# HKUDS/GPT-ST

Measured on AMD Instinct MI355X. Metric: pretrain steps/sec at (B=32,T=12,N=170,C=64), higher is better.
Workload: dtype f32; 1 GPU; BASELINE configs[1]: PEMS08-shape synthetic pretrain step, per-GPU B=32 T=12 N=170 C=64 base=1, epoch 200/300 (adaptive mask + KL), fwd+loss+bwd+clip+Adam, hipGraph=True, 4 full optimiser steps on 4 different resident batches per graph replay; global_batch=32, parallelism=dp1

## Files before the change

gpt-st_amd/csrc/guidein.hip:

```cpp
#include "mfma_tile.h"
#include "kl_guest.h"

#define GI_CHUNKS 3

template <int C>
__global__ __launch_bounds__(256) void guide_in_fwd_kernel(const float* __restrict__ src, int lda, const float* __restrict__ w1,
                                                           const float* __restrict__ b1, const float* __restrict__ Wn, const float* __restrict__ bn,
                                                           float* __restrict__ h1, int BT, int N) {
    constexpr int LPR = C / 4, RPP = 256 / LPR, NQ = 256 / C, U = 4;
    __shared__ __attribute__((aligned(16))) float part[NQ * 2 * C];
    __shared__ __attribute__((aligned(16))) float vec[2 * C];
    const int n = blockIdx.x, chunk = blockIdx.y, tid = threadIdx.x;
    {
        const int q = tid / C, o = tid % C;
        const float* W = Wn + (size_t)n * C * C;
        float au = 0.f, ac = 0.f;
#pragma unroll 8
        for (int i = q * (C / NQ); i < (q + 1) * (C / NQ); ++i) {
            const float x = W[(size_t)i * C + o];
            au = fmaf(w1[i], x, au);
            ac = fmaf(b1[i], x, ac);
        }
        part[(q * 2 + 0) * C + o] = au;
        part[(q * 2 + 1) * C + o] = ac;
    }
    __syncthreads();
    if (tid < C) {
        float s0 = 0.f, s1 = 0.f;
#pragma unroll
        for (int q = 0; q < NQ; ++q) { s0 += part[(q * 2 + 0) * C + tid]; s1 += part[(q * 2 + 1) * C + tid]; }
        vec[tid] = s0; vec[C + tid] = s1 + bn[(size_t)n * C + tid];
    }
    __syncthreads();
    const int slot = tid / LPR, c4 = tid % LPR;
    const float4 u4 = ld4(vec + 4 * c4), k4 = ld4(vec + C + 4 * c4);
    const int per = (BT + GI_CHUNKS - 1) / GI_CHUNKS, r0 = chunk * per, r1 = min(BT, r0 + per);
    for (int rr = r0 + slot; rr < r1; rr += RPP * U) {
        float s[U];
#pragma unroll
        for (int u = 0; u < U; ++u) s[u] = src[((size_t)min(rr + u * RPP, r1 - 1) * N + n) * lda];
#pragma unroll
        for (int u = 0; u < U; ++u) {
            const int r = rr + u * RPP;
            if (r < r1) {
                float4 y = f4fma(s[u], u4, k4);
                y.x = lrelu(y.x); y.y = lrelu(y.y); y.z = lrelu(y.z); y.w = lrelu(y.w);
                st4(h1 + ((size_t)r * N + n) * C + 4 * c4, y);
            }
        }
    }
}

template <int C>
__global__ __launch_bounds__(256) void guide_in_bwd_kernel(const float* __restrict__ dPre, const float* __restrict__ src, int lda,
                                                           const float* __restrict__ w1, const float* __restrict__ b1, const float* __restrict__ Wn,
                                                           float* __restrict__ dWb, float* __restrict__ dinp, int BT, int N) {
    __shared__ __attribute__((aligned(16))) float lds[guide_in_bwd_lds_floats<C>()];
    guide_in_bwd_body<C>(dPre, src, lda, w1, b1, Wn, dWb, dinp, BT, N, blockIdx.x, lds);
}

extern "C" int gptst_guide_in_fwd(const float* src, int lda, const float* w1, const float* b1, const float* Wn, const float* bn, float* h1,
                                  int BT, int N, int C, void* stream) {
    if (!src || !w1 || !b1 || !Wn || !bn || !h1 || BT <= 0 || N <= 0 || lda <= 0) return GPTST_EARG;
    if (C == 64) hipLaunchKernelGGL((guide_in_fwd_kernel<64>), dim3(N, GI_CHUNKS), dim3(256), 0, (hipStream_t)stream, src, lda, w1, b1, Wn, bn, h1, BT, N);
    else if (C == 128) hipLaunchKernelGGL((guide_in_fwd_kernel<128>), dim3(N, GI_CHUNKS), dim3(256), 0, (hipStream_t)stream, src, lda, w1, b1, Wn, bn, h1, BT, N);
    else return GPTST_ESHAPE;
    GPTST_CHECK_LAUNCH();
    return GPTST_OK;
}

extern "C" int gptst_guide_in_bwd(const float* dPre, const float* src, int lda, const float* w1, const float* b1, const float* Wn, float* dWb,
                                  float* dinp, int BT, int N, int C, void* stream) {
    if (!dPre || !src || !w1 || !b1 || !Wn || !dWb || !dinp || BT <= 0 || N <= 0 || lda <= 0) return GPTST_EARG;
    if (C == 64) hipLaunchKernelGGL((guide_in_bwd_kernel<64>), dim3(N), dim3(256), 0, (hipStream_t)stream, dPre, src, lda, w1, b1, Wn, dWb, dinp, BT, N);
    else if (C == 128) hipLaunchKernelGGL((guide_in_bwd_kernel<128>), dim3(N), dim3(256), 0, (hipStream_t)stream, dPre, src, lda, w1, b1, Wn, dWb, dinp, BT, N);
    else return GPTST_ESHAPE;
    GPTST_CHECK_LAUNCH();
    return GPTST_OK;
}

template <int C>
__global__ __launch_bounds__(256) void guide_uc_kernel(const float* __restrict__ w1, const float* __restrict__ b1, const float* __restrict__ Wn,
                                                       const float* __restrict__ bn, float* __restrict__ uc) {
    constexpr int NQ = 256 / C;
    __shared__ __attribute__((aligned(16))) float part[NQ * 2 * C];
    const int n = blockIdx.x, tid = threadIdx.x;
    const int q = tid / C, o = tid % C;
    const float* W = Wn + (size_t)n * C * C;
    float au = 0.f, ac = 0.f;
#pragma unroll 8
    for (int i = q * (C / NQ); i < (q + 1) * (C / NQ); ++i) {
        const float x = W[(size_t)i * C + o];
        au = fmaf(w1[i], x, au);
        ac = fmaf(b1[i], x, ac);
    }
    part[(q * 2 + 0) * C + o] = au;
    part[(q * 2 + 1) * C + o] = ac;
    __syncthreads();
    if (tid < C) {
        float s0 = 0.f, s1 = 0.f;
#pragma unroll
        for (int qq = 0; qq < NQ; ++qq) { s0 += part[(qq * 2 + 0) * C + tid]; s1 += part[(qq * 2 + 1) * C + tid]; }
        uc[(size_t)n * 2 * C + tid] = s0;
        uc[(size_t)n * 2 * C + C + tid] = s1 + bn[(size_t)n * C + tid];
    }
}

#define GH_P 68
extern thread_local int g_apply_tpw;
__global__ __launch_bounds__(256, 2) void guide_head_fwd_kernel(const float* __restrict__ src, int lda, const float* __restrict__ uc,
                                                                const float* __restrict__ Wbt, const float* __restrict__ bbt,
                                                                const float* __restrict__ W3, const float* __restrict__ b3,
                                                                float* __restrict__ h1, float* __restrict__ h2, float* __restrict__ prob,
                                                                int* __restrict__ label, int N, int J, int tiles_per_wave) {
    constexpr int C = 64;
    __shared__ __attribute__((aligned(16))) float Wl[C * C];
    __shared__ __attribute__((aligned(16))) float tl[4][16 * GH_P];
    const int lane = threadIdx.x & 63, wave = threadIdx.x >> 6;
    const int j = lane & 15, kk = lane >> 4;
    const int g = blockIdx.x;
    const int ntiles = (N + 15) / 16;
    const int t0 = (blockIdx.y * 4 + wave) * tiles_per_wave, t1 = min(ntiles, t0 + tiles_per_wave);
    const float4 bias4 = ld4(bbt + (size_t)g * C + 4 * j);
    float4 bw[4];
#pragma unroll
    for (int q = 0; q < 4; ++q) bw[q] = j < J ? ld4(W3 + (size_t)j * C + 16 * q + 4 * kk) : f4zero();
    const float bj = j < J ? b3[j] : 0.f;
    float sn;
    float4 un[4], cn[4];
    auto fetch = [&](int t) {
        const int m = min(t * 16 + j, N - 1);
        sn = src[((size_t)g * N + m) * lda];
#pragma unroll
        for (int q = 0; q < 4; ++q) { un[q] = ld4(uc + (size_t)m * 2 * C + 16 * q + 4 * kk); cn[q] = ld4(uc + (size_t)m * 2 * C + C + 16 * q + 4 * kk); }
    };
    if (t0 < t1) fetch(t0);
    load_w_lds<C, 256>(Wl, Wbt + (size_t)g * C * C, 0, threadIdx.x);
    __syncthreads();
    float4 bv[4][4];
#pragma unroll
    for (int q = 0; q < 4; ++q)
#pragma unroll
        for (int e = 0; e < 4; ++e) bv[q][e] = ld4(Wl + (16 * q + 4 * kk + e) * C + 4 * j);
    float* tile = tl[wave];
    for (int t = t0; t < t1; ++t) {
        float4 a[4];
        const int mrow = t * 16 + j;
#pragma unroll
        for (int q = 0; q < 4; ++q) {
            float4 y = f4fma(sn, un[q], cn[q]);
            y.x = lrelu(y.x); y.y = lrelu(y.y); y.z = lrelu(y.z); y.w = lrelu(y.w);
            if (mrow < N) st4(h1 + ((size_t)g * N + mrow) * C + 16 * q + 4 * kk, y); else y = f4zero();
            a[q] = y;
        }
        if (t + 1 < t1) fetch(t + 1);
        SB();
        f32x4 acc[4];
#pragma unroll
        for (int ct = 0; ct < 4; ++ct) acc[ct] = (f32x4){0.f, 0.f, 0.f, 0.f};
#pragma unroll
        for (int q = 0; q < 4; ++q) {
            const float av[4] = {a[q].x, a[q].y, a[q].z, a[q].w};
#pragma unroll
            for (int e = 0; e < 4; ++e) {
                acc[0] = __builtin_amdgcn_mfma_f32_16x16x4f32(av[e], bv[q][e].x, acc[0], 0, 0, 0);
                acc[1] = __builtin_amdgcn_mfma_f32_16x16x4f32(av[e], bv[q][e].y, acc[1], 0, 0, 0);
                acc[2] = __builtin_amdgcn_mfma_f32_16x16x4f32(av[e], bv[q][e].z, acc[2], 0, 0, 0);
                acc[3] = __builtin_amdgcn_mfma_f32_16x16x4f32(av[e], bv[q][e].w, acc[3], 0, 0, 0);
            }
        }
        SB();
#pragma unroll
        for (int r = 0; r < 4; ++r) {
            const int m = t * 16 + kk * 4 + r;
            float4 y = f4add(make_float4(acc[0][r], acc[1][r], acc[2][r], acc[3][r]), bias4);
            y.x = lrelu(y.x); y.y = lrelu(y.y); y.z = lrelu(y.z); y.w = lrelu(y.w);
            if (m < N) st4(h2 + ((size_t)g * N + m) * C + 4 * j, y);
            st4(tile + (kk * 4 + r) * GH_P + 4 * j, y);
        }
        f32x4 z0 = {0.f, 0.f, 0.f, 0.f}, z1 = {0.f, 0.f, 0.f, 0.f};
#pragma unroll
        for (int q = 0; q < 4; ++q) {
            const float4 x = ld4(tile + j * GH_P + 16 * q + 4 * kk);
            z0 = __builtin_amdgcn_mfma_f32_16x16x4f32(x.x, bw[q].x, z0, 0, 0, 0);
            z1 = __builtin_amdgcn_mfma_f32_16x16x4f32(x.y, bw[q].y, z1, 0, 0, 0);
            z0 = __builtin_amdgcn_mfma_f32_16x16x4f32(x.z, bw[q].z, z0, 0, 0, 0);
            z1 = __builtin_amdgcn_mfma_f32_16x16x4f32(x.w, bw[q].w, z1, 0, 0, 0);
        }
#pragma unroll
        for (int r = 0; r < 4; ++r) {
            const int m = t * 16 + kk * 4 + r;
            const size_t i = (size_t)g * N + m;
            float v = z0[r] + z1[r] + bj;
            const float mx = group_max<16>(j < J ? v : -3.0e38f);
            const float e = j < J ? expf(v - mx) : 0.f;
            v = e / group_sum<16>(e);
            if (m < N && j < J) prob[i * J + j] = v;
            const float vv = j < J ? v : -3.0e38f;
            const float gm = group_max<16>(vv);
            const int first = (int)(-group_max<16>(vv == gm ? -(float)j : -3.0e38f));
            if (m < N && j == 0) label[i] = first;
        }
    }
}

extern "C" int gptst_guide_uc_floats(int N, int C) { return N * 2 * C; }

extern "C" int gptst_guide_head_fwd(const float* src, int lda, const float* w1, const float* b1, const float* Wn, const float* bn, const float* Wbt,
                                    const float* bbt, const float* W3, const float* b3, float* uc, float* h1, float* h2, float* prob, int* label,
                                    int BT, int N, int C, int J, void* stream) {
    if (!src || !w1 || !b1 || !Wn || !bn || !Wbt || !bbt || !W3 || !b3 || !uc || !h1 || !h2 || !prob || !label || BT <= 0 || N <= 0 || lda <= 0 || J <= 0)
        return GPTST_EARG;
    if (C != 64 || J > 16) return GPTST_ESHAPE;
    hipLaunchKernelGGL((guide_uc_kernel<64>), dim3(N), dim3(256), 0, (hipStream_t)stream, w1, b1, Wn, bn, uc);
    const int ntiles = (N + 15) / 16;
    int tpw = 1;
    if (g_apply_tpw > 0) tpw = g_apply_tpw;
    if (tpw < 1) tpw = 1;
    const int gy = (ntiles + 4 * tpw - 1) / (4 * tpw);
    hipLaunchKernelGGL(guide_head_fwd_kernel, dim3(BT, gy), dim3(256), 0, (hipStream_t)stream, src, lda, uc, Wbt, bbt, W3, b3, h1, h2, prob, label, N, J, tpw);
    GPTST_CHECK_LAUNCH();
    return GPTST_OK;
}
```

gpt-st_amd/csrc/stepbegin.hip:

```cpp
#include "common.h"

__device__ __forceinline__ void philox4x32_10(unsigned c0, unsigned c1, unsigned c2, unsigned c3, unsigned k0, unsigned k1, unsigned (&o)[4]) {
#pragma unroll
    for (int r = 0; r < 10; ++r) {
        const unsigned long long p0 = 0xD2511F53ull * c0, p1 = 0xCD9E8D57ull * c2;
        const unsigned n0 = (unsigned)(p1 >> 32) ^ c1 ^ k0, n1 = (unsigned)p1, n2 = (unsigned)(p0 >> 32) ^ c3 ^ k1, n3 = (unsigned)p0;
        c0 = n0; c1 = n1; c2 = n2; c3 = n3;
        k0 += 0x9E3779B9u; k1 += 0xBB67AE85u;
    }
    o[0] = c0; o[1] = c1; o[2] = c2; o[3] = c3;
}

__global__ __launch_bounds__(256) void step_begin_kernel(float* __restrict__ z0, long n0, float* __restrict__ z1, long n1,
                                                         const float* __restrict__ src, float* __restrict__ tidx, int BT, int N, int lda,
                                                         int base, float* __restrict__ noise, long n_noise, const int* __restrict__ rng) {
    const long q0 = n0 / 4, q1 = n1 / 4, stride = (long)gridDim.x * 256;
    for (long i = (long)blockIdx.x * 256 + threadIdx.x; i < q0 + q1; i += stride) {
        if (i < q0) st4(z0 + 4 * i, f4zero()); else st4(z1 + 4 * (i - q0), f4zero());
    }
    if (blockIdx.x == 0) {
        for (long i = 4 * q0 + threadIdx.x; i < n0; i += 256) z0[i] = 0.f;
        for (long i = 4 * q1 + threadIdx.x; i < n1; i += 256) z1[i] = 0.f;
    }
    if (tidx != nullptr)
        for (long i = (long)blockIdx.x * 256 + threadIdx.x; i < 2L * BT; i += stride)
            tidx[i] = src[(size_t)(i / 2) * N * lda + base + (i & 1)];
    if (noise != nullptr) {
        const unsigned seed = (unsigned)rng[0], step = (unsigned)rng[1];
        for (long i = (long)blockIdx.x * 256 + threadIdx.x; 4 * i < n_noise; i += stride) {
            unsigned w[4];
            philox4x32_10((unsigned)i, (unsigned)(i >> 32), step, 0u, seed, 0x5EEDu, w);
            const float4 u = make_float4((w[0] >> 8) * 5.9604644775390625e-8f, (w[1] >> 8) * 5.9604644775390625e-8f,
                                         (w[2] >> 8) * 5.9604644775390625e-8f, (w[3] >> 8) * 5.9604644775390625e-8f);
            if (4 * i + 3 < n_noise) st4(noise + 4 * i, u);
            else { const float uv[4] = {u.x, u.y, u.z, u.w}; for (int k = 0; 4 * i + k < n_noise; ++k) noise[4 * i + k] = uv[k]; }
        }
    }
}

extern "C" int gptst_step_begin(float* z0, long n0, float* z1, long n1, const float* src, float* tidx, int BT, int N, int lda, int base,
                                float* noise, long n_noise, const int* rng, void* stream) {
    if (!z0 || n0 <= 0 || n1 < 0 || (n1 > 0 && !z1) || (tidx && (!src || BT <= 0 || N <= 0 || lda < base + 2))) return GPTST_EARG;
    if (noise && (n_noise <= 0 || !rng)) return GPTST_EARG;
    long q = (n0 + n1) / 4;
    int nb = (int)((q + 255) / 256); if (nb > 1024) nb = 1024; if (nb < 1) nb = 1;
    hipLaunchKernelGGL(step_begin_kernel, dim3(nb), dim3(256), 0, (hipStream_t)stream, z0, n0, z1, n1, src, tidx, BT, N, lda, base, noise,
                       noise ? n_noise : 0L, rng);
    GPTST_CHECK_LAUNCH();
    return GPTST_OK;
}
```

gpt-st_amd/csrc/timefeat.hip:

```cpp
#include "common.h"

struct TfParams {
    const float *wd, *bd, *ww, *bw, *w1, *b1, *w2, *b2, *w3, *b3;
};
struct TfGrads {
    float *wd, *bd, *ww, *bw, *w1, *b1, *w2, *b2, *w3, *b3;
};

template <int E, int NT = 256> struct TfCfg { static constexpr int ROWS = NT / E; };

template <int E>
__device__ __forceinline__ float tf_matvec(const float (&wrow)[E], float b, const float* __restrict__ xline) {
    float s = b;
#pragma unroll
    for (int i = 0; i < E; ++i) s = fmaf(wrow[i], xline[i], s);
    return s;
}

template <int E>
__device__ __forceinline__ float tf_input(const TfParams& p, const float* __restrict__ tidx, int r, int e, int K) {
    float s = p.bd[e] + p.bw[e];
    for (int k = 0; k < K; ++k) {
        s = fmaf(p.wd[e * K + k], tidx[((size_t)r * K + k) * 2 + 0], s);
        s = fmaf(p.ww[e * K + k], tidx[((size_t)r * K + k) * 2 + 1], s);
    }
    return s;
}

#define TF_SH_FLOATS (7 * 128 * 3)

template <int E>
__device__ __forceinline__ void tf_fwd_body(const TfParams& p, const float* __restrict__ tidx, float* __restrict__ out,
                                            int rows, int K, int blk, float* __restrict__ shraw) {
    constexpr int ROWS = TfCfg<E>::ROWS;
    float (*line)[E + 1] = reinterpret_cast<float (*)[E + 1]>(shraw);
    const int e = threadIdx.x % E, rl = threadIdx.x / E;
    const int r = blk * ROWS + rl;
    const bool valid = r < rows;
    float w1[E], w2[E], w3[E];
#pragma unroll
    for (int i = 0; i < E; ++i) { w1[i] = p.w1[e * E + i]; w2[i] = p.w2[e * E + i]; w3[i] = p.w3[e * E + i]; }
    line[rl][e] = valid ? tf_input<E>(p, tidx, r, e, K) : 0.f;
    __syncthreads();
    float h = fmaxf(tf_matvec<E>(w1, p.b1[e], line[rl]), 0.f);
    __syncthreads();
    line[rl][e] = h;
    __syncthreads();
    h = fmaxf(tf_matvec<E>(w2, p.b2[e], line[rl]), 0.f);
    __syncthreads();
    line[rl][e] = h;
    __syncthreads();
    h = tf_matvec<E>(w3, p.b3[e], line[rl]);
    if (valid) out[(size_t)r * E + e] = h;
}

template <bool DET> __device__ __forceinline__ void tf_add(float* p, float v) { if (DET) *p += v; else atomicAdd(p, v); }

template <int E, bool DET, int NT>
__device__ __forceinline__ void tf_bwd_body(const TfParams& p, const TfGrads& g, const float* __restrict__ tidx,
                                            const float* __restrict__ dout, int rows, int K, int blk, float* __restrict__ shraw) {
    constexpr int ROWS = TfCfg<E, NT>::ROWS;
    float (*sh)[ROWS][E + 1] = reinterpret_cast<float (*)[ROWS][E + 1]>(shraw);
    const int tid = threadIdx.x, e = tid % E, rl = tid / E;
    const int r = blk * ROWS + rl;
    const bool valid = r < rows;
    float w1[E], w2[E], w3[E], c1[E], c2[E], c3[E];
#pragma unroll
    for (int i = 0; i < E; ++i) {
        w1[i] = p.w1[e * E + i]; w2[i] = p.w2[e * E + i]; w3[i] = p.w3[e * E + i];
        c1[i] = p.w1[i * E + e]; c2[i] = p.w2[i * E + e]; c3[i] = p.w3[i * E + e];
    }
    const float h0 = valid ? tf_input<E>(p, tidx, r, e, K) : 0.f;
    sh[0][rl][e] = h0;
    __syncthreads();
    const float h1 = fmaxf(tf_matvec<E>(w1, p.b1[e], sh[0][rl]), 0.f);
    sh[1][rl][e] = h1;
    __syncthreads();
    const float h2 = fmaxf(tf_matvec<E>(w2, p.b2[e], sh[1][rl]), 0.f);
    sh[2][rl][e] = h2;
    const float d3 = valid ? dout[(size_t)r * E + e] : 0.f;
    sh[3][rl][e] = d3;
    __syncthreads();
    const float z2 = h2 > 0.f ? tf_matvec<E>(c3, 0.f, sh[3][rl]) : 0.f;
    sh[4][rl][e] = z2;
    __syncthreads();
    const float z1 = h1 > 0.f ? tf_matvec<E>(c2, 0.f, sh[4][rl]) : 0.f;
    sh[5][rl][e] = z1;
    __syncthreads();
    const float z0 = tf_matvec<E>(c1, 0.f, sh[5][rl]);
    sh[6][rl][e] = z0;
    __syncthreads();
    const int nrow = min(ROWS, rows - blk * ROWS);
    for (int idx = tid; idx < 3 * E * E; idx += NT) {
        const int which = idx / (E * E), eo = (idx / E) % E, i = idx % E;
        const int ga = which == 0 ? 3 : (which == 1 ? 4 : 5), gb = which == 0 ? 2 : (which == 1 ? 1 : 0);
        float s = 0.f;
        for (int rr = 0; rr < nrow; ++rr) s = fmaf(sh[ga][rr][eo], sh[gb][rr][i], s);
        float* dst = which == 0 ? g.w3 : (which == 1 ? g.w2 : g.w1);
        tf_add<DET>(dst + eo * E + i, s);
    }
    for (int idx = tid; idx < 4 * E; idx += NT) {
        const int which = idx / E, eo = idx % E;
        const int ga = which == 0 ? 3 : (which == 1 ? 4 : (which == 2 ? 5 : 6));
        float s = 0.f;
        for (int rr = 0; rr < nrow; ++rr) s += sh[ga][rr][eo];
        if (which == 0) tf_add<DET>(g.b3 + eo, s);
        else if (which == 1) tf_add<DET>(g.b2 + eo, s);
        else if (which == 2) tf_add<DET>(g.b1 + eo, s);
        else { tf_add<DET>(g.bd + eo, s); tf_add<DET>(g.bw + eo, s); }
    }
    for (int idx = tid; idx < 2 * E * K; idx += NT) {
        const int ch = idx / (E * K), eo = (idx / K) % E, k = idx % K;
        float s = 0.f;
        for (int rr = 0; rr < nrow; ++rr)
            s = fmaf(sh[6][rr][eo], tidx[((size_t)(blk * ROWS + rr) * K + k) * 2 + ch], s);
        tf_add<DET>((ch == 0 ? g.wd : g.ww) + eo * K + k, s);
    }
}

#define TF_MAXJ 16
struct TfJob { TfParams p; TfGrads g; const float* tidx; float* out; const float* dout; int rows, K, E, blk0; };
struct TfJobs { TfJob j[TF_MAXJ]; int n; };

#define TF_DET_T 1024
template <int BWD>
__global__ __launch_bounds__(BWD == 2 ? TF_DET_T : 256) void timefeat_jobs_kernel(TfJobs t) {
    constexpr int NT = BWD == 2 ? TF_DET_T : 256;
    __shared__ float shraw[TF_SH_FLOATS * (NT / 256)];
    int q = 0;
    if (BWD == 2) q = blockIdx.x;
    else for (int i = 1; i < t.n; ++i) if ((int)blockIdx.x >= t.j[i].blk0) q = i;
    const TfJob& a = t.j[q];
    const int blk = blockIdx.x - a.blk0;
    const int nblk = (a.rows + NT / a.E - 1) / (NT / a.E);
#define TF_CASE(EE)                                                                              \
    case EE:                                                                                     \
        if (BWD == 2) { for (int b2 = 0; b2 < nblk; ++b2) { tf_bwd_body<EE, true, NT>(a.p, a.g, a.tidx, a.dout, a.rows, a.K, b2, shraw); __syncthreads(); } } \
        else if (BWD == 1) tf_bwd_body<EE, false, NT>(a.p, a.g, a.tidx, a.dout, a.rows, a.K, blk, shraw); \
        else tf_fwd_body<EE>(a.p, a.tidx, a.out, a.rows, a.K, blk, shraw);                       \
        break;
    switch (a.E) { TF_CASE(2) TF_CASE(4) TF_CASE(8) TF_CASE(16) default: break; }
#undef TF_CASE
}

static int tf_launch(TfJobs& t, int bwd, hipStream_t st) {
    int nb = 0;
    for (int q = 0; q < t.n; ++q) {
        TfJob& a = t.j[q];
        if (!a.p.wd || !a.tidx || a.rows <= 0 || a.K <= 0 || (bwd ? (!a.dout || !a.g.wd) : !a.out)) return GPTST_EARG;
        if (a.E != 2 && a.E != 4 && a.E != 8 && a.E != 16) return GPTST_ESHAPE;
        const int rows_per = 256 / a.E;
        a.blk0 = nb;
        nb += (a.rows + rows_per - 1) / rows_per;
    }
    if (bwd && g_deterministic) hipLaunchKernelGGL(timefeat_jobs_kernel<2>, dim3(t.n), dim3(TF_DET_T), 0, st, t);
    else if (bwd) hipLaunchKernelGGL(timefeat_jobs_kernel<1>, dim3(nb), dim3(256), 0, st, t);
    else hipLaunchKernelGGL(timefeat_jobs_kernel<0>, dim3(nb), dim3(256), 0, st, t);
    GPTST_CHECK_LAUNCH();
    return GPTST_OK;
}

extern "C" int gptst_timefeat_fwd(const float* wd, const float* bd, const float* ww, const float* bw, const float* w1, const float* b1,
                                  const float* w2, const float* b2, const float* w3, const float* b3, const float* tidx, float* out,
                                  int rows, int K, int E, void* stream) {
    TfJobs t; t.n = 1;
    t.j[0] = TfJob{TfParams{wd, bd, ww, bw, w1, b1, w2, b2, w3, b3}, TfGrads{}, tidx, out, nullptr, rows, K, E, 0};
    return tf_launch(t, 0, (hipStream_t)stream);
}

extern "C" int gptst_timefeat_bwd(const float* wd, const float* bd, const float* ww, const float* bw, const float* w1, const float* b1,
                                  const float* w2, const float* b2, const float* w3, const float* b3, float* gwd, float* gbd, float* gww,
                                  float* gbw, float* gw1, float* gb1, float* gw2, float* gb2, float* gw3, float* gb3, const float* tidx,
                                  const float* dout, int rows, int K, int E, void* stream) {
    TfJobs t; t.n = 1;
    t.j[0] = TfJob{TfParams{wd, bd, ww, bw, w1, b1, w2, b2, w3, b3}, TfGrads{gwd, gbd, gww, gbw, gw1, gb1, gw2, gb2, gw3, gb3}, tidx,
                   nullptr, dout, rows, K, E, 0};
    return tf_launch(t, 1, (hipStream_t)stream);
}

extern "C" int gptst_timefeat_jobs(int njobs, int bwd, const void* const* params, const void* const* grads, const float* tidx,
                                   const void* const* io, const int* rows, const int* K, const int* E, void* stream) {
    if (njobs <= 0 || njobs > TF_MAXJ || !params || !io || !rows || !K || !E || (bwd && !grads)) return GPTST_EARG;
    TfJobs t; t.n = njobs;
    for (int q = 0; q < njobs; ++q) {
        const float* const* pp = (const float* const*)params + 10 * q;
        TfGrads g{};
        if (bwd) { float* const* gg = (float* const*)grads + 10 * q; g = TfGrads{gg[0], gg[1], gg[2], gg[3], gg[4], gg[5], gg[6], gg[7], gg[8], gg[9]}; }
        t.j[q] = TfJob{TfParams{pp[0], pp[1], pp[2], pp[3], pp[4], pp[5], pp[6], pp[7], pp[8], pp[9]}, g, tidx,
                       bwd ? nullptr : (float*)io[q], bwd ? (const float*)io[q] : nullptr, rows[q], K[q], E[q], 0};
    }
    return tf_launch(t, bwd, (hipStream_t)stream);
}
```

gpt-st_amd/engine.py:

```python
import contextlib
import os
import threading
from typing import Any, NamedTuple

import torch

from . import _C, ops
from .ops import (EPI_ADD_DPRE, EPI_ADD_PREMUL, EPI_LRELU, EPI_PREMUL, EPI_PLAIN, EPI_RES_LRELU, MODE_NODE, MODE_SHARED, MODE_TIME, PRO_DPRE, PRO_NONE)

TF_NAMES = ("ln_day", "ln_week", "ln1", "ln2", "ln")


class ZeroArena:

    def __init__(self, device):
        self.device, self.buf, self.off, self.need = device, None, 0, 0

    def begin(self, zero=True):
        pending = None
        if self.buf is None or self.buf.numel() < self.need:
            self.buf = torch.zeros(max(self.need, 1), device=self.device) if self.need else None
        elif self.buf is not None:
            if zero:
                self.buf.zero_()
            else:
                pending = self.buf
        self.off, self.need = 0, 0
        return pending

    def zeros(self, *shape):
        n = 1
        for d in shape:
            n *= d
        n4 = (n + 3) // 4 * 4
        self.need += n4
        if self.buf is None or self.off + n4 > self.buf.numel():
            return torch.zeros(*shape, device=self.device)
        t = self.buf[self.off:self.off + n].view(*shape)
        self.off += n4
        return t


class _Context(threading.local):
    ARENA = None
    NODE_REDUCE = None
    NO_HANDOFFS = False


CTX = _Context()




class Reductions:

    def __init__(self):
        self.jobs = ops.PoolJobs()
        self.late = ops.PoolJobs()
        self.no_carry = False
        self.grams = []
        self.tf = []
        self.keep = []
        self.on_bucket = None
        self.nbucket = 0
        self.bucket_inline = False
        self.fork_side = None
        self.forked = False
        self._dG = self._dA = None

    def take_carry(self, mb):
        if not CARRY_RED or self.no_carry or self.on_bucket is not None or CTX.NODE_REDUCE is not None or not self.jobs.jobs:
            return None
        take, rest, nb = [], [], 0.0
        for j in self.jobs.jobs:
            b = 4.0 * j[5] * j[7] * j[8] / 2 ** 20
            if j[0] in (ops.PoolJobs.BWD_POOL, ops.PoolJobs.BWD_EMB) and nb + b <= mb and len(take) < 100 and (j[7] | j[9]) % 4 == 0:
                take.append(j); nb += b
            else:
                rest.append(j)
        if not take:
            return None
        self.jobs.jobs = rest
        c = ops.PoolJobs()
        c.jobs = take
        return c

    def untake(self, carry):
        if carry is not None and carry.jobs:
            self.jobs.jobs = carry.jobs + self.jobs.jobs
            carry.jobs = []

    def gram(self, A, dG, dA, N, nsG):
        self.grams.append((A, dG, dA, N, nsG))

    def timefeat(self, p, g, pfx, tidx, dout, spg=False):
        B, T = tidx.shape[0], tidx.shape[1]
        rows, K = (B, T) if spg else (B * T, 1)
        self.tf.append((_tf_tensors(p, pfx), _tf_tensors(g, pfx), dout, rows, K))

    def flush_async(self, tidx):
        if self.bucket_inline and self.on_bucket is not None and self.nbucket == 0 and (self.jobs.jobs or self.late.jobs or self.grams or self.tf):
            self._run(tidx)
            self.fork_side.wait_stream(torch.cuda.current_stream())
            with torch.cuda.stream(self.fork_side):
                self.on_bucket(0)
            self.forked = True
            self.nbucket += 1

    def flush(self, tidx):
        self._run(tidx)
        if self.forked:
            torch.cuda.current_stream().wait_stream(self.fork_side)
            self.forked = False

    def _run(self, tidx):
        gr, self.grams = sorted(self.grams, key=lambda t: t[0].data_ptr()), []
        while gr:
            A, dG, dA, N, nsG = gr.pop(0)
            while gr and gr[0][0].data_ptr() == A.data_ptr() + 4 * A.numel() and gr[0][1].data_ptr() == dG.data_ptr() + 4 * dG.numel() \
                    and gr[0][2].data_ptr() == dA.data_ptr() + 4 * dA.numel() and gr[0][3:] == (N, nsG):
                A2, dG2, dA2 = gr.pop(0)[:3]
                A = torch.as_strided(A, (A.shape[0] + A2.shape[0],) + tuple(A.shape[1:]), A.stride())
                dG = torch.as_strided(dG, (dG.shape[0] + dG2.shape[0],) + tuple(dG.shape[1:]), dG.stride())
                dA = torch.as_strided(dA, (dA.shape[0] + dA2.shape[0],) + tuple(dA.shape[1:]), dA.stride())
            ops.gram_bwd(A, dG, out=dA, layers=A.shape[0] // N, nsplit=nsG)
        self.jobs.jobs, self.late.jobs = self.jobs.jobs + self.late.jobs, []
        self.jobs.launch()
        tf, self.tf = self.tf, []
        ops.timefeat_jobs_bwd(tf, tidx)
        self.keep = []


def _zeros(ref, *shape):
    if CTX.ARENA is not None:
        return CTX.ARENA.zeros(*shape)
    return torch.zeros(*shape, device=ref.device)


def _tf_tensors(d, pfx):
    out = []
    for n in TF_NAMES:
        out += [d[pfx + n + ".weight"], d[pfx + n + ".bias"]]
    return out


def _tf_job(p, pfx, tidx, spg=False):
    B, T = tidx.shape[0], tidx.shape[1]
    rows, K = (B, T) if spg else (B * T, 1)
    return (_tf_tensors(p, pfx), rows, K)


DROP_R = os.environ.get("GPTST_DROP_R", "0") == "1"


def _ht_fused_bwd(dims):
    return dims[3] == 64 and FUSE_HT_BWD


def hypertem_core_fwd(x, G, Wbt, bbt, dims):
    B, T, N, C = dims
    if C == 64:
        keep = not (DROP_R and _ht_fused_bwd(dims) and ops.wgrad_nsplit(MODE_TIME, B * T, N, C) == 1)
        R, out = ops.hypertem_fwd(x.view(B, T, N, C), G, Wbt, bbt, want_R=keep)
        R, out = (R.view(-1, C) if keep else None), out.view(-1, C)
    else:
        R = ops.tmix(x.view(B, T, N, C), G).view(-1, C)
        out = ops.apply(R, Wbt, MODE_TIME, B * T, N, bias=bbt, resid=x, epi=EPI_RES_LRELU)
    return out, (x, R, out, G, Wbt)


FUSE_HT_BWD = True


def graph_grad_splits(dims):
    return dims[0] if dims[3] == 64 else 1


CHAIN128 = os.environ.get("GPTST_CHAIN128", "1") == "1"


def chain_ok(dims):
    return _ht_fused_bwd(dims) or (CHAIN128 and dims[3] == 128)


def _wb_cols(dWb, C):
    return dWb[:, :C * C], dWb[:, C * C:]


def _wb_record(dWb, ns, C):
    return dWb[:, :C * C], ns, dWb[:, C * C:]


def hypertem_core_bwd(saved, dout, dG_out, dims, chain=False, premul=False):
    B, T, N, C = dims
    x, R, out, G, Wbt = saved
    BT = B * T
    assert not chain or chain_ok(dims)
    if _ht_fused_bwd(dims):
        dx, dWb, ns, _ = ops.hypertem_bwd_wgrad(dout.view(B, T, N, C), None if chain else out.view(B, T, N, C), x.view(B, T, N, C), G, Wbt,
                                                R.view(B, T, N, C) if R is not None else None, dG=dG_out, premul=chain and premul)
        dWbt, dbias = _wb_cols(dWb, C)
        dx = dx.view(-1, C)
    elif C == 64:
        dWb, ns = ops.wgrad(R, dout, MODE_TIME, BT, N, D2=out, pro=PRO_DPRE, colsum_d=True)
        dWbt, dbias = _wb_cols(dWb, C)
        dx, _, _ = ops.hypertem_bwd(dout.view(B, T, N, C), out.view(B, T, N, C), x.view(B, T, N, C), G, Wbt, dG=dG_out, want_dbias=False)
        dx = dx.view(-1, C)
    elif chain:
        dWb, ns = ops.wgrad(R, dout, MODE_TIME, BT, N, colsum_d=True)
        dWbt, dbias = _wb_cols(dWb, C)
        dR = ops.apply(dout, Wbt, MODE_TIME, BT, N, transw=True)
        dx, _ = ops.tmix_bwd_chain(dR.view(B, T, N, C), x.view(B, T, N, C), G, dout.view(B, T, N, C), premul=premul, dG=dG_out[0])
        dx = dx.view(-1, C)
    else:
        dWb, ns = ops.wgrad(R, dout, MODE_TIME, BT, N, D2=out, pro=PRO_DPRE, colsum_d=True)
        dWbt, dbias = _wb_cols(dWb, C)
        dR = ops.apply(dout, Wbt, MODE_TIME, BT, N, A2=out, transw=True, pro=PRO_DPRE)
        dx, _ = ops.tmix_bwd(dR.view(B, T, N, C), x.view(B, T, N, C), G, dout.view(B, T, N, C), out.view(B, T, N, C), dG=dG_out[0])
        dx = dx.view(-1, C)
    return dx, (dWbt, ns, dbias)


CARRY_RED = os.environ.get("GPTST_CARRY_RED", "1") == "1"
CARRY_MB = float(os.environ.get("GPTST_CARRY_MB", "25"))
CARRY_KL = os.environ.get("GPTST_CARRY_KL", "1") == "1"
PAIR_UNDER_DP = os.environ.get("GPTST_PAIR_UNDER_DP", "1") == "1"
PAIR_BWD = os.environ.get("GPTST_PAIR_BWD", "1") == "1"


@contextlib.contextmanager
def no_handoffs():
    from . import _C
    keep = (CTX.NO_HANDOFFS, _C.lib().value("gptst_mask_cooperative_state"))
    CTX.NO_HANDOFFS = True
    _C.lib().call("gptst_mask_cooperative", 0)
    try:
        yield
    finally:
        CTX.NO_HANDOFFS = keep[0]
        _C.lib().call("gptst_mask_cooperative", keep[1])


def pair_bwd_on():
    return PAIR_BWD and not CTX.NO_HANDOFFS


def cross_role():
    return 0 if CTX.NO_HANDOFFS else CROSS_ROLE


def _ht_pair_shape_ok(dims):
    B, T, N, C = dims
    if T != 12 or C != 64:
        return False
    ns = ops.wgrad_nsplit(MODE_TIME, B * T, N, C)
    rps = (-(-N // ns) + 1) & ~1
    return -(-N // rps) == ns


def ht_pair_ok(saved1, saved0, dims):
    return (pair_bwd_on() and dims[3] == 64 and not isinstance(saved1, EncIn) and saved1[1] is not None and saved0[1] is not None
            and _ht_fused_bwd(dims) and _ht_pair_shape_ok(dims))


class PendingH1:

    def __init__(self, saved, dd, dG, dWb):
        self.saved, self.dd, self.dG, self.dWb = saved, dd, dG, dWb


def ht_pair_bwd(saved1, saved0, dout, dG1, dG0, dims, dWb1=None):
    B, T, N, C = dims
    if not ht_pair_ok(saved1, saved0, dims):
        assert dWb1 is None
        return None
    x1, R1, _, G1, Wbt1 = saved1
    x0, R0, _, G0, Wbt0 = saved0
    v = lambda a: a.view(B, T, N, C)
    r = ops.hypertem_bwd_pair(v(dout), v(x1), G1, Wbt1, v(R1), v(x0), G0, Wbt0, v(R0), dG1, dG0, _zeros(dout, B), dWb1=dWb1)
    assert r is not None or dWb1 is None
    if r is None:
        return None
    dmid, dx0, dWb1, dWb0, ns = r
    return dx0.view(-1, C), _wb_record(dWb1, ns, C), _wb_record(dWb0, ns, C)


FUSE_CROSS = os.environ.get("GPTST_FUSE_CROSS", "1") == "1"
CAP_LIN = os.environ.get("GPTST_CAP_LIN", "1") == "1"
CROSS_ROLE = int(os.environ.get("GPTST_CROSS_ROLE", "1"))


def cap_head_fwd(p, pfx, x, dadj, dyn, dims, num_route, HS, HT):
    B, T, N, C = dims
    c, s, Y = ops.cap_route_fwd(x.view(B, T, N, C), p[pfx + "ln_p.weight"], p[pfx + "ln_p.bias"], dadj, HS, num_route,
                                reduce_nodes=CTX.NODE_REDUCE, want_Y=True)
    fused = ops.cap_cross_rec_fwd(s, dyn, p[pfx + "mask_template"], c, B, T, N, HS, HT) if (FUSE_CROSS and CTX.NODE_REDUCE is None) else None
    if fused is not None:
        v, Ht, Rt, rec = fused
    else:
        v, Ht, Rt = ops.cap_cross_fwd(s, dyn, p[pfx + "mask_template"], B, T, HS, HT)
        rec = ops.cap_rec_fwd(c, v, N, C)
    return rec, c, (s, v, Ht, Rt, Y)


def cap_core_fwd(p, pfx, x, dadj, dyn, Wn, bn, dims, num_route, HS, HT):
    B, T, N, C = dims
    rec, c, (s, v, Ht, Rt, Y) = cap_head_fwd(p, pfx, x, dadj, dyn, dims, num_route, HS, HT)
    out = ops.apply(rec, Wn, MODE_NODE, B * T, N, bias=bn, resid=x, epi=EPI_RES_LRELU)
    return out, c, (x, out, rec, c, s, v, Ht, Rt, dyn, Wn, Y)


CHAIN_FWD = os.environ.get("GPTST_CHAIN_FWD", "1") == "1"


def chain_fwd_ok(dims):
    return CHAIN_FWD and dims[3] == 64 and not DROP_R


def ht_chain_fwd(x, stages, dims, kl=None):
    B, T, N, C = dims
    res = ops.hypertem_chain_fwd(x.view(B, T, N, C), stages, guest=kl.guest() if kl is not None else None)
    saved, xin = [], x
    for (G, Wbt, _b), (R, o) in zip(stages, res):
        o = o.view(-1, C)
        saved.append((xin, R.view(-1, C), o, G, Wbt))
        xin = o
    return saved, xin


def cap_core_bwd(p, g, pfx, saved, dout, dims, HS, HT, red, chain=False):
    B, T, N, C = dims
    x, out, rec, c, s, v, Ht, Rt, dyn, Wn, Y = saved
    BT, dev = B * T, x.device
    assert not chain or chain_ok(dims)
    if C == 64:
        drec, dWn, dbn, ns = ops.apply_wgrad(dout, None if chain else out, rec, Wn, MODE_NODE, BT, N)
    elif chain:
        drec = ops.apply(dout, Wn, MODE_NODE, BT, N, transw=True)
        dWb, ns = ops.wgrad(rec, dout, MODE_NODE, BT, N, colsum_d=True)
        dWn, dbn = _wb_cols(dWb, C)
    else:
        drec = ops.apply(dout, Wn, MODE_NODE, BT, N, A2=out, transw=True, pro=PRO_DPRE)
        dWb, ns = ops.wgrad(rec, dout, MODE_NODE, BT, N, D2=out, pro=PRO_DPRE, colsum_d=True)
        dWn, dbn = _wb_cols(dWb, C)
    dc1, dv = ops.cap_rec_bwd(drec, c, v, reduce_nodes=CTX.NODE_REDUCE)
    gw, gb = g[pfx + "ln_p.weight"], g[pfx + "ln_p.bias"]
    if FUSE_CROSS and CAP_LIN and C == 64 and CTX.NODE_REDUCE is None and Y is None:
        carry = red.take_carry(CARRY_MB) if cross_role() and _C.lib().value("gptst_cap_route_roles_ok", B, T, N, C, HS, HT) == 1 else None
        lin = ops.cap_cross_route_lin_bwd(x.view(B, T, N, C), p[pfx + "ln_p.weight"], p[pfx + "ln_p.bias"], c, dc1, dv, s, Rt, Ht, dyn,
                                          p[pfx + "mask_template"], dout, None if chain else out, chain, B, T, HS, HT,
                                          flags=_zeros(x, 4 * B) if cross_role() else None, jobs=carry)
        red.untake(carry)
        if lin is not None:
            dx, dWp, dbp, dlogit, ddyn = lin
            red.jobs.bwd_pool(_ones(dev, dWp.shape[0]), dWp, gw.view(1, C * C))
            red.jobs.bwd_pool(_ones(dev, dbp.shape[0]), dbp, gb.view(1, C))
            return dx, (dWn, ns, dbn, ddyn, dlogit)
    fused = None
    if FUSE_CROSS and CTX.NODE_REDUCE is None and Y is None:
        fused = ops.cap_cross_route_bwd(x.view(B, T, N, C), p[pfx + "ln_p.weight"], p[pfx + "ln_p.bias"], c, dc1, dv, s, Rt, Ht, dyn,
                                        p[pfx + "mask_template"], B, T, HS, HT, flags=_zeros(x, 4 * B) if cross_role() else None)
    if fused is not None:
        dY, dlogit, ddyn = fused
    else:
        dS, ddyn = ops.cap_cross_bwd(dv, s, Rt, Ht, dyn, p[pfx + "mask_template"], B, T, HS, HT)
        dY, dlogit = ops.cap_route_bwd(x.view(B, T, N, C), p[pfx + "ln_p.weight"], p[pfx + "ln_p.bias"], c, dc1, dS, Y=Y)
    if C == 64:
        dx, dWp, dbp, ns2 = ops.linear_bwd(dY, x, p[pfx + "ln_p.weight"], dout, None if chain else out, premul=chain)
        red.jobs.bwd_pool(_ones(dev, ns2), dWp, gw.view(1, C * C))
        red.jobs.bwd_pool(_ones(dev, ns2), dbp, gb.view(1, C))
    else:
        if chain:
            dx = ops.apply(dY, p[pfx + "ln_p.weight"], MODE_SHARED, BT, N, resid=dout, resid2=x, epi=EPI_ADD_PREMUL)
        else:
            dx = ops.apply(dY, p[pfx + "ln_p.weight"], MODE_SHARED, BT, N, resid=dout, resid2=out, epi=EPI_ADD_DPRE)
        dWp, ns2 = ops.wgrad(dY, x, MODE_SHARED, BT, N, colsum_a=True)
        dWp, dbp = _wb_cols(dWp, C)
        red.jobs.bwd_pool(_ones(dev, ns2), dWp, gw.view(1, C * C))
        red.jobs.bwd_pool(_ones(dev, ns2), dbp, gb.view(1, C))
    return dx, (dWn, ns, dbn, ddyn, dlogit)


_ONES = {}


def _ones(dev, n=1):
    if (dev, n) not in _ONES:
        _ONES[(dev, n)] = torch.ones(n, 1, device=dev)
    return _ONES[(dev, n)]


def condlin_fwd(x, Wg, bg, mode, dims):
    B, T, N, C = dims
    out = ops.apply(x, Wg, mode, B * T, N, bias=bg, epi=EPI_LRELU)
    return out, (x, out, Wg)


def condlin_bwd(saved, dout, emb, wpool, bpool, g_wpool, g_bpool, d_emb, mode, dims, red, chain=False, premul=False, carried=None):
    B, T, N, C = dims
    x, out, Wg = saved
    R, K = emb.shape
    assert not chain or chain_ok(dims)
    if carried is not None:
        dx, dW, db, ns = carried
    elif C == 64:
        dx, dW, db, ns = ops.apply_wgrad(dout, None if chain else out, x, Wg, mode, B * T, N, premul=chain and premul)
    elif chain:
        dx = (ops.apply(dout, Wg, mode, B * T, N, transw=True, resid2=x, epi=EPI_PREMUL) if premul
              else ops.apply(dout, Wg, mode, B * T, N, transw=True))
        dWb, ns = ops.wgrad(x, dout, mode, B * T, N, colsum_d=True)
        dW, db = _wb_cols(dWb, C)
    else:
        dx = ops.apply(dout, Wg, mode, B * T, N, A2=out, transw=True, pro=PRO_DPRE)
        dWb, ns = ops.wgrad(x, dout, mode, B * T, N, D2=out, pro=PRO_DPRE, colsum_d=True)
        dW, db = _wb_cols(dWb, C)
    dW = dW if dW.dim() == 2 else dW.view(ns * R, C * C)
    red.jobs.bwd_pool(emb, dW, g_wpool.view(K, C * C), nsplit=ns)
    red.jobs.bwd_pool(emb, db, g_bpool, nsplit=ns)
    red.jobs.bwd_emb(dW, wpool.view(K, C * C), d_emb, nsplit=ns)
    red.jobs.bwd_emb(db, bpool, d_emb, nsplit=ns)
    return dx


ENC, DEC = "encoder.STHCN_encode.", "decoder.STHCN_decode."
GUIDE_TF = "encoder.teb4mask."


def _sthcn_names(pfx):
    return [pfx + "hyperTem%d." % i for i in (1, 2, 3, 4)], [pfx + "cap1.", pfx + "cap2."]


def _sthcn_gen_jobs(p, pfx, emb, jobs, A_all, dims, G_all=None, gjobs=None):
    gjobs = jobs if gjobs is None else gjobs
    B, T, N, C = dims
    time_eb, teb, tes = emb
    ne, nes = p[pfx + "node_embeddings"], p[pfx + "node_embeddings_spg"]
    hts, cps = _sthcn_names(pfx)
    adj0 = p[hts[0] + "adj"]
    d, Hm = adj0.shape[0], adj0.shape[1]
    cadj, tadj = p[cps[0] + "adj"], p[cps[0] + "t_adj"]
    ds, HS, HT = cadj.shape[0], cadj.shape[1], tadj.shape[1]
    for i, h in enumerate(hts):
        jobs.fwd(ne, p[h + "adj"].view(d, Hm * T), out=A_all[i])
        if G_all is not None:
            gjobs.gram(ne, p[h + "adj"].view(d, Hm * T), out=G_all[i], A=A_all[i])
    Wb = [jobs.fwd(time_eb, t) for h in hts for t in (p[h + "weights_pool"], p[h + "bias_pool"])]
    Wn = [jobs.fwd(nes, t) for c in cps for t in (p[c + "weights_spa"], p[c + "bias_spa"])]
    dadj = [jobs.fwd(teb, p[c + "adj"].view(ds, HS * N)) for c in cps]
    dyn = [jobs.fwd(tes, p[c + "t_adj"].view(ds, HT * T * HS)).view(B, HT, T * HS) for c in cps]
    return dict(emb=emb, gen=(A_all, hts, cps, d, Hm, ds, HS, HT), Wb=Wb, Wn=Wn, dadj=dadj, dyn=dyn)


def gen_all(p, tidx, dims, which=(ENC, DEC), guide=True, defer=False):
    B, T, N, C = dims
    tfj = []
    for pfx in which:
        tfj += [_tf_job(p, pfx + "time_feature1.", tidx), _tf_job(p, pfx + "time_feature1_.", tidx),
                _tf_job(p, pfx + "time_feature2.", tidx, spg=True)]
    if guide:
        tfj.append(_tf_job(p, GUIDE_TF, tidx))
    embs = ops.timefeat_jobs_fwd(tfj, tidx)
    jobs = ops.PoolJobs()
    now = ops.PoolJobs() if defer else jobs
    res = {}
    L = 4 * len(which)
    if guide:
        gj = now
        m = "encoder.MLP_RL."
        t4m = embs[-1]
        res["guide"] = (t4m, gj.fwd(p["encoder.neb4mask"], p[m + "weights_pool_spa"]), gj.fwd(p["encoder.neb4mask"], p[m + "bias_pool_spa"]),
                        gj.fwd(t4m, p[m + "weights_pool_tem"]), gj.fwd(t4m, p[m + "bias_pool_tem"]))
    if L:
        adj0 = p[which[0] + "hyperTem1.adj"]
        Hm = adj0.shape[1]
        A_all = torch.empty(L, N, Hm * T, device=tidx.device)
        G_all = torch.empty(L, N, T, T, device=tidx.device)
        for k, pfx in enumerate(which):
            res[pfx] = _sthcn_gen_jobs(p, pfx, embs[3 * k:3 * k + 3], jobs, A_all[4 * k:4 * k + 4], dims, G_all[4 * k:4 * k + 4])
            res[pfx]["slot"] = (k, len(which))
            res[pfx]["G_all"] = G_all[4 * k:4 * k + 4]

    if defer:
        now.launch()
        res["pending"] = jobs
        return res
    jobs.launch()
    return res


def sthcn_fwd(p, pfx, tidx, x, dims, num_route, gen=None, head=None, next_gen=None, kl=None):
    if gen is None:
        gen = gen_all(p, tidx, dims, which=(pfx,), guide=False)[pfx]
    A_all, hts, cps, d, Hm, ds, HS, HT = gen["gen"]
    Wn, dadj, dyn = gen["Wn"], gen["dadj"], gen["dyn"]
    ht = lambda i, gn=gen: (gn["G_all"][i], gn["Wb"][2 * i], gn["Wb"][2 * i + 1])
    cap = lambda i, x: cap_core_fwd(p, cps[i], x, dadj[i], dyn[i], Wn[2 * i], Wn[2 * i + 1], dims, num_route, HS, HT)
    pairs = chain_fwd_ok(dims)
    sv, nhead = {}, None
    if head is not None:
        x, sv["h1"] = head
    else:
        x, sv["h1"] = hypertem_core_fwd(x, *ht(0), dims)
    x, c1, sv["c1"] = cap(0, x)
    if pairs:
        if kl is not None and kl.c1 is None:
            kl.c1 = c1
        (sv["h2"], sv["h3"]), x = ht_chain_fwd(x, [ht(1), ht(2)], dims, kl)
    else:
        x, sv["h2"] = hypertem_core_fwd(x, *ht(1), dims)
        x, sv["h3"] = hypertem_core_fwd(x, *ht(2), dims)
    x, _, sv["c2"] = cap(1, x)
    if pairs and next_gen is not None:
        (sv["h4"], h1n), xn = ht_chain_fwd(x, [ht(3), ht(0, next_gen)], dims, kl)
        x, nhead = sv["h4"][2], (xn, h1n)
    else:
        x, sv["h4"] = hypertem_core_fwd(x, *ht(3), dims)
    sv["emb"] = gen["emb"]
    sv["gen"] = gen["gen"]
    sv["slot"] = gen.get("slot")
    return x, c1, sv, nhead


def _grad_buffers(red, slot, N, T, HmT, ref, nsG):
    if slot is None:
        return torch.empty(4, nsG, N, T, T, device=ref.device), torch.empty(4, N, HmT, device=ref.device)
    k, n = slot
    if red._dG is None or red._dG.shape[0] != 4 * n:
        red._dG = torch.empty(4 * n, nsG, N, T, T, device=ref.device)
        red._dA = torch.empty(4 * n, N, HmT, device=ref.device)
    return red._dG[4 * k:4 * k + 4], red._dA[4 * k:4 * k + 4]


def sthcn_bwd(p, g, pfx, tidx, sv, dout, dims, red, chain=False, premul_in=False, defer_h1=False, after_pending=None):
    B, T, N, C = dims
    time_eb, teb, tes = sv["emb"]
    A_all, hts, cps, d, Hm, ds, HS, HT = sv["gen"]
    ne, nes = p[pfx + "node_embeddings"], p[pfx + "node_embeddings_spg"]
    dne, dnes = g[pfx + "node_embeddings"], g[pfx + "node_embeddings_spg"]
    d_te, d_teb, d_tes = _zeros(time_eb, *time_eb.shape), _zeros(teb, *teb.shape), _zeros(tes, *tes.shape)
    nsG = graph_grad_splits(dims)
    dG_all, dA_all = _grad_buffers(red, sv.get("slot"), N, T, Hm * T, dout, nsG)
    J = red.jobs
    CC, BT = C * C, B * T

    def queue_ht(h, hp):
        dWbt, ns, dbias = hp
        J.bwd_pool(time_eb, dWbt, g[h + "weights_pool"].view(d, CC), nsplit=ns)
        J.bwd_pool(time_eb, dbias, g[h + "bias_pool"], nsplit=ns)
        J.bwd_emb(dWbt, p[h + "weights_pool"].view(d, CC), d_te, nsplit=ns)
        J.bwd_emb(dbias, p[h + "bias_pool"], d_te, nsplit=ns)

    def queue_cap(c, cp):
        dWn, ns, dbn, ddyn, dlogit = cp
        dW2 = dWn if dWn.dim() == 2 else dWn.view(ns * N, CC)
        J.bwd_pool(nes, dW2, g[c + "weights_spa"].view(d, CC), nsplit=ns)
        J.bwd_pool(nes, dbn, g[c + "bias_spa"], nsplit=ns)
        J.bwd_emb(dW2, p[c + "weights_spa"].view(d, CC), dnes, nsplit=ns)
        J.bwd_emb(dbn, p[c + "bias_spa"], dnes, nsplit=ns)
        dd2 = ddyn.view(B, HT * T * HS)
        J.bwd_pool(tes, dd2, g[c + "t_adj"].view(ds, HT * T * HS))
        J.bwd_emb(dd2, p[c + "t_adj"].view(ds, HT * T * HS), d_tes)
        dl2 = dlogit.view(BT, HS * N)
        J.bwd_pool(teb, dl2, g[c + "adj"].view(ds, HS * N))
        J.bwd_emb(dl2, p[c + "adj"].view(ds, HS * N), d_teb)

    if isinstance(dout, PendingH1):
        up = dout
        dd, _, hp4 = ht_pair_bwd(up.saved, sv["h4"], up.dd, up.dG, dG_all[3], dims, dWb1=up.dWb)
        red.keep.append(up)
        if after_pending is not None:
            after_pending()
    else:
        dd, hp4 = hypertem_core_bwd(sv["h4"], dout, dG_all[3], dims, chain, True)
    queue_ht(hts[3], hp4)
    dd, cp2 = cap_core_bwd(p, g, cps[1], sv["c2"], dd, dims, HS, HT, red, chain)
    queue_cap(cps[1], cp2)
    pair = ht_pair_bwd(sv["h3"], sv["h2"], dd, dG_all[2], dG_all[1], dims) if chain and pair_bwd_on() else None
    if pair is not None:
        dd, hp3, hp2 = pair
    else:
        dd, hp3 = hypertem_core_bwd(sv["h3"], dd, dG_all[2], dims, chain, True)
        dd, hp2 = hypertem_core_bwd(sv["h2"], dd, dG_all[1], dims, chain, True)
    queue_ht(hts[2], hp3)
    queue_ht(hts[1], hp2)
    dd, cp1 = cap_core_bwd(p, g, cps[0], sv["c1"], dd, dims, HS, HT, red, chain)
    queue_cap(cps[0], cp1)
    if isinstance(sv["h1"], EncIn):
        assert chain
        e = sv["h1"]
        w, bi = p["encoder.dim_in_flow.weight"], p["encoder.dim_in_flow.bias"]
        if nsG == B:
            dWb, _, dinp = ops.encin_ht1_bwd(dd.view(B, T, N, C), e.source, e.mask, e.fill, w, bi, e.Wbt, e.ab, e.wv, dG=dG_all[0])
        else:
            dWb, dGb, dinp = ops.encin_ht1_bwd(dd.view(B, T, N, C), e.source, e.mask, e.fill, w, bi, e.Wbt, e.ab, e.wv)
            torch.sum(dGb, 0, out=dG_all[0][0])
        hp1 = _wb_record(dWb, 1, C)
        wb = _wb_view(g["encoder.dim_in_flow.weight"], g["encoder.dim_in_flow.bias"])
        if wb is not None:
            red.jobs.bwd_pool(_ones(dd.device, dinp.shape[0]), dinp, wb)
        else:
            g["encoder.dim_in_flow.weight"].add_(dinp[:, :C].sum(0).view(C, 1))
            g["encoder.dim_in_flow.bias"].add_(dinp[:, C:].sum(0))
        red.keep.append((dinp, dWb))
        dd = None
    elif defer_h1:
        assert chain and premul_in
        ns = ops.wgrad_nsplit(MODE_TIME, B * T, N, C)
        dWb = torch.empty(ns * B * T, C * C + C, device=dd.device, dtype=torch.float32)
        hp1 = _wb_record(dWb, ns, C)
        dd = PendingH1(sv["h1"], dd, dG_all[0], dWb)
    else:
        dd, hp1 = hypertem_core_bwd(sv["h1"], dd, dG_all[0], dims, chain, premul_in)
    queue_ht(hts[0], hp1)
    red.gram(A_all.view(4 * N, Hm, T), dG_all, dA_all.view(4 * N, Hm, T), N, nsG)
    for i, h in enumerate(hts):
        red.late.bwd_pool(ne, dA_all[i], g[h + "adj"].view(d, Hm * T))
        red.late.bwd_emb(dA_all[i], p[h + "adj"].view(d, Hm * T), dne)
    red.timefeat(p, g, pfx + "time_feature1.", tidx, d_te)
    red.timefeat(p, g, pfx + "time_feature1_.", tidx, d_teb)
    red.timefeat(p, g, pfx + "time_feature2.", tidx, d_tes, spg=True)
    red.keep.append((sv, hp1, hp2, hp3, hp4, cp1, cp2, dout))
    return dd


class EncIn:

    def __init__(self, source, mask, fill, Wbt, ab, wv):
        self.source, self.mask, self.fill, self.Wbt, self.ab, self.wv = source, mask, fill, Wbt, ab, wv


ENCIN = os.environ.get("GPTST_ENCIN", "1") == "1"


def encin_ok(dims, base):
    return ENCIN and base == 1 and dims[3] in (64, 128) and dims[1] == 12 and chain_ok(dims)


GUIDEIN = os.environ.get("GPTST_GUIDEIN", "1") == "1"
GUIDE_HEAD = os.environ.get("GPTST_GUIDE_HEAD", "1") == "1"


def guide_fwd(p, source, tidx, dims, base, gen=None, lowrank_in=False):
    B, T, N, C = dims
    if gen is None:
        gen = gen_all(p, tidx, dims, which=(), guide=True)["guide"]
    t4m, Wspa, bspa, Wtem, btem = gen
    m = "encoder.MLP_RL."
    if lowrank_in and GUIDEIN and GUIDE_HEAD and base == 1 and C == 64:
        r = ops.guide_head_fwd(source, p[m + "ln1.weight"], p[m + "ln1.bias"], Wspa, bspa, Wtem, btem, p[m + "ln3.weight"], p[m + "ln3.bias"])
        if r is not None:
            h1, h2, prob, label = r
            return prob, (t4m, ("lowrank", Wspa), (h1, h2, Wtem), h2, label)
    if lowrank_in and GUIDEIN and base == 1 and C in (64, 128):
        h1 = ops.guide_in_fwd(source, p[m + "ln1.weight"], p[m + "ln1.bias"], Wspa, bspa)
        s1 = ("lowrank", Wspa)
    else:
        h0 = ops.lin_in(source, base + 2, base, p[m + "ln1.weight"], p[m + "ln1.bias"], C)
        h1, s1 = condlin_fwd(h0, Wspa, bspa, MODE_NODE, dims)
    h2, s2 = condlin_fwd(h1, Wtem, btem, MODE_TIME, dims)
    prob, label = ops.rowdot(h2, p[m + "ln3.weight"], p[m + "ln3.bias"], softmax=True, want_label=True)
    return prob, (t4m, s1, s2, h2, label)


def _wb_view(gw, gb):
    n = gw.numel() + gb.numel()
    if gb.data_ptr() != gw.data_ptr() + 4 * gw.numel():
        return None
    return torch.as_strided(gw, (1, n), (n, 1))


def fused_tails_ok(p, C, base, HS):
    return (C in (64, 128) and base <= ops.TAIL_MAXJ and HS <= ops.TAIL_MAXJ
            and _wb_view(p["decoder.dim_flow_out.weight"], p["decoder.dim_flow_out.bias"]) is not None
            and _wb_view(p["encoder.MLP_RL.ln3.weight"], p["encoder.MLP_RL.ln3.bias"]) is not None)


def loss_tail(p, g, dec, source, mask, base, sigma, mu, thresh, sws, red, chain=False):
    wo = "decoder.dim_flow_out."
    out, dd, part = ops.tail_mae(dec, p[wo + "weight"], p[wo + "bias"], source, base + 2, mask, sigma, mu, thresh, sws, premul=chain)
    red.jobs.bwd_pool(_ones(dec.device, part.shape[0]), part, _wb_view(g[wo + "weight"], g[wo + "bias"]))
    red.keep.append((part, dd))
    return out, dd


def kl_head(p, g, sv_g, prob, c1, N, w, sws, red, chain=False, carried=None):
    m = "encoder.MLP_RL."
    dh2, part = carried if carried is not None else ops.tail_kl(sv_g[3], p[m + "ln3.weight"], prob, c1, N, w, sws, premul=chain)
    red.jobs.bwd_pool(_ones(prob.device, part.shape[0]), part, _wb_view(g[m + "ln3.weight"], g[m + "ln3.bias"]))
    red.keep.append((part, dh2))
    return dh2


def _linear_out_bwd(p, g, pfx, h, dy, C, chain, d_h=None):
    J = dy.shape[1]
    dh = ops.lin_in(dy, J, J, p[pfx + "weight"], None, C, wlayout=1)
    ops.rowouter(dy, J, J, h, g[pfx + "weight"], 1, asum=g[pfx + "bias"])
    if d_h is not None:
        dh = dh + d_h
    if chain:
        dh = dh * torch.where(h > 0, 1.0, 0.01)
    return dh


def guide_bwd(p, g, source, tidx, saved, dlogit, dims, base, red, dh2=None, chain=False, carried=(None, None)):
    B, T, N, C = dims
    t4m, s1, s2, h2 = saved[:4]
    m = "encoder.MLP_RL."
    if dh2 is None:
        dh2 = _linear_out_bwd(p, g, m + "ln3.", h2, dlogit, C, chain)
    d_t4m = _zeros(t4m, *t4m.shape)
    dh1 = condlin_bwd(s2, dh2, t4m, p[m + "weights_pool_tem"], p[m + "bias_pool_tem"], g[m + "weights_pool_tem"],
                      g[m + "bias_pool_tem"], d_t4m, MODE_TIME, dims, red, chain, True, carried=carried[0])
    if isinstance(s1[0], str):
        assert chain
        neb, wpool, bpool = p["encoder.neb4mask"], p[m + "weights_pool_spa"], p[m + "bias_pool_spa"]
        K = neb.shape[1]
        dWb, dinp = carried[1] if carried[1] is not None else ops.guide_in_bwd(dh1, source, p[m + "ln1.weight"], p[m + "ln1.bias"], s1[1])
        dW, db = _wb_cols(dWb, C)
        red.jobs.bwd_pool(neb, dW, g[m + "weights_pool_spa"].view(K, C * C))
        red.jobs.bwd_pool(neb, db, g[m + "bias_pool_spa"])
        red.jobs.bwd_emb(dW, wpool.view(K, C * C), g["encoder.neb4mask"])
        red.jobs.bwd_emb(db, bpool, g["encoder.neb4mask"])
        wb = _wb_view(g[m + "ln1.weight"], g[m + "ln1.bias"])
        if wb is not None:
            red.jobs.bwd_pool(_ones(dh1.device, N), dinp, wb)
        else:
            g[m + "ln1.weight"].add_(dinp[:, :C].sum(0).view(C, 1))
            g[m + "ln1.bias"].add_(dinp[:, C:].sum(0))
        red.keep.append((dWb, dinp))
        dh0 = None
    else:
        dh0 = condlin_bwd(s1, dh1, p["encoder.neb4mask"], p[m + "weights_pool_spa"], p[m + "bias_pool_spa"],
                          g[m + "weights_pool_spa"], g[m + "bias_pool_spa"], g["encoder.neb4mask"], MODE_NODE, dims, red, chain, False)
        _in_proj_grads(source, base, dh0, g[m + "ln1.weight"], g[m + "ln1.bias"], None, 0.0, red)
    red.timefeat(p, g, GUIDE_TF, tidx, d_t4m)
    red.keep.append((saved, dlogit, dh2, dh1, dh0))


def kl_carry_ok(dims, HS, sv_g):
    B, T, N, C = dims
    return (CARRY_KL and C == 64 and T == 12 and HS <= ops.TAIL_MAXJ and chain_fwd_ok(dims) and chain_ok(dims)
            and sv_g is not None and isinstance(sv_g[1][0], str))


class KlCarry:

    def __init__(self, p, sv_g, prob, source, dims, w, sws):
        self.p, self.sv_g, self.prob, self.source, self.dims, self.w, self.sws = p, sv_g, prob, source, dims, w, sws
        self.c1 = None
        self.stage = 0
        self.out = {}

    def guest(self):
        if self.c1 is None or self.stage == 3:
            return None
        B, T, N, C = self.dims
        m = "encoder.MLP_RL."
        p, sv_g, dev = self.p, self.sv_g, self.prob.device
        HS = self.prob.shape[1]
        st = self.stage + 1
        f = dict(device=dev, dtype=torch.float32)
        if st == 1:
            h2, W3 = sv_g[3], p[m + "ln3.weight"]
            dh2 = torch.empty_like(h2)
            part = torch.empty(ops.tail_parts(B * T * N), HS * C + HS, **f)
            self.out[1] = (dh2, part)
            ts = [h2, W3, self.prob, self.c1, dh2, part, self.sws]
        elif st == 2:
            h1, _, Wtem = sv_g[2]
            dh2 = self.out[1][0]
            ns = _C.lib().value("gptst_apply_wgrad_nsplit", MODE_TIME, B * T, N)
            dh1, dW, db = torch.empty_like(h1), torch.empty(ns * B * T, C * C, **f), torch.empty(ns * B * T, C, **f)
            self.out[2] = (dh1, dW, db, ns)
            ts = [dh2, h1, Wtem, dh1, dW, db]
        else:
            dWb, dinp = torch.empty(N, C * C + C, **f), torch.empty(N, 2 * C, **f)
            self.out[3] = (dWb, dinp)
            ts = [self.out[2][0], self.source, p[m + "ln1.weight"], p[m + "ln1.bias"], sv_g[1][1], dWb, dinp]
        self.stage = st
        return (st, ts, 0, ops.kl_guest_blocks(st, B, T, N), HS, self.source.shape[-1], self.w)

    def carried(self, st):
        return self.out.get(st)


def _in_proj_grads(source, base, dY, gW, gb, mask, fill, red):
    wb = _wb_view(gW, gb)
    if base == 1 and wb is not None:
        C = dY.shape[1]
        part = ops.rowouter_part(source, base + 2, base, dY, mask=mask, fill=fill)
        red.jobs.bwd_pool(_ones(dY.device, part.shape[0]), part[:, :2 * C], wb)
        red.keep.append(part)
    else:
        ops.rowouter(source, base + 2, base, dY, gW, 0, csum=gb, mask=mask, fill=fill)


class Forward(NamedTuple):
    emb: Any
    c1: Any
    dec: Any
    out: Any
    sv_e: Any
    sv_d: Any


def autoencoder_fwd(p, source, mask, dims, base, num_route, scaler_zeros, gen=None, tidx=None, lowrank_in=False, kl=None, head=True,
                    decoder=True, join=True):
    B, T, N, C = dims
    if tidx is None:
        tidx = source[:, :, 0, base:base + 2].contiguous()
    gen_e, gen_d = (gen[ENC], gen[DEC] if decoder else None) if gen is not None else (None, None)
    first = None
    if lowrank_in and gen_e is not None and encin_ok(dims, base):
        w, bi = p["encoder.dim_in_flow.weight"], p["encoder.dim_in_flow.bias"]
        G1, Wb = gen_e["G_all"][0], gen_e["Wb"]
        o1, ab, wv = ops.encin_ht1_fwd(source, base, mask, 0.0 if mask is None else scaler_zeros, w, bi, G1, Wb[0], Wb[1])
        first = (o1.view(-1, C), EncIn(source, mask, 0.0 if mask is None else scaler_zeros, Wb[0], ab, wv))
        x0 = None
    else:
        x0 = ops.lin_in(source, base + 2, base, p["encoder.dim_in_flow.weight"], p["encoder.dim_in_flow.bias"], C,
                        mask=mask, fill=scaler_zeros)
    emb, c1, sv_e, dec_h1 = sthcn_fwd(p, ENC, tidx, x0, dims, num_route, gen=gen_e, head=first, next_gen=gen_d if join else None, kl=kl)
    if not decoder:
        return Forward(emb, c1, None, None, sv_e, None)
    dec, _, sv_d, _ = sthcn_fwd(p, DEC, tidx, emb, dims, num_route, gen=gen_d, head=dec_h1, kl=kl)
    out = ops.rowdot(dec, p["decoder.dim_flow_out.weight"], p["decoder.dim_flow_out.bias"]) if head else None
    return Forward(emb, c1, dec, out, sv_e, sv_d)


def model_bwd(p, g, source, mask, tidx, sv_e, sv_d, dec, d_out, d_dec, dims, base, scaler_zeros, red, dd=None, chain=False):
    B, T, N, C = dims
    if dd is None:
        dd = _linear_out_bwd(p, g, "decoder.dim_flow_out.", dec, d_out, C, chain, d_h=d_dec)
    defer = (chain and (red.on_bucket is None or PAIR_UNDER_DP) and not isinstance(sv_d["h1"], EncIn)
             and ht_pair_ok(sv_d["h1"], sv_e["h4"], dims))
    late = defer and red.on_bucket is not None
    d_emb = sthcn_bwd(p, g, DEC, tidx, sv_d, dd, dims, red, chain, True, defer_h1=defer)
    if not late:
        red.flush_async(tidx)
    d_x0 = sthcn_bwd(p, g, ENC, tidx, sv_e, d_emb, dims, red, chain, False,
                     after_pending=(lambda: red.flush_async(tidx)) if late else None)
    red.flush_async(tidx)
    if d_x0 is not None:
        _in_proj_grads(source, base, d_x0, g["encoder.dim_in_flow.weight"], g["encoder.dim_in_flow.bias"], mask, scaler_zeros, red)


def step_bwd(p, g, source, mask, tidx, fw, prob, sv_g, dims, base, scaler_zeros, red, loss, stats, sws=None, with_kl=False, kl=None):
    B, T, N, C = dims
    sigma, mu, thresh = loss
    if sws is not None:
        chain = chain_ok(dims)
        done = kl.carried if kl is not None else (lambda st: None)
        _, dd = loss_tail(p, g, fw.dec, source, mask, base, sigma, mu, thresh, sws, red, chain=chain)
        model_bwd(p, g, source, mask, tidx, fw.sv_e, fw.sv_d, fw.dec, None, None, dims, base, scaler_zeros, red, dd=dd, chain=chain)
        if with_kl:
            dh2 = kl_head(p, g, sv_g, prob, fw.c1, N, 0.1, sws, red, chain=chain, carried=done(1))
            guide_bwd(p, g, source, tidx, sv_g, None, dims, base, red, dh2=dh2, chain=chain, carried=(done(2), done(3)))
    else:
        M = B * T * N
        ops.mae_fwd(fw.out, source, base + 2, mask, sigma, mu, thresh, M, base, stats)
        d_out = ops.mae_bwd(fw.out, source, base + 2, mask, sigma, mu, thresh, M, base, stats, normalize=False)
        model_bwd(p, g, source, mask, tidx, fw.sv_e, fw.sv_d, fw.dec, d_out, None, dims, base, scaler_zeros, red)
        if with_kl:
            dlogit = ops.kl(prob, fw.c1, N, 0.1, stats)
            guide_bwd(p, g, source, tidx, sv_g, dlogit, dims, base, red)


def module_bwd(p, g, source, mask, tidx, fw, prob, sv_g, dims, base, scaler_zeros, red, d_out, d_dec=None, d_prob=None, chain=False):
    model_bwd(p, g, source, mask, tidx, fw.sv_e, fw.sv_d, fw.dec, d_out, d_dec, dims, base, scaler_zeros, red, chain=chain)
    if d_prob is not None:
        dlogit = (prob * (d_prob - (d_prob * prob).sum(-1, keepdim=True))).contiguous()
        guide_bwd(p, g, source, tidx, sv_g, dlogit, dims, base, red, chain=chain)


def warm_up(fn):
    s = torch.cuda.Stream()
    s.wait_stream(torch.cuda.current_stream())
    with torch.cuda.stream(s):
        for _ in range(2):
            fn()
    torch.cuda.current_stream().wait_stream(s)
    torch.cuda.synchronize()
```

gpt-st_amd/ops.py:

```python
import torch

from . import _C

MODE_TIME, MODE_NODE, MODE_SHARED = 0, 1, 2
PRO_NONE, PRO_DPRE = 0, 1
EPI_PLAIN, EPI_RES_LRELU, EPI_ADD_DPRE, EPI_LRELU, EPI_ADD_PREMUL, EPI_PREMUL = 0, 1, 2, 3, 4, 5

_p = _C.ptr


TIMER = None
LAST_CALL = {}


CALL_LOCK = None


def _call(name, *args, tag="", nbytes=0):
    if CALL_LOCK is not None:
        with CALL_LOCK:
            _C.lib().call(name, *args, _C.stream())
        return
    if TIMER is None:
        _C.lib().call(name, *args, _C.stream())
        return
    e0, e1 = torch.cuda.Event(enable_timing=True), torch.cuda.Event(enable_timing=True)
    e0.record()
    _C.lib().call(name, *args, _C.stream())
    e1.record()
    TIMER.append((name, tag, e0, e1, nbytes))
    LAST_CALL[(name, tag)] = args


def _nb(*ts):
    return sum(t.numel() * t.element_size() for t in ts if t is not None)


def _chk(*ts):
    for t in ts:
        if t is not None:
            assert t.is_cuda and t.dtype == torch.float32 and t.is_contiguous(), (t.device, t.dtype, t.is_contiguous())


def poolgen(emb, pool, pool2=None):
    _chk(emb, pool, pool2)
    R, K = emb.shape
    cols = pool.numel() // K
    out = torch.empty((R,) + tuple(pool.shape[1:]), device=emb.device, dtype=torch.float32)
    out2, cols2 = None, 0
    if pool2 is not None:
        cols2 = pool2.numel() // K
        out2 = torch.empty((R,) + tuple(pool2.shape[1:]), device=emb.device, dtype=torch.float32)
    _call("gptst_poolgen_fwd", _p(emb), _p(pool), _p(out), cols, _p(pool2), _p(out2), cols2, R, K, nbytes=_nb(emb, pool, out, pool2, out2))
    return (out, out2) if pool2 is not None else out


def poolgen_bwd_pool(emb, dW, dpool, dW2=None, dpool2=None, nsplit=1):
    _chk(emb, dW, dpool, dW2, dpool2)
    R, K = emb.shape
    cols = dpool.numel() // K
    cols2 = dpool2.numel() // K if dpool2 is not None else 0
    _call("gptst_poolgen_bwd_pool", _p(emb), _p(dW), _p(dpool), cols, _p(dW2), _p(dpool2), cols2, R, nsplit, K,
          nbytes=_nb(emb, dW, dpool, dW2, dpool2))


def poolgen_bwd_emb(dW, pool, demb, dW2=None, pool2=None, nsplit=1):
    _chk(dW, pool, demb, dW2, pool2)
    R, K = demb.shape
    cols = pool.numel() // K
    cols2 = pool2.numel() // K if pool2 is not None else 0
    _call("gptst_poolgen_bwd_emb", _p(dW), _p(pool), cols, _p(dW2), _p(pool2), cols2, _p(demb), R, nsplit, K,
          nbytes=_nb(dW, pool, dW2, pool2, demb))


def _ptrs(ts):
    import ctypes
    return (ctypes.c_void_p * len(ts))(*[t.data_ptr() for t in ts])


def _ints(vs):
    import ctypes
    return (ctypes.c_int * len(vs))(*[int(v) for v in vs])


def poolgen_multi(emb, pools, outs=None):
    _chk(emb, *pools)
    R, K = emb.shape
    if outs is None:
        outs = [torch.empty((R,) + tuple(pl.shape[1:]), device=emb.device, dtype=torch.float32) for pl in pools]
    cols = [pl.numel() // K for pl in pools]
    _call("gptst_poolgen_fwd_multi", _p(emb), len(pools), _ptrs(pools), _ptrs(outs), _ints(cols), R, K, nbytes=_nb(emb, *pools, *outs))
    return outs


def poolgen_bwd_pool_multi(emb, dWs, dpools, nsplits=None):
    _chk(emb, *dWs, *dpools)
    R, K = emb.shape
    cols = [dp.numel() // K for dp in dpools]
    ns = nsplits if nsplits is not None else [1] * len(dWs)
    _call("gptst_poolgen_bwd_pool_multi", _p(emb), len(dWs), _ptrs(dWs), _ptrs(dpools), _ints(cols), _ints(ns), R, K,
          nbytes=_nb(emb, *dWs, *dpools))


def poolgen_bwd_emb_multi(dWs, pools, demb, nsplits=None):
    _chk(demb, *dWs, *pools)
    R, K = demb.shape
    cols = [pl.numel() // K for pl in pools]
    ns = nsplits if nsplits is not None else [1] * len(dWs)
    _call("gptst_poolgen_bwd_emb_multi", len(dWs), _ptrs(dWs), _ptrs(pools), _ints(cols), _ints(ns), _p(demb), R, K,
          nbytes=_nb(demb, *dWs, *pools))


class PoolJobs:
    FWD, BWD_POOL, BWD_EMB, GRAM = 0, 1, 2, 3

    def __init__(self):
        self.jobs = []
        self.post = []

    def fwd(self, emb, pool, out=None):
        _chk(emb, pool, out)
        R, K = emb.shape
        if out is None:
            out = torch.empty((R,) + tuple(pool.shape[1:]), device=emb.device, dtype=torch.float32)
        self.jobs.append((self.FWD, emb, None, pool, out, R, K, pool.numel() // K, 1, 0))
        return out

    def gram(self, emb, pool, out, A=None):
        _chk(emb, pool, out, A)
        R, K = emb.shape
        cols = pool.numel() // K
        assert cols % 12 == 0 and out.numel() == R * 144 and out.is_contiguous()
        if _C.lib().value("gptst_pool_jobs_gram_rows", K, cols) <= 0:
            assert A is not None and A.numel() == R * cols, "gram job does not fit and no forward output was given"
            self.post.append((A, out, R, cols // 12))
            return out
        self.jobs.append((self.GRAM, emb, None, pool, out, R, K, cols, 1, 0))
        return out

    @staticmethod
    def _ldx(dW, cols):
        assert dW.is_cuda and dW.dtype == torch.float32 and dW.dim() == 2 and dW.shape[1] == cols and dW.stride(1) == 1, (dW.shape, dW.stride(), cols)
        return dW.stride(0)

    def bwd_pool(self, emb, dW, dpool, nsplit=1):
        _chk(emb, dpool)
        R, K = emb.shape
        cols = dpool.numel() // K
        self.jobs.append((self.BWD_POOL, emb, dW, None, dpool, R, K, cols, nsplit, self._ldx(dW, cols)))

    def bwd_emb(self, dW, pool, demb, nsplit=1):
        _chk(pool, demb)
        R, K = demb.shape
        cols = pool.numel() // K
        self.jobs.append((self.BWD_EMB, None, dW, pool, demb, R, K, cols, nsplit, self._ldx(dW, cols)))

    def launch(self):
        js, self.jobs = self.jobs, []
        post, self.post = self.post, []
        if js:
            col = lambda i: [j[i] for j in js]
            _call("gptst_pool_jobs", len(js), _ints(col(0)), _ptrs0(col(1)), _ptrs0(col(2)), _ptrs0(col(3)), _ptrs0(col(4)), _ints(col(5)),
                  _ints(col(6)), _ints(col(7)), _ints(col(8)), _ints(col(9)), nbytes=_nb(*[t for j in js for t in j[1:5]]))
        for A, G, rows, Hm in post:
            _call("gptst_gram_fwd", _p(A), _p(G), rows, Hm)


def _ptrs0(ts):
    import ctypes
    return (ctypes.c_void_p * len(ts))(*[(t.data_ptr() if t is not None else None) for t in ts])


def apply(A, W, mode, BT, N, bias=None, resid=None, A2=None, transw=False, pro=PRO_NONE, epi=EPI_PLAIN, colsum=None,
          out=None, resid2=None):
    _chk(A, W, bias, resid, A2, resid2)
    C = A.shape[-1]
    if out is None:
        out = torch.empty_like(A)
    cs, ns = None, 0
    if colsum is not None:
        G = BT if mode == MODE_TIME else (N if mode == MODE_NODE else 1)
        ns = _C.lib().value("gptst_apply_nsplit", mode, BT, N, C)
        cs = torch.empty(ns * G, C, device=A.device, dtype=torch.float32)
    _call("gptst_apply", _p(A), _p(A2), _p(W), int(W.dim() == 3), int(transw), _p(bias), _p(resid), _p(resid2), _p(out), _p(cs),
          mode, pro, epi, BT, N, C, tag="mode%d pro%d epi%d" % (mode, pro, epi), nbytes=_nb(A, A2, W, bias, resid, resid2, out))
    if colsum is True:
        return out, cs, ns
    if colsum is not None:
        colsum.add_(cs.view(ns, -1, C).sum(0).view_as(colsum))
    return out


def apply_wgrad(dOut, Y, S, W, mode, BT, N, premul=False):
    _chk(dOut, Y, S, W)
    C = dOut.shape[-1]
    G = BT if mode == MODE_TIME else N
    ns = _C.lib().value("gptst_apply_wgrad_nsplit", mode, BT, N)
    dS = torch.empty_like(dOut)
    dW = torch.empty(ns * G, C * C, device=dOut.device, dtype=torch.float32)
    db = torch.empty(ns * G, C, device=dOut.device, dtype=torch.float32)
    _call("gptst_apply_wgrad", _p(dOut), _p(Y), _p(S), _p(W), _p(dS), _p(dW), _p(db), int(premul), mode, BT, N, C, tag="mode%d" % mode,
          nbytes=_nb(dOut, Y, S, W, dS, dW))
    return dS, dW, db, ns


def linear_bwd(dY, X, Wp, dOut, out, premul=False):
    _chk(dY, X, Wp, dOut, out)
    rows, C = dY.shape
    ns = _C.lib().value("gptst_linear_bwd_nsplit", rows)
    dX = torch.empty_like(dY)
    dWp = torch.empty(ns, C * C, device=dY.device, dtype=torch.float32)
    dbp = torch.empty(ns, C, device=dY.device, dtype=torch.float32)
    _call("gptst_linear_bwd", _p(dY), _p(X), _p(Wp), _p(dOut), _p(out), _p(dX), _p(dWp), _p(dbp), int(premul), rows, C,
          nbytes=_nb(dY, X, dOut, out, dX, dWp))
    return dX, dWp, dbp, ns


def wgrad_nsplit(mode, BT, N, C=64):
    return _C.lib().value("gptst_wgrad_nsplit", mode, BT, N, C)


def wgrad(A, D, mode, BT, N, D2=None, pro=PRO_NONE, colsum_a=False, colsum_d=False):
    _chk(A, D, D2)
    C = A.shape[-1]
    ns = wgrad_nsplit(mode, BT, N, C)
    G = BT if mode == MODE_TIME else (N if mode == MODE_NODE else 1)
    if colsum_a or colsum_d:
        dW = torch.empty(ns * G, C * C + C, device=A.device, dtype=torch.float32)
        _call("gptst_wgrad_colsum", _p(A), _p(D), _p(D2), _p(dW), mode, pro, 1 if colsum_a else 2, BT, N, C,
              tag="mode%d pro%d cs" % (mode, pro), nbytes=_nb(A, D, D2, dW))
    else:
        dW = torch.empty(ns * G, C, C, device=A.device, dtype=torch.float32)
        _call("gptst_wgrad", _p(A), _p(D), _p(D2), _p(dW), mode, pro, BT, N, C, tag="mode%d pro%d" % (mode, pro), nbytes=_nb(A, D, D2, dW))
    return dW, ns


def gram_fwd(A):
    N, Hm, T = A.shape
    G = torch.empty(N, T, T, device=A.device, dtype=torch.float32)
    _call("gptst_gram_fwd", _p(A), _p(G), N, Hm)
    return G


def gram_bwd(A, dG, out=None, layers=1, nsplit=1):
    LN, Hm, T = A.shape
    dA = out if out is not None else torch.empty_like(A)
    _call("gptst_gram_bwd", _p(A), _p(dG), _p(dA), layers, LN // layers, Hm, nsplit)
    return dA


def tmix(X, G, dOut=None, Y=None):
    _chk(X, G, dOut, Y)
    B, T, N, C = X.shape
    out = torch.empty_like(X)
    _call("gptst_tmix", _p(X), _p(G), _p(dOut), _p(Y), _p(out), B, T, N, C, tag="bwd" if dOut is not None else "fwd",
          nbytes=_nb(X, G, dOut, Y, out))
    return out


def hypertem_fwd(X, G, Wbt, bbt, want_R=True):
    _chk(X, G, Wbt, bbt)
    B, T, N, C = X.shape
    R = torch.empty_like(X) if want_R else None
    out = torch.empty_like(X)
    _call("gptst_hypertem_fwd", _p(X), _p(G), _p(Wbt), _p(bbt), _p(R), _p(out), B, T, N, C, nbytes=_nb(X, G, Wbt, bbt, R, out))
    return R, out


def hypertem_chain_fwd(X, stages, want_R=True, guest=None):
    B, T, N, C = X.shape
    _chk(X, *[t for st in stages for t in st])
    f = lambda: torch.empty(B, T, N, C, device=X.device, dtype=torch.float32)
    Rs = [f() if want_R else None for _ in stages]
    outs = [f() for _ in stages]
    chain = (_p(X), len(stages), _ptrs0([st[0] for st in stages]), _ptrs0([st[1] for st in stages]), _ptrs0([st[2] for st in stages]),
             _ptrs0(Rs), _ptrs0(outs), B, T, N, C)
    if guest is None:
        _call("gptst_hypertem_chain_fwd", *chain, tag="x%d" % len(stages), nbytes=_nb(X, *Rs, *outs))
    else:
        stage, ts, v0, v1, HS, lda, w = guest
        _chk(*ts)
        _call("gptst_hypertem_chain_fwd_kl", *chain, stage, _ptrs0(ts), v0, v1, HS, lda, float(w), tag="x%d+kl%d" % (len(stages), stage),
              nbytes=_nb(X, *Rs, *outs))
    return list(zip(Rs, outs))


def kl_guest_blocks(stage, B, T, N):
    return _C.lib().value("gptst_kl_guest_blocks", stage, B, T, N)


def encin_ht1_fwd(source, base, mask, fill, w, bi, G, Wbt, bbt):
    B, T, N, F = source.shape
    C = Wbt.shape[-1]
    assert base == 1
    _chk(source, mask, w, bi, G, Wbt, bbt)
    f = dict(device=source.device, dtype=torch.float32)
    out, ab, wv = torch.empty(B, T, N, C, **f), torch.empty(B * T * N, 2, **f), torch.empty(B * T, 2 * C, **f)
    _call("gptst_encin_ht1_fwd", _p(source), F, _p(mask), float(fill), _p(w), _p(bi), _p(G), _p(Wbt), _p(bbt), _p(out), _p(ab), _p(wv), B, T, N, C,
          nbytes=_nb(Wbt, out))
    return out, ab, wv


def encin_ht1_bwd(dPre, source, mask, fill, w, bi, Wbt, ab, wv, dG=None):
    B, T, N, F = source.shape
    C = Wbt.shape[-1]
    _chk(dPre, source, mask, w, bi, Wbt, ab, wv, dG)
    f = dict(device=source.device, dtype=torch.float32)
    dWb, dinp = torch.empty(B * T, C * C + C, **f), torch.empty(B * T, 2 * C, **f)
    if dG is None:
        dG = torch.empty(B, N, T, T, **f)
    _call("gptst_encin_ht1_bwd", _p(dPre), _p(source), F, _p(mask), float(fill), _p(w), _p(bi), _p(Wbt), _p(ab), _p(wv), _p(dWb), _p(dG), _p(dinp),
          B, T, N, C, nbytes=_nb(dPre, Wbt, dWb, dG))
    return dWb, dG, dinp


def guide_in_fwd(source, w1, b1, Wn, bn):
    B, T, N, F = source.shape
    C = Wn.shape[-1]
    _chk(source, w1, b1, Wn, bn)
    h1 = torch.empty(B * T * N, C, device=source.device, dtype=torch.float32)
    _call("gptst_guide_in_fwd", _p(source), F, _p(w1), _p(b1), _p(Wn), _p(bn), _p(h1), B * T, N, C, nbytes=_nb(Wn, h1))
    return h1


def guide_head_fwd(source, w1, b1, Wn, bn, Wbt, bbt, W3, b3):
    B, T, N, F = source.shape
    C, J = Wn.shape[-1], W3.shape[0]
    if C != 64 or J > 16:
        return None
    _chk(source, w1, b1, Wn, bn, Wbt, bbt, W3, b3)
    dev = source.device
    f = dict(device=dev, dtype=torch.float32)
    uc = torch.empty(N, 2 * C, **f)
    h1, h2 = torch.empty(B * T * N, C, **f), torch.empty(B * T * N, C, **f)
    prob = torch.empty(B * T * N, J, **f)
    label = torch.empty(B * T * N, device=dev, dtype=torch.int32)
    _call("gptst_guide_head_fwd", _p(source), F, _p(w1), _p(b1), _p(Wn), _p(bn), _p(Wbt), _p(bbt), _p(W3), _p(b3), _p(uc), _p(h1), _p(h2), _p(prob),
          _p(label), B * T, N, C, J, nbytes=_nb(Wbt, h1, h2, prob))
    return h1, h2, prob, label


def guide_in_bwd(dPre, source, w1, b1, Wn):
    B, T, N, F = source.shape
    C = Wn.shape[-1]
    _chk(dPre, source, w1, b1, Wn)
    f = dict(device=source.device, dtype=torch.float32)
    dWb, dinp = torch.empty(N, C * C + C, **f), torch.empty(N, 2 * C, **f)
    _call("gptst_guide_in_bwd", _p(dPre), _p(source), F, _p(w1), _p(b1), _p(Wn), _p(dWb), _p(dinp), B * T, N, C, nbytes=_nb(dPre, Wn, dWb))
    return dWb, dinp


def hypertem_ntiles(N):
    return _C.lib().value("gptst_hypertem_ntiles", N)


def hypertem_bwd(dOut, Y, X, G, Wbt, dG=None, want_dbias=True, premul=False):
    _chk(dOut, Y, X, G, Wbt, dG)
    B, T, N, C = X.shape
    dX = torch.empty_like(X)
    nt = hypertem_ntiles(N)
    dbias = torch.empty(nt * B * T, C, device=X.device, dtype=torch.float32) if want_dbias else None
    if dG is None:
        dG = torch.empty(B, N, T, T, device=X.device, dtype=torch.float32)
    _call("gptst_hypertem_bwd", _p(dOut), _p(Y), _p(X), _p(G), _p(Wbt), _p(dX), _p(dbias), _p(dG), int(premul), B, T, N, C,
          nbytes=_nb(dOut, Y, X, G, Wbt, dX))
    return dX, dbias, dG


def hypertem_bwd_wgrad(dOut, Y, X, G, Wbt, R, dG=None, premul=False):
    _chk(dOut, Y, X, G, Wbt, R, dG)
    B, T, N, C = X.shape
    dX = torch.empty_like(X)
    if dG is None:
        dG = torch.empty(B, N, T, T, device=X.device, dtype=torch.float32)
    ns = wgrad_nsplit(MODE_TIME, B * T, N, C)
    dWb = torch.empty(ns * B * T, C * C + C, device=X.device, dtype=torch.float32)
    _call("gptst_hypertem_bwd_wgrad", _p(dOut), _p(Y), _p(X), _p(G), _p(Wbt), _p(R), _p(dX), _p(dG), _p(dWb), int(premul), B, T, N, C,
          nbytes=_nb(dOut, Y, X, G, Wbt, R, dX, dWb))
    return dX, dWb, ns, dG


def hypertem_bwd_pair(dOut1, X1, G1, Wbt1, R1, X0, G0, Wbt0, R0, dG1, dG0, cnt, dWb1=None):
    _chk(dOut1, X1, G1, Wbt1, R1, X0, G0, Wbt0, R0, dG1, dG0, cnt, dWb1)
    B, T, N, C = X1.shape
    if C != 64:
        return None
    dXmid, dX0 = torch.empty_like(X1), torch.empty_like(X0)
    ns = wgrad_nsplit(MODE_TIME, B * T, N, C)
    dWb0 = torch.empty(ns * B * T, C * C + C, device=X1.device, dtype=torch.float32)
    if dWb1 is None:
        dWb1 = torch.empty_like(dWb0)
    assert dWb1.shape == dWb0.shape
    try:
        _call("gptst_hypertem_bwd_pair", _p(dOut1), _p(X1), _p(G1), _p(Wbt1), _p(R1), _p(X0), _p(G0), _p(Wbt0), _p(R0), _p(dXmid), _p(dX0),
              _p(dG1), _p(dG0), _p(dWb1), _p(dWb0), _p(cnt), B, T, N, C, nbytes=_nb(dOut1, X1, R1, X0, R0, dXmid, dX0, dWb0, dWb1))
    except _C.GptstError as e:
        if e.code != _C.ESHAPE:
            raise
        return None
    return dXmid, dX0, dWb1, dWb0, ns


def tmix_bwd(dR, X, G, dOut, Y, dG=None):
    _chk(dR, X, G, dOut, Y, dG)
    B, T, N, C = X.shape
    dX = torch.empty_like(X)
    if dG is None:
        dG = torch.empty(N, T, T, device=X.device, dtype=torch.float32)
    _call("gptst_tmix_bwd", _p(dR), _p(X), _p(G), _p(dOut), _p(Y), _p(dX), _p(dG), B, T, N, C, nbytes=_nb(dR, X, dOut, Y, dX))
    return dX, dG


def tmix_bwd_chain(dR, X, G, dPre, premul=False, dG=None):
    _chk(dR, X, G, dPre, dG)
    B, T, N, C = X.shape
    dX = torch.empty_like(X)
    if dG is None:
        dG = torch.empty(N, T, T, device=X.device, dtype=torch.float32)
    _call("gptst_tmix_bwd_chain", _p(dR), _p(X), _p(G), _p(dPre), int(bool(premul)), _p(dX), _p(dG), B, T, N, C, nbytes=_nb(dR, X, dPre, dX))
    return dX, dG


def tmix_dgraph(dR, X, out=None):
    _chk(dR, X, out)
    B, T, N, C = X.shape
    dG = out if out is not None else torch.empty(N, T, T, device=X.device, dtype=torch.float32)
    _call("gptst_tmix_dgraph", _p(dR), _p(X), _p(dG), B, T, N, C, nbytes=_nb(dR, X, dG))
    return dG


FORCE_CAP_BIG = False


def cap_fits_lds(N, C, HS):
    return (not FORCE_CAP_BIG) and bool(_C.lib().value("gptst_cap_fits_lds", N, C, HS))


def _lds_or_stream(lds_call, stream_call):
    if FORCE_CAP_BIG:
        return stream_call()
    try:
        return lds_call()
    except _C.GptstError as e:
        if e.code != _C.ESHAPE:
            raise
        return stream_call()


def _capbig_linear(X, Wp, bp):
    B, T, N, C = X.shape
    return apply(X.reshape(-1, C), Wp, MODE_SHARED, B * T, N, bias=bp, transw=True)


def _capbig_type1(cs, P, S, BT, HS, N, C, reduce_nodes=None):
    _call("gptst_capbig_type1", _p(cs), _p(P), _p(S), BT, HS, N, C)
    if reduce_nodes is not None:
        reduce_nodes(S)


def _cap_route_fwd_big(X, Wp, bp, dadj, HS, R, reduce_nodes=None):
    B, T, N, C = X.shape
    BT, dev = B * T, X.device
    P = _capbig_linear(X, Wp, bp)
    _call("gptst_capbig_squash_rows", _p(P), BT * N, C)
    f = dict(device=dev, dtype=torch.float32)
    cs, c = torch.empty(BT, HS, N, **f), torch.empty(BT, HS, N, **f)
    S, V0, V, s = (torch.empty(BT, HS, C, **f) for _ in range(4))
    bl = torch.zeros(BT, HS, N, **f)
    _call("gptst_capbig_softmax", None, _p(dadj), _p(cs), BT, HS, N, 0, 1)
    _capbig_type1(cs, P, S, BT, HS, N, C, reduce_nodes)
    _call("gptst_capbig_post", _p(S), None, _p(V0), BT * HS, C, 1)
    for r in range(R):
        if r > 0:
            _call("gptst_capbig_type2", _p(V), _p(P), _p(bl), BT, HS, N, C)
        _call("gptst_capbig_softmax", _p(bl), None, _p(cs), BT, HS, N, 1, 0)
        _capbig_type1(cs, P, S, BT, HS, N, C, reduce_nodes)
        _call("gptst_capbig_post", _p(S), _p(V0), _p(V), BT * HS, C, 2)
    if R > 0:
        _call("gptst_capbig_type2", _p(V), _p(P), _p(bl), BT, HS, N, C)
    _call("gptst_capbig_softmax", _p(bl), _p(dadj), _p(c), BT, HS, N, 1, 1)
    _capbig_type1(c, P, S, BT, HS, N, C, reduce_nodes)
    _call("gptst_capbig_post", _p(S), None, _p(s), BT * HS, C, 0)
    return c, s


CAP_FLOW = True


def capflow_ok(HS, C):
    return CAP_FLOW and bool(_C.lib().value("gptst_capflow_supported", HS, C))


def _capflow_post(part, nparts, prow, V0, Vout, mode, BT, HS, C, reduce_nodes):
    if reduce_nodes is not None:
        full = torch.empty(BT, prow, C, device=part.device, dtype=torch.float32)
        _call("gptst_capflow_post", _p(part), nparts, prow, None, _p(full), 3, BT, HS, C)
        reduce_nodes(full)
        part, nparts = full, 1
    _call("gptst_capflow_post", _p(part), nparts, prow, _p(V0), _p(Vout), mode, BT, HS, C)


def _cap_route_fwd_flow(X, Wp, bp, dadj, HS, R, reduce_nodes=None):
    B, T, N, C = X.shape
    BT, dev = B * T, X.device
    f = dict(device=dev, dtype=torch.float32)
    Y = _capbig_linear(X, Wp, bp)
    P = torch.empty_like(Y)
    npart = _C.lib().value("gptst_capflow_nparts", N)
    part = torch.empty(BT, npart, HS + 1, C, **f)
    c = torch.empty(BT, HS, N, **f)
    V0, V, s = (torch.empty(BT, HS, C, **f) for _ in range(3))
    _call("gptst_capflow_squash", _p(Y), _p(dadj), _p(P), _p(part), BT, HS, N, C)
    _capflow_post(part, npart, HS + 1, V0, V if R > 0 else None, 0, BT, HS, C, reduce_nodes)
    bl = None
    for r in range(1, R):
        bl2 = torch.empty(BT, HS, N, **f)
        _call("gptst_capflow_route", _p(P), _p(V), _p(bl), _p(bl2), None, None, None, _p(part), BT, HS, N, C)
        bl = bl2
        _capflow_post(part, npart, HS, V0, V, 1, BT, HS, C, reduce_nodes)
    _call("gptst_capflow_route", _p(P), _p(V) if R > 0 else None, _p(bl), None, _p(dadj), None, _p(c), _p(part), BT, HS, N, C)
    _capflow_post(part, npart, HS, None, s, 2, BT, HS, C, reduce_nodes)
    return c, s, Y


def cap_route_fwd(X, Wp, bp, dadj, HS, R, reduce_nodes=None, want_Y=False):
    _chk(X, Wp, bp, dadj)
    B, T, N, C = X.shape

    def stream():
        if capflow_ok(HS, C):
            return _cap_route_fwd_flow(X, Wp, bp, dadj, HS, R, reduce_nodes)
        return _cap_route_fwd_big(X, Wp, bp, dadj, HS, R, reduce_nodes) + (None,)

    def lds():
        c = torch.empty(B * T, HS, N, device=X.device, dtype=torch.float32)
        s = torch.empty(B * T, HS, C, device=X.device, dtype=torch.float32)
        _call("gptst_cap_route_fwd", _p(X), _p(Wp), _p(bp), _p(dadj), _p(c), _p(s), B * T, N, C, HS, R, nbytes=_nb(X, Wp, bp, dadj, c, s))
        return c, s, None
    out = stream() if reduce_nodes is not None else _lds_or_stream(lds, stream)
    return out if want_Y else out[:2]


def cap_cross_fwd(s, dyn, tmpl, B, T, HS, HT):
    _chk(s, dyn, tmpl)
    C = s.shape[-1]
    v = torch.empty_like(s)
    Ht = torch.empty(B, HT, C, device=s.device, dtype=torch.float32)
    Rt = torch.empty_like(s)
    _call("gptst_cap_cross_fwd", _p(s), _p(dyn), _p(tmpl), _p(v), _p(Ht), _p(Rt), B, T, C, HS, HT)
    return v, Ht, Rt


def cap_cross_rec_fwd(s, dyn, tmpl, c, B, T, N, HS, HT):
    _chk(s, dyn, tmpl, c)
    C = s.shape[-1]
    if C != 64 or FORCE_CAP_BIG:
        return None
    v, Rt = torch.empty_like(s), torch.empty_like(s)
    Ht = torch.empty(B, HT, C, device=s.device, dtype=torch.float32)
    rec = torch.empty(B * T * N, C, device=s.device, dtype=torch.float32)
    try:
        _call("gptst_cap_cross_rec_fwd", _p(s), _p(dyn), _p(tmpl), _p(c), _p(v), _p(Ht), _p(Rt), _p(rec), B, T, N, C, HS, HT,
              nbytes=_nb(s, dyn, c, v, Rt, rec))
    except _C.GptstError as e:
        if e.code != _C.ESHAPE:
            raise
        return None
    return v, Ht, Rt, rec


def cap_cross_bwd(dv, s, Rt, Ht, dyn, tmpl, B, T, HS, HT):
    _chk(dv, s, Rt, Ht, dyn, tmpl)
    C = s.shape[-1]
    dS = torch.empty_like(s)
    ddyn = torch.empty_like(dyn)
    nws = _C.lib().value("gptst_cap_cross_ws_floats", B, T, C, HS, HT)
    ws = torch.empty(nws, device=s.device, dtype=torch.float32) if nws else None
    _call("gptst_cap_cross_bwd", _p(dv), _p(s), _p(Rt), _p(Ht), _p(dyn), _p(tmpl), _p(dS), _p(ddyn), _p(ws), B, T, C, HS, HT)
    return dS, ddyn


def cap_rec_fwd(c, v, N, C):
    _chk(c, v)
    BT, HS = c.shape[0], c.shape[1]
    rec = torch.empty(BT * N, C, device=c.device, dtype=torch.float32)

    def stream():
        if capflow_ok(HS, C):
            return _call("gptst_capflow_rec_fwd", _p(c), _p(v), _p(rec), BT, HS, N, C)
        return _call("gptst_capbig_rec_fwd", _p(c), _p(v), _p(rec), BT, HS, N, C)
    _lds_or_stream(lambda: _call("gptst_cap_rec_fwd", _p(c), _p(v), _p(rec), BT, N, C, HS, nbytes=_nb(c, v, rec)), stream)
    return rec


def cap_rec_bwd(drec, c, v, reduce_nodes=None):
    _chk(drec, c, v)
    BT, HS, N = c.shape
    C = v.shape[-1]
    dc1 = torch.empty_like(c)
    dv = torch.empty_like(v)

    def stream():
        if capflow_ok(HS, C):
            npart = _C.lib().value("gptst_capflow_nparts", N)
            part = torch.empty(BT, npart, HS, C, device=c.device, dtype=torch.float32)
            _call("gptst_capflow_route", _p(drec), _p(v), None, _p(dc1), None, _p(c), None, _p(part), BT, HS, N, C)
            _capflow_post(part, npart, HS, None, dv, 2, BT, HS, C, reduce_nodes)
            return
        _call("gptst_capbig_rec_bwd_dc", _p(drec), _p(v), _p(dc1), BT, HS, N, C)
        _capbig_type1(c, drec, dv, BT, HS, N, C, reduce_nodes)
    if reduce_nodes is not None or (HS > 16 and capflow_ok(HS, C)):
        stream()
    else:
        _lds_or_stream(lambda: _call("gptst_cap_rec_bwd", _p(drec), _p(c), _p(v), _p(dc1), _p(dv), BT, N, C, HS, nbytes=_nb(drec, c, v, dc1, dv)),
                       stream)
    return dc1, dv


def cap_route_bwd(X, Wp, bp, c, dc1, dS, Y=None):
    _chk(X, Wp, bp, c, dc1, dS)
    B, T, N, C = X.shape
    HS = c.shape[1]
    dY = torch.empty(B * T * N, C, device=X.device, dtype=torch.float32)
    dlogit = torch.empty_like(c)

    def stream():
        Yv = Y if Y is not None else _capbig_linear(X, Wp, bp)
        name = "gptst_capflow_route_bwd" if capflow_ok(HS, C) else "gptst_capbig_route_bwd_rows"
        _call(name, _p(Yv), _p(c), _p(dc1), _p(dS), _p(dY), _p(dlogit), B * T, HS, N, C)
    if Y is not None:
        stream()
    else:
        _lds_or_stream(lambda: _call("gptst_cap_route_bwd", _p(X), _p(Wp), _p(bp), _p(c), _p(dc1), _p(dS), _p(dY), _p(dlogit), B * T, N, C, HS,
                                     nbytes=_nb(X, Wp, bp, c, dc1, dS, dY, dlogit)), stream)
    return dY, dlogit


def cap_cross_route_bwd(X, Wp, bp, c, dc1, dv, s, Rt, Ht, dyn, tmpl, B, T, HS, HT, flags=None):
    _chk(X, Wp, bp, c, dc1, dv, s, Rt, Ht, dyn, tmpl)
    N, C = X.shape[2], X.shape[3]
    if C != 64 or FORCE_CAP_BIG:
        return None
    dY = torch.empty(B * T * N, C, device=X.device, dtype=torch.float32)
    dlogit = torch.empty_like(c)
    ddyn = torch.empty_like(dyn)
    try:
        dS_ws = torch.empty(B * T, HS, C, device=X.device, dtype=torch.float32) if flags is not None else None
        _call("gptst_cap_cross_route_bwd", _p(X), _p(Wp), _p(bp), _p(c), _p(dc1), _p(dv), _p(s), _p(Rt), _p(Ht), _p(dyn), _p(tmpl), _p(dY),
              _p(dlogit), _p(ddyn), _p(dS_ws), _p(flags), B, T, N, C, HS, HT, nbytes=_nb(X, Wp, bp, c, dc1, dv, s, Rt, dY, dlogit))
    except _C.GptstError as e:
        if e.code != _C.ESHAPE:
            raise
        return None
    return dY, dlogit, ddyn


def cap_cross_route_lin_bwd(X, Wp, bp, c, dc1, dv, s, Rt, Ht, dyn, tmpl, dPre, out, premul, B, T, HS, HT, flags=None, jobs=None, nsplit=None):
    _chk(X, Wp, bp, c, dc1, dv, s, Rt, Ht, dyn, tmpl, dPre, out)
    N, C = X.shape[2], X.shape[3]
    if C != 64 or FORCE_CAP_BIG:
        return None
    dev = X.device
    if nsplit is None:
        nsplit = _C.lib().value("gptst_cap_split_units", B * T, N, C, HS)
    rows = B * T + nsplit
    dX = torch.empty(B * T * N, C, device=dev, dtype=torch.float32)
    dWp = torch.empty(rows, C * C, device=dev, dtype=torch.float32)
    dbp = torch.empty(rows, C, device=dev, dtype=torch.float32)
    dlogit = torch.empty_like(c)
    ddyn = torch.empty_like(dyn)
    try:
        dS_ws = torch.empty(B * T, HS, C, device=dev, dtype=torch.float32) if flags is not None else None
        js = jobs.jobs if jobs is not None and not jobs.post and all(j[0] in (PoolJobs.BWD_POOL, PoolJobs.BWD_EMB) for j in jobs.jobs) else []
        col = lambda i: [j[i] for j in js]
        _call("gptst_cap_cross_route_lin_bwd_split", _p(X), _p(Wp), _p(bp), _p(c), _p(dc1), _p(dv), _p(s), _p(Rt), _p(Ht), _p(dyn), _p(tmpl),
              _p(dPre), _p(out), int(bool(premul)), _p(dX), _p(dWp), _p(dbp), _p(dlogit), _p(ddyn), _p(dS_ws), _p(flags), B, T, N, C, HS, HT, nsplit,
              len(js), _ints(col(0)), _ptrs0(col(1)), _ptrs0(col(2)), _ptrs0(col(3)), _ptrs0(col(4)), _ints(col(5)), _ints(col(6)), _ints(col(7)),
              _ints(col(8)), _ints(col(9)), nbytes=_nb(X, Wp, bp, c, dc1, dv, s, Rt, dPre, out, dX, dWp, dlogit))
        if js:
            jobs.jobs = []
    except _C.GptstError as e:
        if e.code != _C.ESHAPE:
            raise
        return None
    return dX, dWp, dbp, dlogit, ddyn


_MASK_WS = {}


def _mask_ws(dev):
    if dev not in _MASK_WS:
        _MASK_WS[dev] = torch.zeros(_C.lib().value("gptst_mask_ws_bytes") // 4, dtype=torch.int32, device=dev)
    return _MASK_WS[dev]


def mask_ws_floats():
    return _C.lib().value("gptst_mask_ws_bytes") // 4


def _fused_jobs(jobs, u24):
    if jobs is None or not (jobs.jobs or jobs.post):
        return None
    if not u24 or jobs.post or any(j[0] not in (PoolJobs.FWD, PoolJobs.GRAM) for j in jobs.jobs):
        jobs.launch()
        return None
    odd = [j for j in jobs.jobs if j[0] == PoolJobs.FWD and j[7] % 4]
    if odd:
        rest = [j for j in jobs.jobs if not (j[0] == PoolJobs.FWD and j[7] % 4)]
        jobs.jobs = odd
        jobs.launch()
        jobs.jobs = rest
        if not rest:
            return None
    js, jobs.jobs = jobs.jobs, []
    col = lambda i: [j[i] for j in js]
    return js, (len(js), _ints(col(0)), _ptrs0(col(1)), _ptrs0(col(3)), _ptrs0(col(4)), _ints(col(5)), _ints(col(6)), _ints(col(7)))


def mask_random(noise, k, ws=None, u24=False, jobs=None):
    _chk(noise)
    mask = torch.empty_like(noise)
    fj = _fused_jobs(jobs, u24)
    if fj is not None:
        _call("gptst_mask_u24_fwd_jobs", 0, None, None, None, None, _p(noise), None, 0, noise.numel(), 0, 1, int(k), None, None, _p(mask),
              _p(ws if ws is not None else _mask_ws(noise.device)), int(ws is not None), *fj[1])
        return mask
    _call("gptst_mask_random_u24" if u24 else "gptst_mask_random", _p(noise), noise.numel(), int(k), _p(mask),
          _p(ws if ws is not None else _mask_ws(noise.device)), int(ws is not None))
    return mask


MASK_SMALL = 1 << 13


def mask_labels(prob):
    _chk(prob)
    rows, HS = prob.shape
    label = torch.empty(rows, device=prob.device, dtype=torch.int32)
    counts = torch.empty(HS, device=prob.device, dtype=torch.int32)
    _call("gptst_mask_labels", _p(prob), rows, HS, _p(label), _p(counts))
    return label, counts


def mask_adaptive(label, counts, list_c, nums, noise_a, noise_r, ada_all, base, ws=None, u24=False, jobs=None):
    M, HS = label.numel(), list_c.numel()
    m_ada = torch.empty(M, device=label.device, dtype=torch.float32)
    m_rnd = torch.empty_like(m_ada)
    mask = torch.empty(M * base, device=label.device, dtype=torch.float32)
    fj = _fused_jobs(jobs, u24)
    if fj is not None:
        _call("gptst_mask_u24_fwd_jobs", 1, _p(label), _p(counts), _p(list_c), _p(nums), _p(noise_a), _p(noise_r), int(ada_all), M, HS, base, 0,
              _p(m_ada), _p(m_rnd), _p(mask), _p(ws if ws is not None else _mask_ws(label.device)), int(ws is not None), *fj[1])
        return m_ada, m_rnd, mask
    _call("gptst_mask_adaptive_u24" if u24 else "gptst_mask_adaptive", _p(label), _p(counts), _p(list_c), _p(nums), _p(noise_a), _p(noise_r),
          int(ada_all), M, HS, base, _p(m_ada), _p(m_rnd), _p(mask), _p(ws if ws is not None else _mask_ws(label.device)), int(ws is not None))
    return m_ada, m_rnd, mask


def lin_in(a, lda, J, W, b, C, mask=None, fill=0.0, wlayout=0, rows=None):
    rows = rows if rows is not None else a.numel() // lda
    Y = torch.empty(rows, C, device=a.device, dtype=torch.float32)
    _call("gptst_lin_in", _p(a), lda, _p(mask), float(fill), _p(W), wlayout, _p(b), _p(Y), rows, J, C, nbytes=_nb(a, mask, W, b, Y))
    return Y


def rowdot(X, W, b, softmax=False, want_label=False):
    rows, C = X.shape
    J = W.shape[0]
    Z = torch.empty(rows, J, device=X.device, dtype=torch.float32)
    label = torch.empty(rows, device=X.device, dtype=torch.int32) if want_label else None
    _call("gptst_rowdot", _p(X), _p(W), _p(b), _p(Z), rows, J, C, int(softmax), _p(label), nbytes=_nb(X, W, b, Z))
    return (Z, label) if want_label else Z


def rowouter(a, lda, J, X, out, olayout, csum=None, asum=None, mask=None, fill=0.0):
    rows, C = X.shape
    ws = torch.empty(_C.lib().value("gptst_rowouter_ws_floats", J, C), device=X.device, dtype=torch.float32)
    _call("gptst_rowouter", _p(a), lda, _p(mask), float(fill), _p(X), _p(out), olayout, _p(csum), _p(asum), _p(ws), rows, J, C,
          nbytes=_nb(a, mask, X, out))


def rowouter_part(a, lda, J, X, mask=None, fill=0.0, want_asum=False):
    rows, C = X.shape
    nparts = _C.lib().value("gptst_rowouter_nparts", rows)
    part = torch.empty(nparts, J * C + C + J, device=X.device, dtype=torch.float32)
    _call("gptst_rowouter_part", _p(a), lda, _p(mask), float(fill), _p(X), _p(part), int(want_asum), rows, J, C, nbytes=_nb(X))
    return part


def timefeat_fwd(params, tidx, rows, K):
    E = params[1].numel()
    out = torch.empty(rows, E, device=tidx.device, dtype=torch.float32)
    _call("gptst_timefeat_fwd", *[_p(t) for t in params], _p(tidx), _p(out), rows, K, E)
    return out


def timefeat_bwd(params, grads, tidx, dout, rows, K):
    E = params[1].numel()
    _call("gptst_timefeat_bwd", *[_p(t) for t in params], *[_p(t) for t in grads], _p(tidx), _p(dout), rows, K, E)


def timefeat_jobs_fwd(jobs, tidx):
    outs = [torch.empty(rows, params[1].numel(), device=tidx.device, dtype=torch.float32) for params, rows, K in jobs]
    _call("gptst_timefeat_jobs", len(jobs), 0, _ptrs([t for params, _, _ in jobs for t in params]), None, _p(tidx), _ptrs(outs),
          _ints([r for _, r, _ in jobs]), _ints([k for _, _, k in jobs]), _ints([params[1].numel() for params, _, _ in jobs]))
    return outs


def timefeat_jobs_bwd(jobs, tidx):
    if not jobs:
        return
    _call("gptst_timefeat_jobs", len(jobs), 1, _ptrs([t for j in jobs for t in j[0]]), _ptrs([t for j in jobs for t in j[1]]), _p(tidx),
          _ptrs([j[2] for j in jobs]), _ints([j[3] for j in jobs]), _ints([j[4] for j in jobs]), _ints([j[0][1].numel() for j in jobs]))


def mae_fwd(out, src, lda, mask, sigma, mu, thresh, rows, J, stats):
    _call("gptst_mae_fwd", _p(out), _p(src), lda, _p(mask), float(sigma), float(mu), float(thresh), rows, J, _p(stats))


def mae_bwd(out, src, lda, mask, sigma, mu, thresh, rows, J, stats, normalize=True):
    dOut = torch.empty_like(out)
    _call("gptst_mae_bwd", _p(out), _p(src), lda, _p(mask), float(sigma), float(mu), float(thresh), rows, J, _p(stats), int(normalize),
          _p(dOut))
    return dOut


def kl(prob, c, N, w, stats, want_grad=True):
    rows, HS = prob.shape
    dlogit = torch.empty_like(prob) if want_grad else None
    _call("gptst_kl", _p(prob), _p(c), rows, N, HS, float(w), _p(dlogit), _p(stats))
    return dlogit


TAIL_MAXJ = 16


def set_deterministic(on):
    _C.lib().call("gptst_set_deterministic", int(bool(on)))



def tail_parts(rows):
    return _C.lib().value("gptst_tail_parts", rows)


def tail_sws(rows, device):
    return torch.zeros(_C.lib().value("gptst_tail_parts", rows), 4, device=device, dtype=torch.float32)


def tail_mae(dec, W, b, src, lda, mask, sigma, mu, thresh, sws, premul=False):
    rows, C = dec.shape
    J = W.shape[0]
    nparts = _C.lib().value("gptst_tail_parts", rows)
    out = torch.empty(rows, J, device=dec.device, dtype=torch.float32)
    d_dec = torch.empty_like(dec)
    part = torch.empty(nparts, J * C + J, device=dec.device, dtype=torch.float32)
    _call("gptst_tail_mae", _p(dec), _p(W), _p(b), _p(src), lda, _p(mask), float(sigma), float(mu), float(thresh), _p(out), _p(d_dec),
          _p(part), _p(sws), int(premul), rows, J, C, nbytes=_nb(dec, d_dec))
    return out, d_dec, part


def tail_kl(h2, W3, prob, c, N, w, sws, premul=False):
    rows, C = h2.shape
    HS = W3.shape[0]
    nparts = _C.lib().value("gptst_tail_parts", rows)
    d_h2 = torch.empty_like(h2)
    part = torch.empty(nparts, HS * C + HS, device=h2.device, dtype=torch.float32)
    _call("gptst_tail_kl", _p(h2), _p(W3), _p(prob), _p(c), float(w), _p(d_h2), _p(part), _p(sws), int(premul), rows, N, HS, C, nbytes=_nb(h2, d_h2))
    return d_h2, part


def stats_fold(sws, stats):
    _call("gptst_stats_fold", _p(sws), sws.shape[0], _p(stats))


_ADAM_WS = {}


def step_begin(z0, z1, src, base, noise=None, rng=None):
    B, T, N, lda = src.shape
    tidx = torch.empty(B, T, 2, device=src.device, dtype=torch.float32)
    _call("gptst_step_begin", _p(z0), z0.numel(), _p(z1), z1.numel() if z1 is not None else 0, _p(src), _p(tidx), B * T, N, lda, base,
          _p(noise), noise.numel() if noise is not None else 0, _p(rng))
    return tidx


def clip_adam(p, g, m, v, nA, nB, hyper, stats, ws=None, stats_out=None, sws=None):
    if ws is None:
        if p.device not in _ADAM_WS:
            _ADAM_WS[p.device] = torch.empty(_C.lib().value("gptst_clip_adam_ws_floats"), device=p.device, dtype=torch.float32)
        ws = _ADAM_WS[p.device]
    _call("gptst_clip_adam", _p(p), _p(g), _p(m), _p(v), int(nA), int(nB), _p(hyper), _p(stats), _p(ws), _p(stats_out), _p(sws),
          sws.shape[0] if sws is not None else 0)


def metrics_new(T, N, device):
    return torch.zeros(T, 5, device=device, dtype=torch.float64), torch.zeros(T, N, 6, device=device, dtype=torch.float64)


def metrics_accum(out, src, lda, vis, sigma, mu, mae_thresh, mape_thresh, B, T, N, D, sums_t, sums_tn):
    _call("gptst_metrics_accum", _p(out), _p(src), lda, _p(vis), float(sigma), float(mu), int(mae_thresh is not None),
          float(mae_thresh if mae_thresh is not None else 0.0), float(mape_thresh), B, T, N, D, _p(sums_t), _p(sums_tn))


def metrics_report(sums_t, sums_tn):
    st, sn = sums_t.cpu(), sums_tn.cpu()

    def rows_of(a, m):
        mae, rmse, mape = a[..., 1] / a[..., 0], torch.sqrt(a[..., 2] / a[..., 0]), a[..., 4] / a[..., 3]
        K, sp, sy, spp, syy, spy = (m[..., k] for k in range(6))
        pm, ym = sp / K, sy / K
        cov = spy / K - pm * ym
        pvar, yvar = (spp - K * pm * pm) / (K - 1), (syy - K * ym * ym) / (K - 1)
        c = cov / torch.sqrt(pvar.clamp_min(0) * yvar.clamp_min(0))
        ok = yvar > 1e-9 * (syy / K).clamp_min(1e-30)
        corr = torch.stack([c[i][ok[i]].mean() for i in range(c.shape[0])]) if c.dim() == 2 else c[ok].mean()
        return torch.stack([mae, rmse, mape, corr], -1)

    per_t = rows_of(st, sn)
    avg = rows_of(st.sum(0), sn.sum(0))
    return torch.cat([per_t, avg[None]], 0)
```

gpt-st_amd/step.py:

```python
import contextlib
import math
import os
import random

import torch

from . import engine, ops

DEFER_GEN = os.environ.get("GPTST_DEFER_GEN", "1") == "1"
U24 = os.environ.get("GPTST_MASK_U24", "1") == "1"


class PretrainStep:
    RING = 8
    DETERMINISTIC_MODE = True

    def __init__(self, model, args, scaler_mean, scaler_std, batch_size, use_graph=True, dp=None, seed=0, global_mask=True,
                 deterministic=None):
        self.model, self.args = model, args
        self.mean, self.std = float(scaler_mean), float(scaler_std)
        self.B, self.T, self.N = batch_size, args.lag, args.num_nodes
        self.C, self.base, self.HS = args.hidden_dim, args.input_base_dim, args.HS
        self.dims = (self.B, self.T, self.N, self.C)
        self.dev = model.flat.device
        assert self.dev.type == "cuda", "PretrainStep needs the model on an MI355X (no CPU fallback)"
        self.use_graph, self.dp = use_graph, dp
        self.deterministic = self.DETERMINISTIC_MODE and ((os.environ.get("GPTST_DETERMINISTIC", "0") == "1") if deterministic is None else bool(deterministic))
        n = model.flat.numel()
        self.gbuf = torch.zeros(n + 8, device=self.dev)
        self.gflat, self.stats = self.gbuf[:n], self.gbuf[n:]
        self.g = model.views_of(self.gflat)
        self.m, self.v = torch.zeros(n, device=self.dev), torch.zeros(n, device=self.dev)
        M = self.B * self.T * self.N
        self.src = torch.zeros(self.B, self.T, self.N, self.base + 2, device=self.dev)
        self.noise = torch.zeros(M * self.base, device=self.dev)
        self.noise_ar = torch.zeros(2 * M, device=self.dev)
        self.noise_a, self.noise_r = self.noise_ar[:M], self.noise_ar[M:]
        self.hc = torch.zeros(16 + self.HS + 4, dtype=torch.int32, device=self.dev)
        self.hyper = self.hc[:16].view(torch.float32)
        self.ctrl = self.hc[16:16 + self.HS + 2]
        self.rng_words = self.hc[16 + self.HS + 2:]
        self.noise_seed = 1234567 + seed
        self._ring = [self._views(torch.zeros(16 + self.HS + 4, dtype=torch.int32).pin_memory()) for _ in range(self.RING)]
        self._ring_i = 0
        self.phase_kl = False
        self._gK, self._g_last, self._group_failed = 0, None, False
        self.stats_out = torch.zeros(8, device=self.dev)
        self.mask_buf = torch.ones(M * self.base, device=self.dev)
        self.last_mask = None
        self.force_mask = False
        self.tA = self.tB = 0
        self.lr = args.lr_init
        self.rng = random.Random(seed)
        self.graphs = {}
        self._g_graphs = {}
        self._g_fallback = None
        self._graph_comm_failed = False
        self._ctx_keep = []
        self._sws = None
        self.inject_noise = False
        self.global_count_scale = False
        self.node_reduce = None
        self.join_enc_dec = True
        self.safe_mode = False
        self.lost_steps = 0
        self.lost_batches = 0
        self._unseen = []
        self._last_call = None
        self._g_list_cs = None
        self.arena = engine.ZeroArena(self.dev)
        self.fused_tails = os.environ.get("GPTST_FUSED_TAILS", "1") == "1" and engine.fused_tails_ok(model.param_views(), self.C, self.base, self.HS)
        self.W = dp.world if dp is not None else 1
        self.gmask = bool(global_mask) and dp is not None and self.W > 1
        if self.gmask:
            Mg = M * self.W
            self.noise_g = torch.zeros(Mg * self.base, device=self.dev)
            self.noise_ar_g = torch.zeros(2 * Mg, device=self.dev)
            self.noise_a_g, self.noise_r_g = self.noise_ar_g[:Mg], self.noise_ar_g[Mg:]
            self.label_l = torch.zeros(M, dtype=torch.int32, device=self.dev)
            self.label_g = torch.zeros(Mg, dtype=torch.int32, device=self.dev)
        self.always_guide = os.environ.get("GPTST_ALWAYS_GUIDE", "0") == "1"
        self.dp_overlap = (os.environ.get("GPTST_DP_OVERLAP", "0") != "0" and dp is not None and getattr(dp, "capturable", False)
                           and (self.W > 1 or os.environ.get("GPTST_FORCE_DP", "0") == "1"))
        self.dec_lo, self.dec_hi = self._decoder_bucket(model)
        self.rank_weight = 1.0
        self.fork_side = torch.cuda.Stream() if self.dp_overlap else None

    def _needs_exchange(self, phase):
        return self.gmask and phase == 1 and not self.force_mask

    @staticmethod
    def _decoder_bucket(model):
        offs = [(o, model.state_dict()[k].numel()) for k, o in model._offs.items() if k.startswith("decoder.") and o < model.nA]
        lo = min(o for o, _ in offs)
        hi = max(o + (n + 3) // 4 * 4 for o, n in offs)
        assert hi == model.nA and all(o >= lo for o, _ in offs), (lo, hi, model.nA)
        assert not any(lo <= o < hi for k, o in model._offs.items() if not k.startswith("decoder.")), "decoder bucket is not contiguous"
        return lo, hi

    def _allreduce(self, sl):
        if self.rank_weight != 1.0:
            assert not self.use_graph, "a rank weight is baked into a captured graph: tail rounds use eager steppers"
            lost = self.stats[5:6].clone()
            sl.mul_(self.rank_weight)
            self.stats[5:6].copy_(lost)
        self.dp.allreduce_(sl)

    def _bucket_ready(self, k):
        if k == 0:
            self._allreduce(self.gbuf[self.dec_lo:self.dec_hi])
            self._dec_reduced = True

    def _dp_in_graph(self):
        return self.dp is not None and getattr(self.dp, "capturable", False) and not self._graph_comm_failed

    def _part1(self, phase):
        p, dims, base = self.model.param_views(), self.dims, self.base
        engine.CTX.ARENA, engine.CTX.NODE_REDUCE = self.arena, self.node_reduce
        src = self.src
        noise = None if self.inject_noise or self.force_mask else self._noise_buffer(phase)
        tidx = ops.step_begin(self.gbuf, self.arena.begin(zero=False), src, base, noise=noise, rng=self.rng_words)
        need_guide = self._need_guide(phase)
        gen = engine.gen_all(p, tidx, dims, guide=need_guide, defer=DEFER_GEN)
        red = engine.Reductions()
        red.no_carry = self.deterministic
        self._dec_reduced = False
        if self.dp_overlap and self._dp_in_graph():
            red.on_bucket = self._bucket_ready
            red.bucket_inline, red.fork_side = True, self.fork_side
        lowrank = self.fused_tails and engine.chain_ok(dims)
        prob, sv_g = engine.guide_fwd(p, src, tidx, dims, base, gen=gen["guide"], lowrank_in=lowrank) if need_guide else (None, None)
        if self._needs_exchange(phase):
            self.label_l.copy_(sv_g[4])
        return dict(tidx=tidx, gen=gen, red=red, prob=prob, sv_g=sv_g)

    def _part2(self, phase, ctx):
        if not self.safe_mode:
            return self._part2_impl(phase, ctx)
        with engine.no_handoffs():
            return self._part2_impl(phase, ctx)

    def _part2_impl(self, phase, ctx):
        mdl, p, g, dims, base = self.model, self.model.param_views(), self.g, self.dims, self.base
        a = self.args
        src, tidx, gen, red, prob, sv_g = self.src, ctx["tidx"], ctx["gen"], ctx["red"], ctx["prob"], ctx["sv_g"]
        engine.CTX.ARENA, engine.CTX.NODE_REDUCE = self.arena, self.node_reduce
        pend = gen.pop("pending", None)
        mask = self._make_mask(phase, prob, sv_g[4] if sv_g is not None else None, pend)
        if pend is not None:
            pend.launch()
        self.last_mask = mask
        fused = self.fused_tails
        kl, sws = None, None
        if phase == 1 and self._carry_kl(sv_g):
            sws = self._tail_sws()
            kl = engine.KlCarry(p, sv_g, prob, src, dims, 0.1, sws)
        fw = engine.autoencoder_fwd(p, src, mask, dims, base, mdl.num_route, mdl.scaler_zeros, gen=gen, tidx=tidx,
                                    lowrank_in=fused and engine.chain_ok(dims), kl=kl, head=not fused, join=self.join_enc_dec)
        if fused and sws is None:
            sws = self._tail_sws()
        engine.step_bwd(p, g, src, mask, tidx, fw, prob, sv_g, dims, base, mdl.scaler_zeros, red, (self.std, self.mean, a.mape_thresh),
                        self.stats, sws=sws, with_kl=phase == 1, kl=kl)
        self._fold_stats(sws)
        red.flush(tidx)
        engine.CTX.ARENA = engine.CTX.NODE_REDUCE = None
        self._after_backward(phase)

    def _noise_buffer(self, phase):
        if self.gmask:
            return self.noise_g if phase == 0 else self.noise_ar_g
        return self.noise if phase == 0 else self.noise_ar

    def _need_guide(self, phase):
        return phase == 1 or self.always_guide

    def _make_mask(self, phase, prob, label, pend):
        a, base, M = self.args, self.base, self.B * self.T * self.N
        if self.gmask:
            return self._global_mask(phase, jobs=pend)
        if self.force_mask:
            return self.mask_buf
        if phase == 0:
            return ops.mask_random(self.noise, int(M * base * a.mask_ratio), ws=self._mask_ws(), u24=U24, jobs=pend)
        return ops.mask_adaptive(label, None, self.ctrl[:self.HS], self.ctrl[self.HS:], self.noise_a, self.noise_r,
                                 a.ada_type == "all", base, ws=self._mask_ws(), u24=U24, jobs=pend)[2]

    def _fold_stats(self, sws):
        if sws is None:
            return
        if self.dp is None:
            self._sws = sws
        else:
            ops.stats_fold(sws, self.stats)

    def _after_backward(self, phase):
        if self.dp is None:
            self._optim()
        elif self._dp_in_graph():
            if self._dec_reduced:
                self._allreduce(self.gbuf[:self.dec_lo])
                self._allreduce(self.gbuf[self.dec_hi:])
            else:
                self._allreduce(self.gbuf)
            self._optim()

    def _tail_sws(self):
        return self.arena.zeros(ops.tail_parts(self.B * self.T * self.N), 4)

    def _carry_kl(self, sv_g):
        return (self.fused_tails and self.dp is None and not self.global_count_scale and not self.deterministic and not self.safe_mode
                and not self.always_guide and engine.CTX.NODE_REDUCE is None and engine.kl_carry_ok(self.dims, self.HS, sv_g))

    def _mask_ws(self):
        return self.arena.zeros(ops.mask_ws_floats())

    def _global_mask(self, phase, jobs=None):
        a, base, M = self.args, self.base, self.B * self.T * self.N
        Mg = M * self.W
        if self.force_mask:
            return self.mask_buf
        if phase == 0:
            mask_g = ops.mask_random(self.noise_g, int(Mg * base * a.mask_ratio), ws=self._mask_ws(), u24=U24, jobs=jobs)
        else:
            mask_g = ops.mask_adaptive(self.label_g, None, self.ctrl[:self.HS], self.ctrl[self.HS:], self.noise_a_g,
                                       self.noise_r_g, a.ada_type == "all", base, ws=self._mask_ws(), u24=U24, jobs=jobs)[2]
        self.last_mask_global = mask_g
        return self.dp.rows_of(mask_g, M * base)

    def _exchange_labels(self):
        self.dp.gather_labels(self.label_l, out=self.label_g)

    def _optim(self):
        sws, self._sws = self._sws, None
        ops.clip_adam(self.model.flat, self.gflat, self.m, self.v, self.model.nA, self.model.nB, self.hyper, self.stats,
                      stats_out=self.stats_out, sws=sws)

    @contextlib.contextmanager
    def _launch_mode(self):
        if self.DETERMINISTIC_MODE:
            ops.set_deterministic(self.deterministic)
        try:
            yield
        finally:
            if self.DETERMINISTIC_MODE:
                ops.set_deterministic(False)
            engine.CTX.ARENA = engine.CTX.NODE_REDUCE = None

    def _enqueue(self, phase):
        ctx = self._part1(phase)
        if self._needs_exchange(phase):
            self._exchange_labels()
        self._part2(phase, ctx)

    def _body(self, phase):
        with self._launch_mode():
            self._enqueue(phase)

    def _views(self, hc):
        HS = self.HS
        n = hc.numpy()
        return dict(hc=hc, hyper=n[:16].view("float32"), ctrl=n[16:16 + HS + 2], rng=n[16 + HS + 2:], ev=None)

    def _slot(self):
        sl = self._ring[self._ring_i]
        self._ring_i = (self._ring_i + 1) % self.RING
        if sl["ev"] is not None:
            sl["ev"].synchronize()
        return sl

    def _host_prepare(self, phase, epoch, list_c):
        sl = self._slot()
        self._fill(sl, phase, epoch, list_c)
        self.hc.copy_(sl["hc"], non_blocking=True)
        if sl["ev"] is None:
            sl["ev"] = torch.cuda.Event()
        sl["ev"].record()

    def _fill(self, sl, phase, epoch, list_c):
        a = self.args
        self.tA += 1
        if phase == 1:
            self.tB += 1
        self.phase_kl = phase == 1
        b1, b2 = 0.9, 0.999
        tA, tB = self.tA, self.tB
        sl["hyper"][11:13] = (1 - b1, 1 - b2)
        sl["hyper"][:11] = (self.lr / (1 - b1 ** tA), math.sqrt(1 - b2 ** tA),
                            self.lr / (1 - b1 ** tB) if tB else 0.0, math.sqrt(1 - b2 ** tB) if tB else 1.0,
                            b1, b2, 1e-8, float(a.max_grad_norm) if a.grad_norm else 0.0, 1.0 if phase == 1 else 0.0,
                            1.0,
                            1.0)
        sl["rng"][:2] = (self.noise_seed & 0x7FFFFFFF, tA & 0x7FFFFFFF)
        if phase == 1:
            if list_c is None:
                list_c = list(range(self.HS))
                self.rng.shuffle(list_c)
            ada, rnd = self.model.adaptive_counts(self.B * self.T * self.N * (self.W if self.gmask else 1), epoch)
            ada, rnd = self._budgets(ada, rnd, epoch)
            sl["ctrl"][:] = [int(v) for v in list_c] + [int(ada), int(rnd)]
        self._filled_list_c = [int(v) for v in list_c] if phase == 1 else None

    def _budgets(self, ada, rnd, epoch):
        return ada, rnd

    def step(self, source, epoch, noise=None, noise_a=None, noise_r=None, list_c=None, forced_mask=None):
        phase = 0 if epoch <= self.args.change_epoch else 1
        self._g_last = None
        self._g_fallback = None
        if source is not self.src:
            self.src.copy_(source, non_blocking=True)
        inject = noise is not None or noise_a is not None
        if inject:
            n0, na, nr = (self.noise_g, self.noise_a_g, self.noise_r_g) if self.gmask else (self.noise, self.noise_a, self.noise_r)
            if phase == 0:
                n0.copy_(noise.reshape(-1), non_blocking=True)
            else:
                na.copy_(noise_a.reshape(-1), non_blocking=True)
                nr.copy_(noise_r.reshape(-1), non_blocking=True)
        if forced_mask is not None:
            self.mask_buf.copy_(forced_mask.reshape(-1), non_blocking=True)
        self._host_prepare(phase, epoch, list_c)
        self._last_call = (epoch, self._filled_list_c, self.rank_weight) if not inject and forced_mask is None else None
        self._unseen.append(phase)
        if len(self._unseen) > 4096:
            del self._unseen[:2048]
        key = (phase, inject, forced_mask is not None)
        if not self.use_graph:
            self.inject_noise, self.force_mask = inject, forced_mask is not None
            self._body(phase)
        else:
            if key not in self.graphs:
                self._capture(key)
            g1, g2 = self.graphs[key]
            g1.replay()
            if g2 is not None:
                self._exchange_labels()
                g2.replay()
        if self.dp is not None and not self._dp_in_graph():
            self._allreduce(self.gbuf)
            self._optim()

    def _capture(self, key):
        try:
            return self._capture_impl(key)
        except Exception as e:
            if not self._dp_in_graph():
                raise
            import sys
            print("gpt-st_amd: capturing the step with its collectives failed (%s: %s) -> collectives between graph replays"
                  % (type(e).__name__, str(e).splitlines()[0][:200]), file=sys.stderr)
            self._graph_comm_failed = True
            self.graphs.clear()
            self._g_graphs.clear()
            torch.cuda.synchronize()
            return self._capture_impl(key)

    def _capture_impl(self, key):
        phase, inject, forced = key
        self.inject_noise, self.force_mask = inject, forced
        keep = (self.model.flat.clone(), self.m.clone(), self.v.clone())
        engine.warm_up(lambda: self._body(phase))
        try:
            with self._launch_mode():
                g1 = torch.cuda.CUDAGraph()
                if self._needs_exchange(phase) and not self._dp_in_graph():
                    with torch.cuda.graph(g1, capture_error_mode="thread_local"):
                        ctx = self._part1(phase)
                    g2 = torch.cuda.CUDAGraph()
                    with torch.cuda.graph(g2, pool=g1.pool(), capture_error_mode="thread_local"):
                        self._part2(phase, ctx)
                    self._ctx_keep.append(ctx)
                else:
                    g2 = None
                    with torch.cuda.graph(g1, capture_error_mode="thread_local"):
                        self._enqueue(phase)
        finally:
            self.model.flat.copy_(keep[0]); self.m.copy_(keep[1]); self.v.copy_(keep[2])
            torch.cuda.synchronize()
        self.graphs[key] = (g1, g2)

    def group_ok(self, epoch):
        phase = 0 if epoch <= self.args.change_epoch else 1
        if self._group_failed:
            return False
        return self.use_graph and (self.dp is None or self._dp_in_graph()) and not (self._needs_exchange(phase) and not self._dp_in_graph())

    def _group_init(self, K):
        if self._gK == K:
            return
        W = self.hc.numel()
        self._gK = K
        self._g_hc = torch.zeros(K, W, dtype=torch.int32, device=self.dev)
        self._g_src = [torch.zeros_like(self.src) for _ in range(K)]
        self._g_stats = torch.zeros(K, 8, device=self.dev)
        self._g_ring = []
        for _ in range(self.RING):
            hc = torch.zeros(K, W, dtype=torch.int32).pin_memory()
            self._g_ring.append(dict(hc=hc, rows=[self._views(hc[j]) for j in range(K)], ev=None))
        self._g_ring_i = 0
        self._g_graphs = {}

    def group_sources(self, K):
        self._group_init(K)
        return self._g_src

    def _sub(self, j):
        HS = self.HS
        r = self._g_hc[j]
        self.src, self.stats_out = self._g_src[j], self._g_stats[j]
        self.hyper, self.ctrl, self.rng_words = r[:16].view(torch.float32), r[16:16 + HS + 2], r[16 + HS + 2:]

    def step_group(self, sources, epoch, list_cs=None):
        K = len(sources)
        if K == 1 or not self.group_ok(epoch):
            snaps = []
            for j, src in enumerate(sources):
                self.step(src, epoch, list_c=None if list_cs is None else list_cs[j])
                snaps.append((self.stats_out.clone(), bool(self.tB and self.phase_kl), src, self._filled_list_c, epoch))
            self._g_last = None
            self._g_fallback = snaps
            return
        phase = 0 if epoch <= self.args.change_epoch else 1
        self._group_init(K)
        for j, src in enumerate(sources):
            if src is not self._g_src[j]:
                self._g_src[j].copy_(src, non_blocking=True)
        if phase not in self._g_graphs:
            keep = (self.src, self.stats_out, self.hyper, self.ctrl, self.rng_words)
            try:
                self._capture_group(phase, K, epoch)
            except Exception as e:
                import sys
                print("gpt-st_amd: capturing %d steps in one graph failed (%s: %s) -> one replay per step"
                      % (K, type(e).__name__, str(e).splitlines()[0][:200] if str(e) else ""), file=sys.stderr)
                self._group_failed = True
                torch.cuda.synchronize()
                torch.cuda.empty_cache()
            finally:
                self.src, self.stats_out, self.hyper, self.ctrl, self.rng_words = keep
            if self.dp is not None and getattr(self.dp, "world", 1) > 1 and hasattr(self.dp, "max_over_ranks"):
                if self.dp.max_over_ranks(1.0 if self._group_failed else 0.0) > 0 and not self._group_failed:
                    self._group_failed = True
                    self._g_graphs.pop(phase, None)
            if self._group_failed:
                return self.step_group(sources, epoch, list_cs)
        sl = self._g_ring[self._g_ring_i]
        self._g_ring_i = (self._g_ring_i + 1) % self.RING
        if sl["ev"] is not None:
            sl["ev"].synchronize()
        self._g_list_cs = []
        for j in range(K):
            self._fill(sl["rows"][j], phase, epoch, None if list_cs is None else list_cs[j])
            self._g_list_cs.append(self._filled_list_c)
        self._g_epoch = epoch
        self._g_hc.copy_(sl["hc"], non_blocking=True)
        if sl["ev"] is None:
            sl["ev"] = torch.cuda.Event()
        sl["ev"].record()
        self._g_graphs[phase].replay()
        self._g_last = (K, phase)

    def _capture_group(self, phase, K, epoch):
        self.inject_noise, self.force_mask = False, False
        keep = (self.model.flat.clone(), self.m.clone(), self.v.clone())
        st = (self.tA, self.tB, self.phase_kl, self.rng.getstate())
        for j in range(K):
            self._fill(self._g_ring[0]["rows"][j], phase, epoch, None)
        self._g_hc.copy_(self._g_ring[0]["hc"])
        torch.cuda.synchronize()
        self.tA, self.tB, self.phase_kl = st[:3]
        self.rng.setstate(st[3])
        base = torch.cuda.memory_allocated()
        torch.cuda.reset_peak_memory_stats()
        subs = iter(range(K))
        engine.warm_up(lambda: (self._sub(next(subs)), self._body(phase)))
        per_step = torch.cuda.max_memory_allocated() - base
        total = torch.cuda.get_device_properties(self.dev).total_memory
        if self.dp is not None and getattr(self.dp, "world", 1) > 1 and hasattr(self.dp, "max_over_ranks"):
            per_step = int(self.dp.max_over_ranks(per_step))
            total = -int(self.dp.max_over_ranks(-total))
        if per_step * K > 0.25 * total:
            self.model.flat.copy_(keep[0]); self.m.copy_(keep[1]); self.v.copy_(keep[2])
            torch.cuda.synchronize()
            raise RuntimeError("a group of %d steps would need ~%.0f GB of activations (device: %.0f GB)" % (K, per_step * K / 2**30, total / 2**30))
        try:
            with self._launch_mode():
                g = torch.cuda.CUDAGraph()
                with torch.cuda.graph(g, capture_error_mode="thread_local"):
                    for j in range(K):
                        self._sub(j)
                        self._enqueue(phase)
        finally:
            self.model.flat.copy_(keep[0]); self.m.copy_(keep[1]); self.v.copy_(keep[2])
            torch.cuda.synchronize()
        self._g_graphs[phase] = g

    def losses_group(self):
        if self._g_last is None:
            if self._g_fallback:
                snaps, self._g_fallback = self._g_fallback, None
                rows = [(st.cpu(), kl) for st, kl, _, _, _ in snaps]
                out = [self._stats_row(st, kl) for st, kl in rows]
                lost = [j for j, (st, _) in enumerate(rows) if float(st[5]) > 0]
                del self._unseen[:]
                if lost:
                    j0 = lost[0]
                    self._enter_safe_mode(len(snaps) - j0, sum(1 for _, kl, _, _, _ in snaps[j0:] if kl))
                    for j in range(j0, len(snaps)):
                        _, kl, src, lc, ep = snaps[j]
                        self.step(src, ep, list_c=lc)
                        out[j] = self._stats_row(self.stats_out.cpu(), kl)
                    del self._unseen[:]
                return out
            return [self.losses()]
        K, phase = self._g_last
        st = self._g_stats.cpu()
        del self._unseen[:]
        rerun = {}
        if float(st[:, 5].max()) > 0:
            j0 = int((st[:, 5] > 0).float().argmax())
            extra = max(0, int(st[K - 1, 6]) - (K - j0))
            if extra:
                import sys
                self.lost_batches += extra
                print("gpt-st_amd: %d step(s) of earlier groups were skipped too and cannot be repeated (their batches are gone): the optimiser counters "
                      "were taken back, the batches were not trained on" % extra, file=sys.stderr)
            self._enter_safe_mode(K - j0 + extra, (K - j0 + extra) if phase == 1 else 0)
            srcs, lcs, epoch = [t.clone() for t in self._g_src[j0:]], self._g_list_cs[j0:], self._g_epoch
            for j, (src, lc) in enumerate(zip(srcs, lcs)):
                self.step(src, epoch, list_c=lc)
                rerun[j0 + j] = self._stats_row(self.stats_out.cpu(), phase == 1)
            del self._unseen[:]
            self._g_last = (K, phase)
        out = []
        for j in range(K):
            out.append(rerun[j] if j in rerun else self._stats_row(st[j], phase == 1))
        return out

    @staticmethod
    def _stats_row(st, kl):
        lf = float(st[0] / max(float(st[1]), 1.0))
        ls = float(st[2]) * 0.1 if kl else 0.0
        return (lf + ls, lf, ls)

    def _enter_safe_mode(self, nsteps, nkl):
        import sys
        from . import _C
        torch.cuda.synchronize()
        print("gpt-st_amd: an in-launch hand-off expired (the GPU was shared?) — %d skipped step(s) are re-run without hand-off launches; "
              "this stepper stays in that mode" % nsteps, file=sys.stderr)
        self.tA -= nsteps
        self.tB -= nkl
        self.lost_steps += nsteps
        self.safe_mode = True
        self.graphs.clear()
        self._g_graphs.clear()
        _C.lib().call("gptst_handoff_reset")

    def losses(self):
        if self._g_last is not None:
            return self.losses_group()[-1]
        st = self.stats_out.cpu()
        unseen, self._unseen = self._unseen, []
        if float(st[5]) > 0:
            if self._last_call is None:
                raise RuntimeError("an in-launch hand-off expired in a step with injected mask inputs: call _enter_safe_mode() and repeat the step")
            nskip = max(1, min(int(st[6]), len(unseen))) if unseen else 1
            epoch, lc, weight = self._last_call
            self._enter_safe_mode(nskip, sum(unseen[-nskip:]) if unseen else (1 if self.phase_kl else 0))
            if nskip > 1:
                import sys
                self.lost_batches += nskip - 1
                print("gpt-st_amd: %d step(s) enqueued before the last one were skipped with it and cannot be repeated (their batches are gone): "
                      "the optimiser counters were taken back, the batches were not trained on" % (nskip - 1), file=sys.stderr)
            keep_w, self.rank_weight = self.rank_weight, weight
            try:
                self.step(self.src, epoch, list_c=lc)
            finally:
                self.rank_weight = keep_w
            st = self.stats_out.cpu()
            del self._unseen[:]
        return self._stats_row(st, bool(self.tB and self.phase_kl))
```

include/gptst_hip.h:

```cpp
#ifndef GPTST_HIP_H
#define GPTST_HIP_H
#include <stdint.h>

#ifdef __cplusplus
extern "C" {
#endif
#if defined(__GNUC__)
#pragma GCC visibility push(default)
#endif

#define GPTST_ABI_VERSION 16
int gptst_abi_version(void);
int gptst_set_deterministic(int on);
int gptst_handoff_timeouts(int* out);
int gptst_handoff_reset(void);
int gptst_mask_cooperative(int on);
int gptst_mask_cooperative_state(void);
int gptst_set_handoff_guard(int on);

int gptst_poolgen_fwd(const float* emb, const float* pool, float* out, int cols, const float* pool2, float* out2,
                      int cols2, int R, int K, void* stream);
int gptst_poolgen_bwd_pool(const float* emb, const float* dW, float* dpool, int cols, const float* dW2, float* dpool2,
                           int cols2, int R, int nsplit, int K, void* stream);
int gptst_poolgen_bwd_emb(const float* dW, const float* pool, int cols, const float* dW2, const float* pool2, int cols2,
                          float* demb, int R, int nsplit, int K, void* stream);

int gptst_poolgen_fwd_multi(const float* emb, int nprob, const void* pools, const void* outs, const int* cols, int R, int K,
                            void* stream);
int gptst_poolgen_bwd_pool_multi(const float* emb, int nprob, const void* dWs, const void* dpools, const int* cols, const int* nsplit,
                                 int R, int K, void* stream);
int gptst_poolgen_bwd_emb_multi(int nprob, const void* dWs, const void* pools, const int* cols, const int* nsplit, float* demb, int R,
                                int K, void* stream);

int gptst_pool_jobs(int njobs, const int* kind, const void* const* emb, const void* const* x, const void* const* pool,
                    const void* const* out, const int* R, const int* K, const int* cols, const int* nsplit, const int* ldx, void* stream);
int gptst_pool_jobs_gram_rows(int K, int cols);

int gptst_apply_nsplit(int mode, int BT, int N, int C);
int gptst_apply(const float* A, const float* A2, const float* W, int w_per_group, int transw, const float* bias,
                const float* resid, const float* resid2, float* out, float* colsum, int mode, int pro, int epi, int BT,
                int N, int C, void* stream);
int gptst_wgrad_nsplit(int mode, int BT, int N, int C);
int gptst_wgrad(const float* A, const float* D, const float* D2, float* dW, int mode, int pro, int BT, int N, int C,
                void* stream);
int gptst_wgrad_colsum(const float* A, const float* D, const float* D2, float* dW, int mode, int pro, int which, int BT, int N, int C,
                       void* stream);

int gptst_apply_wgrad_nsplit(int mode, int BT, int N);
int gptst_apply_wgrad(const float* dOut, const float* Y, const float* S, const float* W, float* dS, float* dW, float* colsum, int premul,
                      int mode, int BT, int N, int C, void* stream);

int gptst_linear_bwd_nsplit(int rows);
int gptst_linear_bwd(const float* dY, const float* X, const float* Wp, const float* dOut, const float* out, float* dX, float* dWp, float* dbp,
                     int premul, int rows, int C, void* stream);

int gptst_gram_fwd(const float* A, float* G, int N, int Hm, void* stream);
int gptst_gram_bwd(const float* A, const float* dG, float* dA, int L, int N, int Hm, int nsplit, void* stream);
int gptst_tmix(const float* X, const float* G, const float* dOut, const float* Y, float* out, int B, int T, int N, int C,
               void* stream);
int gptst_tmix_dgraph(const float* dR, const float* X, float* dG, int B, int T, int N, int C, void* stream);
int gptst_tmix_bwd(const float* dR, const float* X, const float* G, const float* dOut, const float* Y, float* dX, float* dG, int B, int T,
                   int N, int C, void* stream);
int gptst_tmix_bwd_chain(const float* dR, const float* X, const float* G, const float* dPre, int premul, float* dX, float* dG, int B, int T,
                         int N, int C, void* stream);

int gptst_hypertem_fwd(const float* X, const float* G, const float* Wbt, const float* bbt, float* R_out, float* out, int B, int T,
                       int N, int C, void* stream);
int gptst_hypertem_chain_fwd(const float* X, int nstage, const void* Gs, const void* Wbts, const void* bbts, const void* Rs, const void* outs,
                             int B, int T, int N, int C, void* stream);
int gptst_hypertem_chain_fwd_kl(const float* X, int nstage, const void* Gs, const void* Wbts, const void* bbts, const void* Rs, const void* outs,
                                int B, int T, int N, int C, int stage, const void* ops, int v0, int v1, int HS, int lda, float w, void* stream);
int gptst_kl_guest_blocks(int stage, int B, int T, int N);

int gptst_encin_ht1_fwd(const float* src, int lda, const float* mask, float fill, const float* w, const float* bi, const float* G,
                        const float* Wbt, const float* bbt, float* out, float* ab, float* wv, int B, int T, int N, int C, void* stream);
int gptst_encin_ht1_bwd(const float* dPre, const float* src, int lda, const float* mask, float fill, const float* w, const float* bi,
                        const float* Wbt, const float* ab, const float* wv, float* dWb, float* dG, float* dinp, int B, int T, int N, int C,
                        void* stream);

int gptst_guide_in_fwd(const float* src, int lda, const float* w1, const float* b1, const float* Wn, const float* bn, float* h1, int BT, int N,
                       int C, void* stream);
int gptst_guide_in_bwd(const float* dPre, const float* src, int lda, const float* w1, const float* b1, const float* Wn, float* dWb, float* dinp,
                       int BT, int N, int C, void* stream);
int gptst_guide_uc_floats(int N, int C);
int gptst_guide_head_fwd(const float* src, int lda, const float* w1, const float* b1, const float* Wn, const float* bn, const float* Wbt,
                         const float* bbt, const float* W3, const float* b3, float* uc, float* h1, float* h2, float* prob, int* label,
                         int BT, int N, int C, int J, void* stream);

int gptst_hypertem_ntiles(int N);
int gptst_hypertem_bwd(const float* dOut, const float* Y, const float* X, const float* G, const float* Wbt, float* dX, float* dbias,
                       float* dG, int premul, int B, int T, int N, int C, void* stream);
int gptst_hypertem_bwd_wgrad(const float* dOut, const float* Y, const float* X, const float* G, const float* Wbt, const float* R, float* dX,
                             float* dG, float* dWb, int premul, int B, int T, int N, int C, void* stream);
int gptst_hypertem_bwd_pair(const float* dOut1, const float* X1, const float* G1, const float* Wbt1, const float* R1, const float* X0,
                            const float* G0, const float* Wbt0, const float* R0, float* dXmid, float* dX0, float* dG1, float* dG0,
                            float* dWb1, float* dWb0, void* cnt, int B, int T, int N, int C, void* stream);

int gptst_cap_route_fwd(const float* X, const float* Wp, const float* bp, const float* dadj, float* c_out, float* s_out, int BT, int N,
                        int C, int HS, int R, void* stream);
int gptst_cap_cross_fwd(const float* s, const float* dyn, const float* tmpl, float* v, float* Ht, float* Rt, int B, int T, int C,
                        int HS, int HT, void* stream);
int gptst_cap_cross_ws_floats(int B, int T, int C, int HS, int HT);
int gptst_cap_cross_bwd(const float* dv, const float* s, const float* Rt, const float* Ht, const float* dyn, const float* tmpl,
                        float* dS, float* ddyn, float* ws, int B, int T, int C, int HS, int HT, void* stream);
int gptst_cap_rec_fwd(const float* c, const float* v, float* rec, int BT, int N, int C, int HS, void* stream);
int gptst_cap_cross_rec_fwd(const float* s, const float* dyn, const float* tmpl, const float* c, float* v, float* Ht, float* Rt, float* rec,
                            int B, int T, int N, int C, int HS, int HT, void* stream);
int gptst_cap_rec_bwd(const float* drec, const float* c, const float* v, float* dc1, float* dv, int BT, int N, int C, int HS,
                      void* stream);
int gptst_cap_route_bwd(const float* X, const float* Wp, const float* bp, const float* c, const float* dc1, const float* dS,
                        float* dY, float* dlogit, int BT, int N, int C, int HS, void* stream);
int gptst_cap_cross_route_bwd(const float* X, const float* Wp, const float* bp, const float* c, const float* dc1, const float* dv,
                              const float* s, const float* Rt, const float* Ht, const float* dyn, const float* tmpl, float* dY,
                              float* dlogit, float* ddyn, float* dS_ws, void* flags, int B, int T, int N, int C, int HS, int HT, void* stream);
int gptst_cap_cross_route_lin_bwd(const float* X, const float* Wp, const float* bp, const float* c, const float* dc1, const float* dv,
                                  const float* s, const float* Rt, const float* Ht, const float* dyn, const float* tmpl,
                                  const float* dPre, const float* out, int premul, float* dX, float* dWp, float* dbp, float* dlogit,
                                  float* ddyn, float* dS_ws, void* flags, int B, int T, int N, int C, int HS, int HT, void* stream);
int gptst_cap_route_roles_ok(int B, int T, int N, int C, int HS, int HT);
int gptst_cap_cross_route_lin_bwd_jobs(const float* X, const float* Wp, const float* bp, const float* c, const float* dc1, const float* dv,
                                       const float* s, const float* Rt, const float* Ht, const float* dyn, const float* tmpl,
                                       const float* dPre, const float* out, int premul, float* dX, float* dWp, float* dbp, float* dlogit,
                                       float* ddyn, float* dS_ws, void* flags, int B, int T, int N, int C, int HS, int HT,
                                       int njobs, const int* jkind, const void* const* jemb, const void* const* jx, const void* const* jpool,
                                       const void* const* jout, const int* jR, const int* jK, const int* jcols, const int* jnsplit, const int* jldx,
                                       void* stream);
int gptst_cap_split_units(int BT, int N, int C, int HS);
int gptst_cap_cross_route_lin_bwd_split(const float* X, const float* Wp, const float* bp, const float* c, const float* dc1, const float* dv,
                                        const float* s, const float* Rt, const float* Ht, const float* dyn, const float* tmpl,
                                        const float* dPre, const float* out, int premul, float* dX, float* dWp, float* dbp, float* dlogit,
                                        float* ddyn, float* dS_ws, void* flags, int B, int T, int N, int C, int HS, int HT, int nsplit,
                                        int njobs, const int* jkind, const void* const* jemb, const void* const* jx, const void* const* jpool,
                                        const void* const* jout, const int* jR, const int* jK, const int* jcols, const int* jnsplit, const int* jldx,
                                        void* stream);

int gptst_cap_fits_lds(int N, int C, int HS);
int gptst_capbig_squash_rows(float* Y, long rows, int C, void* stream);
int gptst_capbig_softmax(const float* bl, const float* l0, float* cs, int BT, int HS, int N, int use_bl, int use_l0, void* stream);
int gptst_capbig_type1(const float* cs, const float* P, float* S, int BT, int HS, int N, int C, void* stream);
int gptst_capbig_post(const float* S, const float* V0, float* out, long rows, int C, int post, void* stream);
int gptst_capbig_type2(const float* V, const float* P, float* bl, int BT, int HS, int N, int C, void* stream);
int gptst_capbig_rec_fwd(const float* c, const float* v, float* rec, int BT, int HS, int N, int C, void* stream);
int gptst_capbig_rec_bwd_dc(const float* drec, const float* v, float* dc1, int BT, int HS, int N, int C, void* stream);
int gptst_capbig_route_bwd_rows(const float* Y, const float* c, const float* dc1, const float* dS, float* dY, float* dlogit, int BT,
                                int HS, int N, int C, void* stream);

int gptst_capflow_supported(int HS, int C);
int gptst_capflow_nparts(int N);
int gptst_capflow_squash(const float* Y, const float* dadj, float* P, float* part, int BT, int HS, int N, int C, void* stream);
int gptst_capflow_route(const float* rows, const float* V, const float* bl_in, float* bl_out, const float* l0, const float* c_in,
                        float* c_out, float* part, int BT, int HS, int N, int C, void* stream);
int gptst_capflow_post(const float* part, int nparts, int prow, float* V0, float* Vout, int mode, int BT, int HS, int C, void* stream);
int gptst_capflow_rec_fwd(const float* c, const float* v, float* rec, int BT, int HS, int N, int C, void* stream);
int gptst_capflow_route_bwd(const float* Y, const float* c, const float* dc1, const float* dS, float* dY, float* dlogit, int BT,
                            int HS, int N, int C, void* stream);

int gptst_metrics_accum(const float* out, const float* src, int lda, const float* vis, float sigma, float mu, int has_mae_thresh,
                        float mae_thresh, float mape_thresh, int B, int T, int N, int D, double* sums_t, double* sums_tn, void* stream);

int gptst_mask_ws_bytes(void);
int gptst_mask_random(const float* noise, int M, int k, float* mask, void* ws, int ws_zeroed, void* stream);
int gptst_mask_labels(const float* prob, int rows, int HS, int* label, int* counts, void* stream);
int gptst_mask_adaptive(const int* label, const int* counts, const int* list_c, const int* nums, const float* noise_a,
                        const float* noise_r, int ada_all, int M, int HS, int base, float* m_ada, float* m_rnd, float* mask,
                        void* ws, int ws_zeroed, void* stream);

int gptst_mask_random_u24(const float* noise, int M, int k, float* mask, void* ws, int ws_zeroed, void* stream);
int gptst_mask_adaptive_u24(const int* label, const int* counts, const int* list_c, const int* nums, const float* noise_a, const float* noise_r,
                            int ada_all, int M, int HS, int base, float* m_ada, float* m_rnd, float* mask, void* ws, int ws_zeroed, void* stream);
int gptst_mask_u24_fwd_jobs(int adaptive, const int* label, const int* counts, const int* list_c, const int* nums, const float* noise_a,
                            const float* noise_r, int ada_all, int M, int HS, int base, int k, float* m_ada, float* m_rnd, float* mask, void* ws,
                            int ws_zeroed, int njobs, const int* kind, const void* const* emb, const void* const* pool, const void* const* out,
                            const int* R, const int* K, const int* cols, void* stream);

int gptst_lin_in(const float* a, int lda, const float* mask, float fill, const float* W, int wlayout, const float* b, float* Y,
                 int rows, int J, int C, void* stream);
int gptst_rowdot(const float* X, const float* W, const float* b, float* Z, int rows, int J, int C, int do_softmax, int* label,
                 void* stream);
int gptst_fusion_gate_fwd(const float* F, const float* src, int lda, int base, const float* Ws, const float* bs, const float* Wh,
                          const float* bh, const float* Wo, const float* bo, const float* Wt, const float* bt, float* out, float* z,
                          int rows, int C, void* stream);
int gptst_fusion_gate_bwd(const float* dOut, const float* F, const float* z, const float* src, int lda, int base, const float* Wo,
                          const float* Wt, const float* bt, float* dpre, float* dxd, float* Hm, float* xt, int rows, int C, void* stream);
int gptst_rowouter_ws_floats(int J, int C);
int gptst_rowouter_nparts(int rows);
int gptst_rowouter_part(const float* a, int lda, const float* mask, float fill, const float* X, float* part, int want_asum, int rows,
                        int J, int C, void* stream);
int gptst_rowouter(const float* a, int lda, const float* mask, float fill, const float* X, float* out, int olayout, float* csum,
                   float* asum, float* ws, int rows, int J, int C, void* stream);

int gptst_timefeat_fwd(const float* wd, const float* bd, const float* ww, const float* bw, const float* w1, const float* b1,
                       const float* w2, const float* b2, const float* w3, const float* b3, const float* tidx, float* out, int rows,
                       int K, int E, void* stream);
int gptst_timefeat_bwd(const float* wd, const float* bd, const float* ww, const float* bw, const float* w1, const float* b1,
                       const float* w2, const float* b2, const float* w3, const float* b3, float* gwd, float* gbd, float* gww,
                       float* gbw, float* gw1, float* gb1, float* gw2, float* gb2, float* gw3, float* gb3, const float* tidx,
                       const float* dout, int rows, int K, int E, void* stream);

int gptst_tail_parts(int rows);
int gptst_tail_mae(const float* dec, const float* W, const float* b, const float* src, int lda, const float* mask, float sigma, float mu,
                   float thresh, float* out, float* d_dec, float* part, float* sws, int premul, int rows, int J, int C, void* stream);
int gptst_tail_kl(const float* h2, const float* W3, const float* prob, const float* c, float w, float* d_h2, float* part, float* sws,
                  int premul, int rows, int N, int HS, int C, void* stream);
int gptst_stats_fold(const float* sws, int rows, float* stats, void* stream);

int gptst_timefeat_jobs(int njobs, int bwd, const void* const* params, const void* const* grads, const float* tidx,
                        const void* const* io, const int* rows, const int* K, const int* E, void* stream);

int gptst_step_begin(float* z0, long n0, float* z1, long n1, const float* src, float* tidx, int BT, int N, int lda, int base,
                     float* noise, long n_noise, const int* rng, void* stream);

int gptst_mae_fwd(const float* out, const float* src, int lda, const float* mask, float sigma, float mu, float thresh, int rows,
                  int J, float* stats, void* stream);
int gptst_mae_bwd(const float* out, const float* src, int lda, const float* mask, float sigma, float mu, float thresh, int rows,
                  int J, const float* stats, int normalize, float* dOut, void* stream);
int gptst_kl(const float* prob, const float* c, int rows, int N, int HS, float w, float* dlogit, float* stats, void* stream);
int gptst_clip_adam_ws_floats(void);
int gptst_clip_adam(float* p, const float* g, float* m, float* v, long nA, long nB, const float* hyper, float* stats, float* ws,
                    float* stats_out, const float* sws, int sws_rows, void* stream);

int gptst_layer_bytes(int kind, int B, int T, int N, int C, int d, int Hm, int ds, int HS, int HT, int base, long* saved_bytes,
                      long* scratch_bytes);
int gptst_hypertem_layer_fwd(const float* x, const float* node_emb, const float* time_eb, const float* adj, const float* wpool,
                             const float* bpool, float* out, void* saved, long saved_bytes, int B, int T, int N, int C, int d, int Hm,
                             void* stream);
int gptst_hypertem_layer_bwd(const float* dout, const float* x, const float* out, const float* node_emb, const float* time_eb,
                             const float* adj, const float* wpool, const float* bpool, const void* saved, long saved_bytes, float* dx,
                             float* d_node_emb, float* d_time_eb, float* d_adj, float* d_wpool, float* d_bpool, void* scratch,
                             long scratch_bytes, int B, int T, int N, int C, int d, int Hm, void* stream);
int gptst_cap_layer_fwd(const float* x, const float* node_emb_spg, const float* time_eb_spg, const float* teb, const float* ln_p_w,
                        const float* ln_p_b, const float* adj, const float* t_adj, const float* wspa, const float* bspa,
                        const float* mask_template, float* out, float* c_out, float* dyn_out, void* saved, long saved_bytes, int B, int T,
                        int N, int C, int d, int ds, int HS, int HT, int R, void* stream);
int gptst_cap_layer_bwd(const float* dout, const float* x, const float* out, const float* c, const float* dyn, const float* node_emb_spg,
                        const float* time_eb_spg, const float* teb, const float* ln_p_w, const float* ln_p_b, const float* adj,
                        const float* t_adj, const float* wspa, const float* bspa, const float* mask_template, const void* saved,
                        long saved_bytes, float* dx, float* d_node_emb_spg, float* d_time_eb_spg, float* d_teb, float* d_ln_p_w,
                        float* d_ln_p_b, float* d_adj, float* d_t_adj, float* d_wspa, float* d_bspa, void* scratch, long scratch_bytes, int B,
                        int T, int N, int C, int d, int ds, int HS, int HT, void* stream);
int gptst_mlprl_layer_fwd(const float* a, int lda, const float* time_eb, const float* node_emb, const float* ln1_w, const float* ln1_b,
                          const float* wpool_spa, const float* bpool_spa, const float* wpool_tem, const float* bpool_tem, const float* ln3_w,
                          const float* ln3_b, float* logits, void* saved, long saved_bytes, int B, int T, int N, int C, int d, int base,
                          int HS, void* stream);
int gptst_mlprl_layer_bwd(const float* dlogits, const float* a, int lda, const float* time_eb, const float* node_emb, const float* ln1_w,
                          const float* wpool_spa, const float* bpool_spa, const float* wpool_tem, const float* bpool_tem, const float* ln3_w,
                          const void* saved, long saved_bytes, float* d_time_eb, float* d_node_emb, float* d_ln1_w, float* d_ln1_b,
                          float* d_wpool_spa, float* d_bpool_spa, float* d_wpool_tem, float* d_bpool_tem, float* d_ln3_w, float* d_ln3_b,
                          void* scratch, long scratch_bytes, int B, int T, int N, int C, int d, int base, int HS, void* stream);

int gptst_comm_available(void);
int gptst_comm_unique_id(void* out128);
int gptst_comm_init(int rank, int world, const void* unique_id, void** comm_out);
int gptst_allreduce_f32(void* comm, float* buf, long n, void* stream);
int gptst_allgather_i32(void* comm, const int* send, int* recv, long n, void* stream);
int gptst_comm_count(void* comm, int* out);
int gptst_comm_destroy(void* comm);

#if defined(__GNUC__)
#pragma GCC visibility pop
#endif
#ifdef __cplusplus
}
#endif
#endif
```

Baseline: 925.4 steps/s.

## Fuse step-begin, time-feature and pool-gen forward into two role-split head kernels

```diff
diff --git a/gpt-st_amd/csrc/guidein.hip b/gpt-st_amd/csrc/guidein.hip
--- a/gpt-st_amd/csrc/guidein.hip
+++ b/gpt-st_amd/csrc/guidein.hip
@@ -1,5 +1,6 @@
 #include "mfma_tile.h"
 #include "kl_guest.h"
+#include "guidein_dev.h"
 
 #define GI_CHUNKS 3
 
@@ -82,28 +83,8 @@
 template <int C>
 __global__ __launch_bounds__(256) void guide_uc_kernel(const float* __restrict__ w1, const float* __restrict__ b1, const float* __restrict__ Wn,
                                                        const float* __restrict__ bn, float* __restrict__ uc) {
-    constexpr int NQ = 256 / C;
-    __shared__ __attribute__((aligned(16))) float part[NQ * 2 * C];
-    const int n = blockIdx.x, tid = threadIdx.x;
-    const int q = tid / C, o = tid % C;
-    const float* W = Wn + (size_t)n * C * C;
-    float au = 0.f, ac = 0.f;
-#pragma unroll 8
-    for (int i = q * (C / NQ); i < (q + 1) * (C / NQ); ++i) {
-        const float x = W[(size_t)i * C + o];
-        au = fmaf(w1[i], x, au);
-        ac = fmaf(b1[i], x, ac);
-    }
-    part[(q * 2 + 0) * C + o] = au;
-    part[(q * 2 + 1) * C + o] = ac;
-    __syncthreads();
-    if (tid < C) {
-        float s0 = 0.f, s1 = 0.f;
-#pragma unroll
-        for (int qq = 0; qq < NQ; ++qq) { s0 += part[(qq * 2 + 0) * C + tid]; s1 += part[(qq * 2 + 1) * C + tid]; }
-        uc[(size_t)n * 2 * C + tid] = s0;
-        uc[(size_t)n * 2 * C + C + tid] = s1 + bn[(size_t)n * C + tid];
-    }
+    __shared__ __attribute__((aligned(16))) float part[GUIDE_UC_LDS(C)];
+    guide_uc_body<C>(w1, b1, Wn, bn, uc, blockIdx.x, part);
 }
 
 #define GH_P 68
@@ -206,6 +187,18 @@
 
 extern "C" int gptst_guide_uc_floats(int N, int C) { return N * 2 * C; }
 
+static int guide_head_rows_launch(const float* src, int lda, const float* uc, const float* Wbt, const float* bbt, const float* W3, const float* b3, float* h1,
+                                  float* h2, float* prob, int* label, int BT, int N, int J, hipStream_t st) {
+    const int ntiles = (N + 15) / 16;
+    int tpw = 1;
+    if (g_apply_tpw > 0) tpw = g_apply_tpw;
+    if (tpw < 1) tpw = 1;
+    const int gy = (ntiles + 4 * tpw - 1) / (4 * tpw);
+    hipLaunchKernelGGL(guide_head_fwd_kernel, dim3(BT, gy), dim3(256), 0, st, src, lda, uc, Wbt, bbt, W3, b3, h1, h2, prob, label, N, J, tpw);
+    GPTST_CHECK_LAUNCH();
+    return GPTST_OK;
+}
+
 extern "C" int gptst_guide_head_fwd(const float* src, int lda, const float* w1, const float* b1, const float* Wn, const float* bn, const float* Wbt,
                                     const float* bbt, const float* W3, const float* b3, float* uc, float* h1, float* h2, float* prob, int* label,
                                     int BT, int N, int C, int J, void* stream) {
@@ -213,12 +206,12 @@
         return GPTST_EARG;
     if (C != 64 || J > 16) return GPTST_ESHAPE;
     hipLaunchKernelGGL((guide_uc_kernel<64>), dim3(N), dim3(256), 0, (hipStream_t)stream, w1, b1, Wn, bn, uc);
-    const int ntiles = (N + 15) / 16;
-    int tpw = 1;
-    if (g_apply_tpw > 0) tpw = g_apply_tpw;
-    if (tpw < 1) tpw = 1;
-    const int gy = (ntiles + 4 * tpw - 1) / (4 * tpw);
-    hipLaunchKernelGGL(guide_head_fwd_kernel, dim3(BT, gy), dim3(256), 0, (hipStream_t)stream, src, lda, uc, Wbt, bbt, W3, b3, h1, h2, prob, label, N, J, tpw);
-    GPTST_CHECK_LAUNCH();
-    return GPTST_OK;
-}
+    return guide_head_rows_launch(src, lda, uc, Wbt, bbt, W3, b3, h1, h2, prob, label, BT, N, J, (hipStream_t)stream);
+}
+
+extern "C" int gptst_guide_head_rows(const float* src, int lda, const float* uc, const float* Wbt, const float* bbt, const float* W3, const float* b3,
+                                     float* h1, float* h2, float* prob, int* label, int BT, int N, int C, int J, void* stream) {
+    if (!src || !uc || !Wbt || !bbt || !W3 || !b3 || !h1 || !h2 || !prob || !label || BT <= 0 || N <= 0 || lda <= 0 || J <= 0) return GPTST_EARG;
+    if (C != 64 || J > 16) return GPTST_ESHAPE;
+    return guide_head_rows_launch(src, lda, uc, Wbt, bbt, W3, b3, h1, h2, prob, label, BT, N, J, (hipStream_t)stream);
+}
diff --git a/gpt-st_amd/csrc/guidein_dev.h b/gpt-st_amd/csrc/guidein_dev.h
--- /dev/null
+++ b/gpt-st_amd/csrc/guidein_dev.h
@@ -0,0 +1,29 @@
+#pragma once
+#include "common.h"
+
+#define GUIDE_UC_LDS(C) ((256 / (C)) * 2 * (C))
+template <int C>
+__device__ __forceinline__ void guide_uc_body(const float* __restrict__ w1, const float* __restrict__ b1, const float* __restrict__ Wn,
+                                              const float* __restrict__ bn, float* __restrict__ uc, int n, float* __restrict__ part) {
+    constexpr int NQ = 256 / C;
+    const int tid = threadIdx.x;
+    const int q = tid / C, o = tid % C;
+    const float* W = Wn + (size_t)n * C * C;
+    float au = 0.f, ac = 0.f;
+#pragma unroll 8
+    for (int i = q * (C / NQ); i < (q + 1) * (C / NQ); ++i) {
+        const float x = W[(size_t)i * C + o];
+        au = fmaf(w1[i], x, au);
+        ac = fmaf(b1[i], x, ac);
+    }
+    part[(q * 2 + 0) * C + o] = au;
+    part[(q * 2 + 1) * C + o] = ac;
+    __syncthreads();
+    if (tid < C) {
+        float s0 = 0.f, s1 = 0.f;
+#pragma unroll
+        for (int qq = 0; qq < NQ; ++qq) { s0 += part[(qq * 2 + 0) * C + tid]; s1 += part[(qq * 2 + 1) * C + tid]; }
+        uc[(size_t)n * 2 * C + tid] = s0;
+        uc[(size_t)n * 2 * C + C + tid] = s1 + bn[(size_t)n * C + tid];
+    }
+}
diff --git a/gpt-st_amd/csrc/stepbegin.hip b/gpt-st_amd/csrc/stepbegin.hip
--- a/gpt-st_amd/csrc/stepbegin.hip
+++ b/gpt-st_amd/csrc/stepbegin.hip
@@ -1,49 +1,17 @@
 #include "common.h"
-
-__device__ __forceinline__ void philox4x32_10(unsigned c0, unsigned c1, unsigned c2, unsigned c3, unsigned k0, unsigned k1, unsigned (&o)[4]) {
-#pragma unroll
-    for (int r = 0; r < 10; ++r) {
-        const unsigned long long p0 = 0xD2511F53ull * c0, p1 = 0xCD9E8D57ull * c2;
-        const unsigned n0 = (unsigned)(p1 >> 32) ^ c1 ^ k0, n1 = (unsigned)p1, n2 = (unsigned)(p0 >> 32) ^ c3 ^ k1, n3 = (unsigned)p0;
-        c0 = n0; c1 = n1; c2 = n2; c3 = n3;
-        k0 += 0x9E3779B9u; k1 += 0xBB67AE85u;
-    }
-    o[0] = c0; o[1] = c1; o[2] = c2; o[3] = c3;
-}
+#include "stepbegin_dev.h"
 
 __global__ __launch_bounds__(256) void step_begin_kernel(float* __restrict__ z0, long n0, float* __restrict__ z1, long n1,
                                                          const float* __restrict__ src, float* __restrict__ tidx, int BT, int N, int lda,
                                                          int base, float* __restrict__ noise, long n_noise, const int* __restrict__ rng) {
-    const long q0 = n0 / 4, q1 = n1 / 4, stride = (long)gridDim.x * 256;
-    for (long i = (long)blockIdx.x * 256 + threadIdx.x; i < q0 + q1; i += stride) {
-        if (i < q0) st4(z0 + 4 * i, f4zero()); else st4(z1 + 4 * (i - q0), f4zero());
-    }
-    if (blockIdx.x == 0) {
-        for (long i = 4 * q0 + threadIdx.x; i < n0; i += 256) z0[i] = 0.f;
-        for (long i = 4 * q1 + threadIdx.x; i < n1; i += 256) z1[i] = 0.f;
-    }
-    if (tidx != nullptr)
-        for (long i = (long)blockIdx.x * 256 + threadIdx.x; i < 2L * BT; i += stride)
-            tidx[i] = src[(size_t)(i / 2) * N * lda + base + (i & 1)];
-    if (noise != nullptr) {
-        const unsigned seed = (unsigned)rng[0], step = (unsigned)rng[1];
-        for (long i = (long)blockIdx.x * 256 + threadIdx.x; 4 * i < n_noise; i += stride) {
-            unsigned w[4];
-            philox4x32_10((unsigned)i, (unsigned)(i >> 32), step, 0u, seed, 0x5EEDu, w);
-            const float4 u = make_float4((w[0] >> 8) * 5.9604644775390625e-8f, (w[1] >> 8) * 5.9604644775390625e-8f,
-                                         (w[2] >> 8) * 5.9604644775390625e-8f, (w[3] >> 8) * 5.9604644775390625e-8f);
-            if (4 * i + 3 < n_noise) st4(noise + 4 * i, u);
-            else { const float uv[4] = {u.x, u.y, u.z, u.w}; for (int k = 0; 4 * i + k < n_noise; ++k) noise[4 * i + k] = uv[k]; }
-        }
-    }
+    step_begin_body(z0, n0, z1, n1, src, tidx, BT, N, lda, base, noise, n_noise, rng, blockIdx.x, gridDim.x);
 }
 
 extern "C" int gptst_step_begin(float* z0, long n0, float* z1, long n1, const float* src, float* tidx, int BT, int N, int lda, int base,
                                 float* noise, long n_noise, const int* rng, void* stream) {
     if (!z0 || n0 <= 0 || n1 < 0 || (n1 > 0 && !z1) || (tidx && (!src || BT <= 0 || N <= 0 || lda < base + 2))) return GPTST_EARG;
     if (noise && (n_noise <= 0 || !rng)) return GPTST_EARG;
-    long q = (n0 + n1) / 4;
-    int nb = (int)((q + 255) / 256); if (nb > 1024) nb = 1024; if (nb < 1) nb = 1;
+    const int nb = step_begin_blocks(n0, n1);
     hipLaunchKernelGGL(step_begin_kernel, dim3(nb), dim3(256), 0, (hipStream_t)stream, z0, n0, z1, n1, src, tidx, BT, N, lda, base, noise,
                        noise ? n_noise : 0L, rng);
     GPTST_CHECK_LAUNCH();
diff --git a/gpt-st_amd/csrc/stepbegin_dev.h b/gpt-st_amd/csrc/stepbegin_dev.h
--- /dev/null
+++ b/gpt-st_amd/csrc/stepbegin_dev.h
@@ -0,0 +1,46 @@
+#pragma once
+#include "common.h"
+
+__device__ __forceinline__ void philox4x32_10(unsigned c0, unsigned c1, unsigned c2, unsigned c3, unsigned k0, unsigned k1, unsigned (&o)[4]) {
+#pragma unroll
+    for (int r = 0; r < 10; ++r) {
+        const unsigned long long p0 = 0xD2511F53ull * c0, p1 = 0xCD9E8D57ull * c2;
+        const unsigned n0 = (unsigned)(p1 >> 32) ^ c1 ^ k0, n1 = (unsigned)p1, n2 = (unsigned)(p0 >> 32) ^ c3 ^ k1, n3 = (unsigned)p0;
+        c0 = n0; c1 = n1; c2 = n2; c3 = n3;
+        k0 += 0x9E3779B9u; k1 += 0xBB67AE85u;
+    }
+    o[0] = c0; o[1] = c1; o[2] = c2; o[3] = c3;
+}
+
+__device__ __forceinline__ void step_begin_body(float* __restrict__ z0, long n0, float* __restrict__ z1, long n1, const float* __restrict__ src,
+                                                float* __restrict__ tidx, int BT, int N, int lda, int base, float* __restrict__ noise,
+                                                long n_noise, const int* __restrict__ rng, int blk, int nblk) {
+    const long q0 = n0 / 4, q1 = n1 / 4, stride = (long)nblk * 256;
+    for (long i = (long)blk * 256 + threadIdx.x; i < q0 + q1; i += stride) {
+        if (i < q0) st4(z0 + 4 * i, f4zero()); else st4(z1 + 4 * (i - q0), f4zero());
+    }
+    if (blk == 0) {
+        for (long i = 4 * q0 + threadIdx.x; i < n0; i += 256) z0[i] = 0.f;
+        for (long i = 4 * q1 + threadIdx.x; i < n1; i += 256) z1[i] = 0.f;
+    }
+    if (tidx != nullptr)
+        for (long i = (long)blk * 256 + threadIdx.x; i < 2L * BT; i += stride)
+            tidx[i] = src[(size_t)(i / 2) * N * lda + base + (i & 1)];
+    if (noise != nullptr) {
+        const unsigned seed = (unsigned)rng[0], step = (unsigned)rng[1];
+        for (long i = (long)blk * 256 + threadIdx.x; 4 * i < n_noise; i += stride) {
+            unsigned w[4];
+            philox4x32_10((unsigned)i, (unsigned)(i >> 32), step, 0u, seed, 0x5EEDu, w);
+            const float4 u = make_float4((w[0] >> 8) * 5.9604644775390625e-8f, (w[1] >> 8) * 5.9604644775390625e-8f,
+                                         (w[2] >> 8) * 5.9604644775390625e-8f, (w[3] >> 8) * 5.9604644775390625e-8f);
+            if (4 * i + 3 < n_noise) st4(noise + 4 * i, u);
+            else { const float uv[4] = {u.x, u.y, u.z, u.w}; for (int k = 0; 4 * i + k < n_noise; ++k) noise[4 * i + k] = uv[k]; }
+        }
+    }
+}
+
+static inline int step_begin_blocks(long n0, long n1) {
+    const long q = (n0 + n1) / 4;
+    int nb = (int)((q + 255) / 256); if (nb > 1024) nb = 1024; if (nb < 1) nb = 1;
+    return nb;
+}
diff --git a/gpt-st_amd/csrc/stephead.hip b/gpt-st_amd/csrc/stephead.hip
--- /dev/null
+++ b/gpt-st_amd/csrc/stephead.hip
@@ -0,0 +1,96 @@
+#include "common.h"
+#include "guidein_dev.h"
+#include "poolgen_dev.h"
+#include "stepbegin_dev.h"
+#include "timefeat_dev.h"
+
+#define SH_MAXPJ 8
+struct ShPJobs { PJob j[SH_MAXPJ]; int n; };
+struct ShBegin {
+    float* z0; long n0; float* z1; long n1;
+    const float* src; float* tidx; int BT, N, lda, base;
+    float* noise; long n_noise; const int* rng;
+};
+
+__device__ __forceinline__ void sh_pj_role(const ShPJobs& t, int rel) {
+    int p = 0;
+    for (int q = 1; q < t.n; ++q) if (rel >= t.j[q].blk0) p = q;
+    const PJob& a = t.j[p];
+    const int r = rel - a.blk0;
+    pj_fwd_mfma(a, r % a.nbx, r / a.nbx, PG_MFMA_ROWS, threadIdx.x);
+}
+
+__global__ __launch_bounds__(256, 6) void step_head_a_kernel(ShBegin b, TfJobs tf, ShPJobs pj, int ntf, int npj, int nbegin) {
+    __shared__ float shraw[TF_SH_FLOATS];
+    const int blk = blockIdx.x;
+    if (blk < ntf) tf_fwd_jobs(tf, b.src + b.base, (long)b.N * b.lda, blk, shraw);
+    else if (blk < ntf + npj) sh_pj_role(pj, blk - ntf);
+    else step_begin_body(b.z0, b.n0, b.z1, b.n1, b.src, b.tidx, b.BT, b.N, b.lda, b.base, b.noise, b.n_noise, b.rng, blk - ntf - npj, nbegin);
+}
+
+__global__ __launch_bounds__(256) void step_head_b_kernel(ShPJobs pj, int npj, const float* __restrict__ w1, const float* __restrict__ b1,
+                                                          const float* __restrict__ Wn, const float* __restrict__ bn, float* __restrict__ uc) {
+    __shared__ __attribute__((aligned(16))) float part[GUIDE_UC_LDS(64)];
+    const int blk = blockIdx.x;
+    if (blk < npj) sh_pj_role(pj, blk);
+    else guide_uc_body<64>(w1, b1, Wn, bn, uc, blk - npj, part);
+}
+
+GPTST_INTERNAL int gptst_pj_embed_table(PJobs* t, int njobs, const int* kind, const void* const* emb, const void* const* pool, const void* const* out,
+                                        const int* R, const int* K, const int* cols, int* nf, int* nvb, int* ngw);
+
+static int sh_table(ShPJobs* s, int njobs, const void* const* emb, const void* const* pool, const void* const* out, const int* R, const int* K,
+                    const int* cols, int* nb) {
+    s->n = 0; *nb = 0;
+    if (njobs == 0) return GPTST_OK;
+    if (njobs < 0 || njobs > SH_MAXPJ) return GPTST_ESHAPE;
+    if (!emb || !pool || !out || !R || !K || !cols) return GPTST_EARG;
+    PJobs t;
+    int nf = 0, ngw = 0;
+    const int rc = gptst_pj_embed_table(&t, njobs, nullptr, emb, pool, out, R, K, cols, &nf, nb, &ngw);
+    if (rc) return rc;
+    for (int p = 0; p < t.n; ++p) s->j[p] = t.j[p];
+    s->n = t.n;
+    return GPTST_OK;
+}
+
+extern "C" int gptst_step_head_a(float* z0, long n0, float* z1, long n1, const float* src, float* tidx, int BT, int N, int lda, int base, float* noise,
+                                 long n_noise, const int* rng, int ntf, const void* const* tf_params, const void* const* tf_out, const int* tf_rows,
+                                 const int* tf_K, const int* tf_E, int npj, const void* const* emb, const void* const* pool, const void* const* out,
+                                 const int* R, const int* K, const int* cols, void* stream) {
+    if (!z0 || n0 <= 0 || n1 < 0 || (n1 > 0 && !z1) || !tidx || !src || BT <= 0 || N <= 0 || lda < base + 2 || base < 0) return GPTST_EARG;
+    if (noise && (n_noise <= 0 || !rng)) return GPTST_EARG;
+    if (ntf <= 0 || ntf > TF_MAXJ || !tf_params || !tf_out || !tf_rows || !tf_K || !tf_E) return GPTST_EARG;
+    TfJobs tf; tf.n = ntf;
+    for (int q = 0; q < ntf; ++q) {
+        const float* const* pp = (const float* const*)tf_params + 10 * q;
+        if ((long)tf_rows[q] * tf_K[q] > BT) return GPTST_EARG;
+        tf.j[q] = TfJob{TfParams{pp[0], pp[1], pp[2], pp[3], pp[4], pp[5], pp[6], pp[7], pp[8], pp[9]}, TfGrads{}, nullptr, (float*)tf_out[q], nullptr,
+                        tf_rows[q], tf_K[q], tf_E[q], 0};
+    }
+    const int nbt = tf_fwd_number(tf);
+    if (nbt < 0) return nbt;
+    ShPJobs pj;
+    int nbp = 0;
+    const int rc = sh_table(&pj, npj, emb, pool, out, R, K, cols, &nbp);
+    if (rc) return rc;
+    const int nbb = step_begin_blocks(n0, n1);
+    const ShBegin b{z0, n0, z1, n1, src, tidx, BT, N, lda, base, noise, noise ? n_noise : 0L, rng};
+    hipLaunchKernelGGL(step_head_a_kernel, dim3(nbt + nbp + nbb), dim3(256), 0, (hipStream_t)stream, b, tf, pj, nbt, nbp, nbb);
+    GPTST_CHECK_LAUNCH();
+    return GPTST_OK;
+}
+
+extern "C" int gptst_step_head_b(int npj, const void* const* emb, const void* const* pool, const void* const* out, const int* R, const int* K,
+                                 const int* cols, const float* w1, const float* b1, const float* Wn, const float* bn, float* uc, int N, int C,
+                                 void* stream) {
+    if (!w1 || !b1 || !Wn || !bn || !uc || N <= 0) return GPTST_EARG;
+    if (C != 64) return GPTST_ESHAPE;
+    ShPJobs pj;
+    int nbp = 0;
+    const int rc = sh_table(&pj, npj, emb, pool, out, R, K, cols, &nbp);
+    if (rc) return rc;
+    hipLaunchKernelGGL(step_head_b_kernel, dim3(nbp + N), dim3(256), 0, (hipStream_t)stream, pj, nbp, w1, b1, Wn, bn, uc);
+    GPTST_CHECK_LAUNCH();
+    return GPTST_OK;
+}
diff --git a/gpt-st_amd/csrc/timefeat.hip b/gpt-st_amd/csrc/timefeat.hip
--- a/gpt-st_amd/csrc/timefeat.hip
+++ b/gpt-st_amd/csrc/timefeat.hip
@@ -1,58 +1,6 @@
 #include "common.h"
 
-struct TfParams {
-    const float *wd, *bd, *ww, *bw, *w1, *b1, *w2, *b2, *w3, *b3;
-};
-struct TfGrads {
-    float *wd, *bd, *ww, *bw, *w1, *b1, *w2, *b2, *w3, *b3;
-};
-
-template <int E, int NT = 256> struct TfCfg { static constexpr int ROWS = NT / E; };
-
-template <int E>
-__device__ __forceinline__ float tf_matvec(const float (&wrow)[E], float b, const float* __restrict__ xline) {
-    float s = b;
-#pragma unroll
-    for (int i = 0; i < E; ++i) s = fmaf(wrow[i], xline[i], s);
-    return s;
-}
-
-template <int E>
-__device__ __forceinline__ float tf_input(const TfParams& p, const float* __restrict__ tidx, int r, int e, int K) {
-    float s = p.bd[e] + p.bw[e];
-    for (int k = 0; k < K; ++k) {
-        s = fmaf(p.wd[e * K + k], tidx[((size_t)r * K + k) * 2 + 0], s);
-        s = fmaf(p.ww[e * K + k], tidx[((size_t)r * K + k) * 2 + 1], s);
-    }
-    return s;
-}
-
-#define TF_SH_FLOATS (7 * 128 * 3)
-
-template <int E>
-__device__ __forceinline__ void tf_fwd_body(const TfParams& p, const float* __restrict__ tidx, float* __restrict__ out,
-                                            int rows, int K, int blk, float* __restrict__ shraw) {
-    constexpr int ROWS = TfCfg<E>::ROWS;
-    float (*line)[E + 1] = reinterpret_cast<float (*)[E + 1]>(shraw);
-    const int e = threadIdx.x % E, rl = threadIdx.x / E;
-    const int r = blk * ROWS + rl;
-    const bool valid = r < rows;
-    float w1[E], w2[E], w3[E];
-#pragma unroll
-    for (int i = 0; i < E; ++i) { w1[i] = p.w1[e * E + i]; w2[i] = p.w2[e * E + i]; w3[i] = p.w3[e * E + i]; }
-    line[rl][e] = valid ? tf_input<E>(p, tidx, r, e, K) : 0.f;
-    __syncthreads();
-    float h = fmaxf(tf_matvec<E>(w1, p.b1[e], line[rl]), 0.f);
-    __syncthreads();
-    line[rl][e] = h;
-    __syncthreads();
-    h = fmaxf(tf_matvec<E>(w2, p.b2[e], line[rl]), 0.f);
-    __syncthreads();
-    line[rl][e] = h;
-    __syncthreads();
-    h = tf_matvec<E>(w3, p.b3[e], line[rl]);
-    if (valid) out[(size_t)r * E + e] = h;
-}
+#include "timefeat_dev.h"
 
 template <bool DET> __device__ __forceinline__ void tf_add(float* p, float v) { if (DET) *p += v; else atomicAdd(p, v); }
 
@@ -70,7 +18,7 @@
         w1[i] = p.w1[e * E + i]; w2[i] = p.w2[e * E + i]; w3[i] = p.w3[e * E + i];
         c1[i] = p.w1[i * E + e]; c2[i] = p.w2[i * E + e]; c3[i] = p.w3[i * E + e];
     }
-    const float h0 = valid ? tf_input<E>(p, tidx, r, e, K) : 0.f;
+    const float h0 = valid ? tf_input<E>(p, tidx, 2, r, e, K) : 0.f;
     sh[0][rl][e] = h0;
     __syncthreads();
     const float h1 = fmaxf(tf_matvec<E>(w1, p.b1[e], sh[0][rl]), 0.f);
@@ -118,10 +66,6 @@
     }
 }
 
-#define TF_MAXJ 16
-struct TfJob { TfParams p; TfGrads g; const float* tidx; float* out; const float* dout; int rows, K, E, blk0; };
-struct TfJobs { TfJob j[TF_MAXJ]; int n; };
-
 #define TF_DET_T 1024
 template <int BWD>
 __global__ __launch_bounds__(BWD == 2 ? TF_DET_T : 256) void timefeat_jobs_kernel(TfJobs t) {
@@ -137,7 +81,7 @@
     case EE:                                                                                     \
         if (BWD == 2) { for (int b2 = 0; b2 < nblk; ++b2) { tf_bwd_body<EE, true, NT>(a.p, a.g, a.tidx, a.dout, a.rows, a.K, b2, shraw); __syncthreads(); } } \
         else if (BWD == 1) tf_bwd_body<EE, false, NT>(a.p, a.g, a.tidx, a.dout, a.rows, a.K, blk, shraw); \
-        else tf_fwd_body<EE>(a.p, a.tidx, a.out, a.rows, a.K, blk, shraw);                       \
+        else tf_fwd_body<EE>(a.p, a.tidx, 2, a.out, a.rows, a.K, blk, shraw);                       \
         break;
     switch (a.E) { TF_CASE(2) TF_CASE(4) TF_CASE(8) TF_CASE(16) default: break; }
 #undef TF_CASE
diff --git a/gpt-st_amd/csrc/timefeat_dev.h b/gpt-st_amd/csrc/timefeat_dev.h
--- /dev/null
+++ b/gpt-st_amd/csrc/timefeat_dev.h
@@ -0,0 +1,85 @@
+#pragma once
+#include "common.h"
+
+struct TfParams {
+    const float *wd, *bd, *ww, *bw, *w1, *b1, *w2, *b2, *w3, *b3;
+};
+struct TfGrads {
+    float *wd, *bd, *ww, *bw, *w1, *b1, *w2, *b2, *w3, *b3;
+};
+
+template <int E, int NT = 256> struct TfCfg { static constexpr int ROWS = NT / E; };
+
+template <int E>
+__device__ __forceinline__ float tf_matvec(const float (&wrow)[E], float b, const float* __restrict__ xline) {
+    float s = b;
+#pragma unroll
+    for (int i = 0; i < E; ++i) s = fmaf(wrow[i], xline[i], s);
+    return s;
+}
+
+template <int E>
+__device__ __forceinline__ float tf_input(const TfParams& p, const float* __restrict__ tidx, long ts, int r, int e, int K) {
+    float s = p.bd[e] + p.bw[e];
+    for (int k = 0; k < K; ++k) {
+        s = fmaf(p.wd[e * K + k], tidx[((size_t)r * K + k) * ts + 0], s);
+        s = fmaf(p.ww[e * K + k], tidx[((size_t)r * K + k) * ts + 1], s);
+    }
+    return s;
+}
+
+#define TF_SH_FLOATS (7 * 128 * 3)
+
+template <int E>
+__device__ __forceinline__ void tf_fwd_body(const TfParams& p, const float* __restrict__ tidx, long ts, float* __restrict__ out,
+                                            int rows, int K, int blk, float* __restrict__ shraw) {
+    constexpr int ROWS = TfCfg<E>::ROWS;
+    float (*line)[E + 1] = reinterpret_cast<float (*)[E + 1]>(shraw);
+    const int e = threadIdx.x % E, rl = threadIdx.x / E;
+    const int r = blk * ROWS + rl;
+    const bool valid = r < rows;
+    float w1[E], w2[E], w3[E];
+#pragma unroll
+    for (int i = 0; i < E; ++i) { w1[i] = p.w1[e * E + i]; w2[i] = p.w2[e * E + i]; w3[i] = p.w3[e * E + i]; }
+    line[rl][e] = valid ? tf_input<E>(p, tidx, ts, r, e, K) : 0.f;
+    __syncthreads();
+    float h = fmaxf(tf_matvec<E>(w1, p.b1[e], line[rl]), 0.f);
+    __syncthreads();
+    line[rl][e] = h;
+    __syncthreads();
+    h = fmaxf(tf_matvec<E>(w2, p.b2[e], line[rl]), 0.f);
+    __syncthreads();
+    line[rl][e] = h;
+    __syncthreads();
+    h = tf_matvec<E>(w3, p.b3[e], line[rl]);
+    if (valid) out[(size_t)r * E + e] = h;
+}
+
+#define TF_MAXJ 16
+struct TfJob { TfParams p; TfGrads g; const float* tidx; float* out; const float* dout; int rows, K, E, blk0; };
+struct TfJobs { TfJob j[TF_MAXJ]; int n; };
+
+__device__ __forceinline__ void tf_fwd_jobs(const TfJobs& t, const float* __restrict__ tidx, long ts, int blk, float* __restrict__ shraw) {
+    int q = 0;
+    for (int i = 1; i < t.n; ++i) if (blk >= t.j[i].blk0) q = i;
+    const TfJob& a = t.j[q];
+    switch (a.E) {
+        case 2: tf_fwd_body<2>(a.p, tidx, ts, a.out, a.rows, a.K, blk - a.blk0, shraw); break;
+        case 4: tf_fwd_body<4>(a.p, tidx, ts, a.out, a.rows, a.K, blk - a.blk0, shraw); break;
+        case 8: tf_fwd_body<8>(a.p, tidx, ts, a.out, a.rows, a.K, blk - a.blk0, shraw); break;
+        case 16: tf_fwd_body<16>(a.p, tidx, ts, a.out, a.rows, a.K, blk - a.blk0, shraw); break;
+        default: break;
+    }
+}
+
+static inline int tf_fwd_number(TfJobs& t) {
+    int nb = 0;
+    for (int q = 0; q < t.n; ++q) {
+        TfJob& a = t.j[q];
+        if (!a.p.wd || !a.out || a.rows <= 0 || a.K <= 0) return GPTST_EARG;
+        if (a.E != 2 && a.E != 4 && a.E != 8 && a.E != 16) return GPTST_ESHAPE;
+        a.blk0 = nb;
+        nb += (a.rows + 256 / a.E - 1) / (256 / a.E);
+    }
+    return nb;
+}
diff --git a/gpt-st_amd/engine.py b/gpt-st_amd/engine.py
--- a/gpt-st_amd/engine.py
+++ b/gpt-st_amd/engine.py
@@ -451,8 +451,13 @@
     return dict(emb=emb, gen=(A_all, hts, cps, d, Hm, ds, HS, HT), Wb=Wb, Wn=Wn, dadj=dadj, dyn=dyn)
 
 
-def gen_all(p, tidx, dims, which=(ENC, DEC), guide=True, defer=False):
-    B, T, N, C = dims
+HEAD_ROLES = os.environ.get("GPTST_HEAD_ROLES", "0") == "1"
+
+
+def gen_all(p, tidx, dims, which=(ENC, DEC), guide=True, defer=False, begin=None):
+    B, T, N, C = dims
+    if begin is not None:
+        return _gen_all_head(p, dims, which, guide, begin)
     tfj = []
     for pfx in which:
         tfj += [_tf_job(p, pfx + "time_feature1.", tidx), _tf_job(p, pfx + "time_feature1_.", tidx),
@@ -485,6 +490,48 @@
         res["pending"] = jobs
         return res
     jobs.launch()
+    return res
+
+
+def _gen_all_head(p, dims, which, guide, begin):
+    src = begin["src"]
+    B, T = src.shape[0], src.shape[1]
+    tfj = []
+    for pfx in which:
+        tfj += [(_tf_tensors(p, pfx + "time_feature1."), B * T, 1), (_tf_tensors(p, pfx + "time_feature1_."), B * T, 1),
+                (_tf_tensors(p, pfx + "time_feature2."), B, T)]
+    if guide:
+        tfj.append((_tf_tensors(p, GUIDE_TF), B * T, 1))
+    embs = ops.timefeat_outs(tfj, src.device)
+    ja, jb = ops.PoolJobs(), ops.PoolJobs()
+    res = {}
+    if guide:
+        m = "encoder.MLP_RL."
+        t4m = embs[-1]
+        res["guide"] = (t4m, ja.fwd(p["encoder.neb4mask"], p[m + "weights_pool_spa"]), ja.fwd(p["encoder.neb4mask"], p[m + "bias_pool_spa"]),
+                        jb.fwd(t4m, p[m + "weights_pool_tem"]), jb.fwd(t4m, p[m + "bias_pool_tem"]))
+    tidx = ops.step_head_a(begin["z0"], begin["z1"], src, begin["base"], tfj, embs, ja, noise=begin["noise"], rng=begin["rng"])
+    if tidx is None:
+        tidx = ops.step_begin(begin["z0"], begin["z1"], src, begin["base"], noise=begin["noise"], rng=begin["rng"])
+        ops.timefeat_jobs_fwd(tfj, tidx, outs=embs)
+        ja.jobs += jb.jobs
+        jb.jobs = []
+        ja.launch()
+    res["tidx"] = tidx
+    if guide:
+        res["guide_pending"] = jb
+    jobs = ops.PoolJobs()
+    L = 4 * len(which)
+    if L:
+        Hm = p[which[0] + "hyperTem1.adj"].shape[1]
+        N = dims[2]
+        A_all = torch.empty(L, N, Hm * T, device=src.device)
+        G_all = torch.empty(L, N, T, T, device=src.device)
+        for k, pfx in enumerate(which):
+            res[pfx] = _sthcn_gen_jobs(p, pfx, embs[3 * k:3 * k + 3], jobs, A_all[4 * k:4 * k + 4], dims, G_all[4 * k:4 * k + 4])
+            res[pfx]["slot"] = (k, len(which))
+            res[pfx]["G_all"] = G_all[4 * k:4 * k + 4]
+    res["pending"] = jobs
     return res
 
 
@@ -640,14 +687,20 @@
 GUIDE_HEAD = os.environ.get("GPTST_GUIDE_HEAD", "1") == "1"
 
 
-def guide_fwd(p, source, tidx, dims, base, gen=None, lowrank_in=False):
+def guide_fwd(p, source, tidx, dims, base, gen=None, lowrank_in=False, pend=None):
     B, T, N, C = dims
     if gen is None:
         gen = gen_all(p, tidx, dims, which=(), guide=True)["guide"]
     t4m, Wspa, bspa, Wtem, btem = gen
     m = "encoder.MLP_RL."
-    if lowrank_in and GUIDEIN and GUIDE_HEAD and base == 1 and C == 64:
-        r = ops.guide_head_fwd(source, p[m + "ln1.weight"], p[m + "ln1.bias"], Wspa, bspa, Wtem, btem, p[m + "ln3.weight"], p[m + "ln3.bias"])
+    head = lowrank_in and GUIDEIN and GUIDE_HEAD and base == 1 and C == 64
+    uc = None
+    if pend is not None:
+        if head and ops.guide_head_ok(C, p[m + "ln3.weight"].shape[0]):
+            uc = ops.step_head_b(pend, p[m + "ln1.weight"], p[m + "ln1.bias"], Wspa, bspa)
+        pend.launch()
+    if head:
+        r = ops.guide_head_fwd(source, p[m + "ln1.weight"], p[m + "ln1.bias"], Wspa, bspa, Wtem, btem, p[m + "ln3.weight"], p[m + "ln3.bias"], uc=uc)
         if r is not None:
             h1, h2, prob, label = r
             return prob, (t4m, ("lowrank", Wspa), (h1, h2, Wtem), h2, label)
diff --git a/gpt-st_amd/ops.py b/gpt-st_amd/ops.py
--- a/gpt-st_amd/ops.py
+++ b/gpt-st_amd/ops.py
@@ -323,18 +323,26 @@
     return h1
 
 
-def guide_head_fwd(source, w1, b1, Wn, bn, Wbt, bbt, W3, b3):
+def guide_head_ok(C, J):
+    return C == 64 and J <= 16
+
+
+def guide_head_fwd(source, w1, b1, Wn, bn, Wbt, bbt, W3, b3, uc=None):
     B, T, N, F = source.shape
     C, J = Wn.shape[-1], W3.shape[0]
-    if C != 64 or J > 16:
+    if not guide_head_ok(C, J):
         return None
     _chk(source, w1, b1, Wn, bn, Wbt, bbt, W3, b3)
     dev = source.device
     f = dict(device=dev, dtype=torch.float32)
-    uc = torch.empty(N, 2 * C, **f)
     h1, h2 = torch.empty(B * T * N, C, **f), torch.empty(B * T * N, C, **f)
     prob = torch.empty(B * T * N, J, **f)
     label = torch.empty(B * T * N, device=dev, dtype=torch.int32)
+    if uc is not None:
+        _call("gptst_guide_head_rows", _p(source), F, _p(uc), _p(Wbt), _p(bbt), _p(W3), _p(b3), _p(h1), _p(h2), _p(prob), _p(label), B * T, N, C, J,
+              nbytes=_nb(Wbt, h1, h2, prob))
+        return h1, h2, prob, label
+    uc = torch.empty(N, 2 * C, **f)
     _call("gptst_guide_head_fwd", _p(source), F, _p(w1), _p(b1), _p(Wn), _p(bn), _p(Wbt), _p(bbt), _p(W3), _p(b3), _p(uc), _p(h1), _p(h2), _p(prob),
           _p(label), B * T, N, C, J, nbytes=_nb(Wbt, h1, h2, prob))
     return h1, h2, prob, label
@@ -801,8 +809,13 @@
     _call("gptst_timefeat_bwd", *[_p(t) for t in params], *[_p(t) for t in grads], _p(tidx), _p(dout), rows, K, E)
 
 
-def timefeat_jobs_fwd(jobs, tidx):
-    outs = [torch.empty(rows, params[1].numel(), device=tidx.device, dtype=torch.float32) for params, rows, K in jobs]
+def timefeat_outs(jobs, device):
+    return [torch.empty(rows, params[1].numel(), device=device, dtype=torch.float32) for params, rows, K in jobs]
+
+
+def timefeat_jobs_fwd(jobs, tidx, outs=None):
+    if outs is None:
+        outs = timefeat_outs(jobs, tidx.device)
     _call("gptst_timefeat_jobs", len(jobs), 0, _ptrs([t for params, _, _ in jobs for t in params]), None, _p(tidx), _ptrs(outs),
           _ints([r for _, r, _ in jobs]), _ints([k for _, _, k in jobs]), _ints([params[1].numel() for params, _, _ in jobs]))
     return outs
@@ -886,6 +899,48 @@
     return tidx
 
 
+def _served(name, *args, **kw):
+    try:
+        _call(name, *args, **kw)
+    except _C.GptstError as e:
+        if e.code != _C.ESHAPE:
+            raise
+        return False
+    return True
+
+
+def _fwd_cols(gen):
+    js = gen.jobs if gen is not None else []
+    assert all(j[0] == PoolJobs.FWD for j in js)
+    col = lambda i: [j[i] for j in js]
+    return len(js), _ptrs(col(1)), _ptrs(col(3)), _ptrs(col(4)), _ints(col(5)), _ints(col(6)), _ints(col(7))
+
+
+def step_head_a(z0, z1, src, base, tf_jobs, tf_outs, gen=None, noise=None, rng=None):
+    B, T, N, lda = src.shape
+    tidx = torch.empty(B, T, 2, device=src.device, dtype=torch.float32)
+    ok = _served("gptst_step_head_a", _p(z0), z0.numel(), _p(z1), z1.numel() if z1 is not None else 0, _p(src), _p(tidx), B * T, N, lda, base,
+                 _p(noise), noise.numel() if noise is not None else 0, _p(rng), len(tf_jobs), _ptrs([t for params, _, _ in tf_jobs for t in params]),
+                 _ptrs(tf_outs), _ints([r for _, r, _ in tf_jobs]), _ints([k for _, _, k in tf_jobs]), _ints([params[1].numel() for params, _, _ in tf_jobs]),
+                 *_fwd_cols(gen))
+    if not ok:
+        return None
+    if gen is not None:
+        gen.jobs = []
+    return tidx
+
+
+def step_head_b(gen, w1, b1, Wn, bn):
+    _chk(w1, b1, Wn, bn)
+    N, C = Wn.shape[0], Wn.shape[-1]
+    uc = torch.empty(N, 2 * C, device=Wn.device, dtype=torch.float32)
+    if not _served("gptst_step_head_b", *_fwd_cols(gen), _p(w1), _p(b1), _p(Wn), _p(bn), _p(uc), N, C):
+        return None
+    if gen is not None:
+        gen.jobs = []
+    return uc
+
+
 def clip_adam(p, g, m, v, nA, nB, hyper, stats, ws=None, stats_out=None, sws=None):
     if ws is None:
         if p.device not in _ADAM_WS:
diff --git a/gpt-st_amd/step.py b/gpt-st_amd/step.py
--- a/gpt-st_amd/step.py
+++ b/gpt-st_amd/step.py
@@ -119,9 +119,14 @@
         engine.CTX.ARENA, engine.CTX.NODE_REDUCE = self.arena, self.node_reduce
         src = self.src
         noise = None if self.inject_noise or self.force_mask else self._noise_buffer(phase)
-        tidx = ops.step_begin(self.gbuf, self.arena.begin(zero=False), src, base, noise=noise, rng=self.rng_words)
         need_guide = self._need_guide(phase)
-        gen = engine.gen_all(p, tidx, dims, guide=need_guide, defer=DEFER_GEN)
+        begin = dict(z0=self.gbuf, z1=self.arena.begin(zero=False), src=src, base=base, noise=noise, rng=self.rng_words)
+        if DEFER_GEN and engine.HEAD_ROLES:
+            gen = engine.gen_all(p, None, dims, guide=need_guide, defer=True, begin=begin)
+            tidx = gen.pop("tidx")
+        else:
+            tidx = ops.step_begin(begin["z0"], begin["z1"], src, base, noise=noise, rng=self.rng_words)
+            gen = engine.gen_all(p, tidx, dims, guide=need_guide, defer=DEFER_GEN)
         red = engine.Reductions()
         red.no_carry = self.deterministic
         self._dec_reduced = False
@@ -129,7 +134,8 @@
             red.on_bucket = self._bucket_ready
             red.bucket_inline, red.fork_side = True, self.fork_side
         lowrank = self.fused_tails and engine.chain_ok(dims)
-        prob, sv_g = engine.guide_fwd(p, src, tidx, dims, base, gen=gen["guide"], lowrank_in=lowrank) if need_guide else (None, None)
+        prob, sv_g = (engine.guide_fwd(p, src, tidx, dims, base, gen=gen["guide"], lowrank_in=lowrank, pend=gen.pop("guide_pending", None))
+                      if need_guide else (None, None))
         if self._needs_exchange(phase):
             self.label_l.copy_(sv_g[4])
         return dict(tidx=tidx, gen=gen, red=red, prob=prob, sv_g=sv_g)
diff --git a/include/gptst_hip.h b/include/gptst_hip.h
--- a/include/gptst_hip.h
+++ b/include/gptst_hip.h
@@ -9,7 +9,7 @@
 #pragma GCC visibility push(default)
 #endif
 
-#define GPTST_ABI_VERSION 16
+#define GPTST_ABI_VERSION 17
 int gptst_abi_version(void);
 int gptst_set_deterministic(int on);
 int gptst_handoff_timeouts(int* out);
@@ -86,6 +86,8 @@
 int gptst_guide_head_fwd(const float* src, int lda, const float* w1, const float* b1, const float* Wn, const float* bn, const float* Wbt,
                          const float* bbt, const float* W3, const float* b3, float* uc, float* h1, float* h2, float* prob, int* label,
                          int BT, int N, int C, int J, void* stream);
+int gptst_guide_head_rows(const float* src, int lda, const float* uc, const float* Wbt, const float* bbt, const float* W3, const float* b3,
+                          float* h1, float* h2, float* prob, int* label, int BT, int N, int C, int J, void* stream);
 
 int gptst_hypertem_ntiles(int N);
 int gptst_hypertem_bwd(const float* dOut, const float* Y, const float* X, const float* G, const float* Wbt, float* dX, float* dbias,
@@ -210,6 +212,14 @@
 int gptst_step_begin(float* z0, long n0, float* z1, long n1, const float* src, float* tidx, int BT, int N, int lda, int base,
                      float* noise, long n_noise, const int* rng, void* stream);
 
+int gptst_step_head_a(float* z0, long n0, float* z1, long n1, const float* src, float* tidx, int BT, int N, int lda, int base, float* noise,
+                      long n_noise, const int* rng, int ntf, const void* const* tf_params, const void* const* tf_out, const int* tf_rows,
+                      const int* tf_K, const int* tf_E, int npj, const void* const* emb, const void* const* pool, const void* const* out,
+                      const int* R, const int* K, const int* cols, void* stream);
+int gptst_step_head_b(int npj, const void* const* emb, const void* const* pool, const void* const* out, const int* R, const int* K,
+                      const int* cols, const float* w1, const float* b1, const float* Wn, const float* bn, float* uc, int N, int C,
+                      void* stream);
+
 int gptst_mae_fwd(const float* out, const float* src, int lda, const float* mask, float sigma, float mu, float thresh, int rows,
                   int J, float* stats, void* stream);
 int gptst_mae_bwd(const float* out, const float* src, int lda, const float* mask, float sigma, float mu, float thresh, int rows,
```

New measurement: 924.1 steps/s. Within noise of the previous version (-0.1%).
